# AbrahamSanders/realtime-codec-agent

Measured on AMD Instinct MI355X. Metric: batch-encode audio-hours/hour (+ xRT and p50 frame-step latency of 1 duplex stream in `duplex`), higher is better.
Workload: dtype f32; 1 GPU; batch MagiCodec-style encode, 16 kHz stereo, 0.1 s chunks / 2.0 s context, 256 windows per step (BASELINE configs[1]); codebook=131072x16

## Files before the change

include/rca.h:

```cpp
#ifndef RCA_H
#define RCA_H

#include <stdint.h>

#ifdef __cplusplus
extern "C" {
#endif

#define RCA_OK 0
#define RCA_ERR_ARG -1
#define RCA_ERR_HIP -2
#define RCA_ERR_STATE -3
#define RCA_ERR_MISSING -4

#define RCA_MAX_STAGES 8

typedef struct rca_codec rca_codec_t;
typedef struct rca_lm rca_lm_t;

#define RCA_F32 0
#define RCA_BF16 1
#define RCA_Q8_0 2
#define RCA_F16 3
#define RCA_Q6_K 5
// ... 92 lines not shown
    int32_t n_kv_heads;
    int32_t head_dim;
    int32_t ffn;
    int32_t n_ctx;
    float rms_eps;
    float rope_theta;
    int32_t rope_scaling;
    float rope_factor;
    float rope_low_freq_factor;
    float rope_high_freq_factor;
    int32_t rope_orig_ctx;
    int32_t logits_all;
    int32_t decode_weights;
} rca_lm_config_t;

typedef struct {
    int32_t top_k;
    float top_p;
    float min_p;
    float temp;
    uint32_t seed;
    int32_t n_bias;
    const int32_t* bias_ids;
    const float* bias_vals;
    float repeat_penalty;
    float freq_penalty;
    float presence_penalty;
    int32_t penalty_last_n;
} rca_sampler_params_t;

int rca_lm_create(const rca_lm_config_t* cfg, const rca_tensor_t* tensors, int32_t n_tensors,
                  int32_t device, rca_lm_t** out);
int rca_lm_create_random(const rca_lm_config_t* cfg, uint64_t seed, float init_std, int32_t device,
                         rca_lm_t** out);
int rca_lm_create_shared(rca_lm_t* parent, int32_t n_ctx, int32_t logits_all, rca_lm_t** out);
int rca_lm_destroy(rca_lm_t* h);

int rca_lm_reset(rca_lm_t* h);
int rca_lm_eval(rca_lm_t* h, const int32_t* ids, int32_t n);
int rca_lm_eval_async(rca_lm_t* h, const int32_t* ids, int32_t n);
int rca_lm_copy_kv(rca_lm_t* dst, rca_lm_t* src, int32_t n_pos);
int rca_lm_swap_kv(rca_lm_t* a, rca_lm_t* b);
int rca_lm_kv_remove(rca_lm_t* h, int32_t p0, int32_t p1);
int rca_lm_kv_read(rca_lm_t* h, int32_t layer, int32_t pos0, int32_t n_pos, uint16_t* k_host, uint16_t* v_host);
int rca_lm_set_low_priority(rca_lm_t* h, int32_t enable);
int rca_lm_get_n_tokens(const rca_lm_t* h, int32_t* n);
int rca_lm_set_n_tokens(rca_lm_t* h, int32_t n);
int rca_lm_get_logits(rca_lm_t* h, float* out_host);
int rca_lm_get_logits_row(rca_lm_t* h, int32_t pos, float* out_host);
int rca_lm_logits_dev(rca_lm_t* h, const float** out_dev);

int rca_lm_sampler_init(rca_lm_t* h, const rca_sampler_params_t* p);
int rca_lm_sample(rca_lm_t* h, int32_t* token);
int rca_lm_step(rca_lm_t* h, const int32_t* ids, int32_t n, int32_t* token);
int rca_lm_frame(rca_lm_t* h, const int32_t* first_pair, const int32_t* user_ids, int32_t n_steps, int32_t audio_id_floor,
                 int32_t* out_tokens, int32_t* n_done);
typedef struct rca_duplex_frame_args {
    const float* pcm_window;
    const int64_t* code_ctx;
    int32_t T;
    int32_t F_ctx;
    int32_t n_steps;
    int32_t n_samples;
    int32_t code_token_base;
    int32_t audio_id_floor;
    int32_t probe_id;
    int32_t first_pair[2];
} rca_duplex_frame_args_t;
typedef struct rca_duplex_frame_out {
    int64_t user_codes[8];
    int32_t tokens[8];
    int32_t n_done;
    int32_t flags;
    float probe_prob;
} rca_duplex_frame_out_t;
int rca_duplex_frame(rca_lm_t* lm, rca_codec_t* codec, const rca_duplex_frame_args_t* args, rca_duplex_frame_out_t* out,
                     float* pcm_out_host);
int rca_duplex_prepare(rca_lm_t* lm, int32_t T, int32_t F_ctx, int32_t n_steps, int32_t n_samples);
int rca_duplex_precapture(rca_lm_t* lm, rca_lm_t* twin, rca_codec_t* codec, const rca_duplex_frame_args_t* args, int32_t n_probe);
int rca_codec_workspace_sig(rca_codec_t* h, uint64_t* sig);
int rca_codec_stream_handoff(rca_codec_t* h, void* stream);
int rca_codec_codebook_size(const rca_codec_t* h, int32_t* n);
int rca_lm_step_probe(rca_lm_t* h, const int32_t* ids, int32_t n, const int32_t* probe_ids, int32_t n_probe, int32_t* token, float* probs_out);
int rca_lm_token_probs(rca_lm_t* h, const int32_t* token_ids, int32_t n, float* probs_out);
int rca_lm_mask_head_rows(rca_lm_t* h, int32_t row_begin, int32_t row_end);
int rca_lm_persist_codec_embeddings(rca_lm_t* h, const float* codec_embed, int32_t n_codes, int32_t dim,
                                    const float* w1, const float* b1, const float* w2, const float* b2,
                                    int32_t codec_vocab_start, float* out_f32);
int rca_lm_set_logits_all(rca_lm_t* h, int32_t enable);
int rca_lm_set_graphs(rca_lm_t* h, int32_t enable);
int rca_lm_set_mfma_prefill(rca_lm_t* h, int32_t enable);
int rca_lm_prefill_route(const rca_lm_t* h, int32_t* route);
int rca_lm_weight_format(const rca_lm_t* h, int32_t* fmt, int64_t* bytes_per_step);
int rca_lm_set_attn_fuse(rca_lm_t* h, int32_t enable);
int rca_lm_set_act_format(rca_lm_t* h, int32_t fmt);
int rca_lm_get_act_format(const rca_lm_t* h, int32_t* fmt);
int rca_lm_gemv_tap(rca_lm_t* h, int32_t layer, int32_t kind, const float* x_host, int32_t M, float* y_host, int64_t y_numel,
                    uint16_t* kv_host);
int rca_lm_sync(rca_lm_t* h);
int rca_codec_sync(rca_codec_t* h);

#ifdef __cplusplus
}
#endif
#endif
```

realtime_codec_agent_amd/_native.py:

```python
from __future__ import annotations

import ctypes as C
import os
import subprocess
from typing import Dict, Iterable, List, Optional, Tuple

import numpy as np

_PKG_DIR = os.path.dirname(os.path.abspath(__file__))
CSRC_DIR = os.path.join(_PKG_DIR, "csrc")
LIB_PATH = os.environ.get("RCA_LIB_PATH") or os.path.join(_PKG_DIR, "librca_hip.so")
HIP_SOURCES = ["rca_codec.hip", "rca_lm.hip"]
HIPCC_FLAGS = ["--offload-arch=gfx950", "-O3", "-ffp-contract=off", "-std=c++17", "-fPIC", "-shared",
               "-Wno-unused-result", "-mllvm", "-amdgpu-kernarg-preload-count=14"]

MAX_STAGES = 8
RCA_F32, RCA_BF16, RCA_Q8_0, RCA_F16, RCA_Q4_K, RCA_Q6_K, RCA_Q5_K, RCA_Q4_0, RCA_Q4_1 = 0, 1, 2, 3, 4, 5, 6, 7, 8


class RcaError(RuntimeError):
    pass


class Q8Blocks:
# ... 135 lines not shown


class Tensor(C.Structure):
    _fields_ = [("name", C.c_char_p), ("data", C.c_void_p), ("numel", C.c_int64), ("dtype", C.c_int32)]


class CodecConfigC(C.Structure):
    _fields_ = [
        ("sample_rate", C.c_int32),
        ("n_stages", C.c_int32),
        ("strides", C.c_int32 * MAX_STAGES),
        ("channels", C.c_int32 * (MAX_STAGES + 1)),
        ("k_in", C.c_int32),
        ("k_latent", C.c_int32),
        ("latent_dim", C.c_int32),
        ("codebook_size", C.c_int32),
        ("codebook_raw_dim", C.c_int32),
        ("codebook_dim", C.c_int32),
        ("leaky_slope", C.c_float),
    ]


class LMConfigC(C.Structure):
    _fields_ = [
        ("vocab_size", C.c_int32),
        ("hidden", C.c_int32),
        ("n_layers", C.c_int32),
        ("n_heads", C.c_int32),
        ("n_kv_heads", C.c_int32),
        ("head_dim", C.c_int32),
        ("ffn", C.c_int32),
        ("n_ctx", C.c_int32),
        ("rms_eps", C.c_float),
        ("rope_theta", C.c_float),
        ("rope_scaling", C.c_int32),
        ("rope_factor", C.c_float),
        ("rope_low_freq_factor", C.c_float),
        ("rope_high_freq_factor", C.c_float),
        ("rope_orig_ctx", C.c_int32),
        ("logits_all", C.c_int32),
        ("decode_weights", C.c_int32),
    ]


class SamplerParamsC(C.Structure):
    _fields_ = [
        ("top_k", C.c_int32),
        ("top_p", C.c_float),
        ("min_p", C.c_float),
        ("temp", C.c_float),
        ("seed", C.c_uint32),
        ("n_bias", C.c_int32),
        ("bias_ids", C.POINTER(C.c_int32)),
        ("bias_vals", C.POINTER(C.c_float)),
        ("repeat_penalty", C.c_float),
        ("freq_penalty", C.c_float),
        ("presence_penalty", C.c_float),
        ("penalty_last_n", C.c_int32),
    ]


class DuplexFrameArgsC(C.Structure):
    _fields_ = [
        ("pcm_window", C.c_void_p),
        ("code_ctx", C.c_void_p),
        ("T", C.c_int32),
        ("F_ctx", C.c_int32),
        ("n_steps", C.c_int32),
        ("n_samples", C.c_int32),
        ("code_token_base", C.c_int32),
        ("audio_id_floor", C.c_int32),
        ("probe_id", C.c_int32),
        ("first_pair", C.c_int32 * 2),
    ]


class DuplexFrameOutC(C.Structure):
    _fields_ = [
        ("user_codes", C.c_int64 * 8),
        ("tokens", C.c_int32 * 8),
        ("n_done", C.c_int32),
        ("flags", C.c_int32),
        ("probe_prob", C.c_float),
    ]


def sources() -> List[str]:
    return [os.path.join(CSRC_DIR, s) for s in HIP_SOURCES if os.path.exists(os.path.join(CSRC_DIR, s))]


def _build_key() -> Tuple[str, List[str], List[str]]:
    import hashlib
    extra = os.environ.get("RCA_EXTRA_HIPCC_FLAGS", "").split()
    hipcc = os.environ.get("HIPCC", "/opt/rocm/bin/hipcc")
    if not os.path.exists(hipcc):
        hipcc = "hipcc"
    cflags = [f for f in HIPCC_FLAGS if f != "-shared"] + extra
    return hashlib.sha1(" ".join([hipcc] + cflags).encode()).hexdigest()[:10], hipcc, cflags


def _stamp_path() -> str:
    return LIB_PATH + ".flags"


def needs_build() -> bool:
    if not os.path.exists(LIB_PATH):
        return True
    try:
        with open(_stamp_path()) as f:
            if f.read().strip() != _build_key()[0]:
                return True
    except OSError:
        return True
    deps = sources() + [os.path.join(CSRC_DIR, f) for f in os.listdir(CSRC_DIR) if f.endswith(".h")]
    deps.append(os.path.join(os.path.dirname(_PKG_DIR), "include", "rca.h"))
    t = os.path.getmtime(LIB_PATH)
    return any(os.path.getmtime(d) > t for d in deps if os.path.exists(d))


def build(force: bool = False, verbose: bool = False) -> str:
    key, hipcc, cflags = _build_key()
    extra = os.environ.get("RCA_EXTRA_HIPCC_FLAGS", "").split()
    if extra and not os.environ.get("RCA_LIB_PATH"):
        raise RcaError(f"RCA_EXTRA_HIPCC_FLAGS={' '.join(extra)!r} without RCA_LIB_PATH: a diagnostic build must not replace "
                       f"{LIB_PATH}; set RCA_LIB_PATH=/tmp/<name>.so")
    if not force and not needs_build():
        return LIB_PATH
    import fcntl
    obj_dir = os.path.join(CSRC_DIR, ".obj")
    os.makedirs(obj_dir, exist_ok=True)
    with open(os.path.join(obj_dir, ".lock"), "w") as lock:
        fcntl.flock(lock, fcntl.LOCK_EX)
        if not force and not needs_build():
            return LIB_PATH
        headers = [os.path.join(CSRC_DIR, f) for f in os.listdir(CSRC_DIR) if f.endswith(".h")]
        headers.append(os.path.join(os.path.dirname(_PKG_DIR), "include", "rca.h"))
        hdr_t = max([os.path.getmtime(p) for p in headers if os.path.exists(p)] + [0.0])
        sfx = f".{os.getpid()}.tmp"
        objs, jobs = [], []
        for src in sources():
            obj = os.path.join(obj_dir, f"{os.path.splitext(os.path.basename(src))[0]}.{key}.o")
            objs.append(obj)
            if force or not os.path.exists(obj) or os.path.getmtime(obj) < max(os.path.getmtime(src), hdr_t):
                cmd = [hipcc] + cflags + ["-c", src, "-o", obj + sfx]
                if verbose:
                    print(" ".join(cmd))
                jobs.append((subprocess.Popen(cmd), cmd, obj))
        tmps = [obj + sfx for _, _, obj in jobs] + [LIB_PATH + sfx]
        try:
            failed = [cmd for p, cmd, _ in jobs if p.wait() != 0]
            if failed:
                raise subprocess.CalledProcessError(1, failed[0])
            for _, _, obj in jobs:
                os.replace(obj + sfx, obj)
            cmd = [hipcc, "--offload-arch=gfx950", "-shared", "-fPIC"] + objs + ["-o", LIB_PATH + sfx]
            if verbose:
                print(" ".join(cmd))
            subprocess.check_call(cmd)
            os.replace(LIB_PATH + sfx, LIB_PATH)
            with open(_stamp_path() + sfx, "w") as f:
                f.write(key + "\n")
            os.replace(_stamp_path() + sfx, _stamp_path())
        finally:
            for t in tmps + [_stamp_path() + sfx]:
                if os.path.exists(t):
                    os.remove(t)
    return LIB_PATH


_lib = None

ABI_SYMBOLS = [
    "rca_last_error", "rca_device_count", "rca_device_sync", "rca_version",
    "rca_codec_create", "rca_codec_destroy", "rca_codec_hop", "rca_codec_num_frames",
    "rca_codec_encode", "rca_codec_encode_dev", "rca_codec_encode_windows_dev", "rca_codec_encode_chunk_range_dev", "rca_codec_encode_rows_dev",
    "rca_codec_decode", "rca_codec_decode_dev",
    "rca_codec_encode_tail_dev", "rca_codec_decode_tail_dev", "rca_codec_encode_tail", "rca_codec_decode_tail", "rca_codec_set_stream_graphs", "rca_codec_receptive_field", "rca_codec_set_window_trim",
    "rca_codec_encoder_dev", "rca_codec_quantize_dev", "rca_codec_decoder_dev", "rca_codec_codebook_dev",
    "rca_codec_codebook", "rca_codec_encode_tap", "rca_codec_encode_tap_bf16", "rca_codec_set_variant", "rca_codec_sync",
    "rca_codec_profile", "rca_codec_profile_read",
    "rca_lm_create", "rca_lm_create_random", "rca_lm_destroy", "rca_lm_reset", "rca_lm_eval",
    "rca_lm_get_n_tokens", "rca_lm_set_n_tokens", "rca_lm_get_logits", "rca_lm_get_logits_row",
    "rca_lm_logits_dev", "rca_lm_sampler_init", "rca_lm_sample", "rca_lm_step", "rca_lm_token_probs",
    "rca_lm_sync", "rca_lm_set_graphs", "rca_lm_mask_head_rows", "rca_lm_set_mfma_prefill", "rca_lm_set_logits_all",
    "rca_lm_persist_codec_embeddings", "rca_lm_create_shared", "rca_lm_eval_async", "rca_lm_copy_kv", "rca_lm_swap_kv",
    "rca_lm_set_low_priority", "rca_lm_frame", "rca_lm_weight_format", "rca_lm_set_attn_fuse", "rca_lm_prefill_route",
    "rca_lm_set_act_format", "rca_lm_get_act_format", "rca_lm_gemv_tap", "rca_lm_kv_remove", "rca_lm_kv_read",
    "rca_duplex_frame", "rca_codec_workspace_sig", "rca_codec_stream_handoff", "rca_codec_codebook_size", "rca_codec_set_mfma_mode", "rca_lm_step_probe", "rca_duplex_prepare", "rca_duplex_precapture",
]


def lib():
    global _lib
    if _lib is not None:
        return _lib
    if not os.path.exists(LIB_PATH):
        raise RcaError(
            f"{LIB_PATH} not found: build the HIP extension first (python -c 'import __graft_entry__ as g; g.build()'). "
            "There is no CPU fallback for the product path."
        )
    import torch
    try:
        _lib = C.CDLL(LIB_PATH)
    except OSError as e:
        raise RcaError(f"cannot load {LIB_PATH}: {e}") from e
    _lib.rca_last_error.restype = C.c_char_p
    _lib.rca_version.restype = C.c_char_p
    return _lib


def check(rc: int, what: str = "") -> None:
    if rc != 0:
        msg = lib().rca_last_error()
        raise RcaError(f"{what} failed (rc={rc}): {msg.decode(errors='replace') if msg else ''}")


def make_tensors(weights: Dict[str, np.ndarray]) -> Tuple[C.Array, list]:
    keep = []
    arr = (Tensor * len(weights))()
    for i, (name, a) in enumerate(weights.items()):
        if isinstance(a, (Q8Blocks, Q4KBlocks, Q5KBlocks, Q6KBlocks, Q40Blocks)):
            raw = np.ascontiguousarray(a.raw)
            nb = name.encode()
            keep += [raw, nb]
            arr[i] = Tensor(nb, raw.ctypes.data, int(np.prod(a.shape)), {Q8Blocks: RCA_Q8_0, Q4KBlocks: RCA_Q4_K, Q5KBlocks: RCA_Q5_K, Q6KBlocks: RCA_Q6_K, Q40Blocks: RCA_Q4_0, Q41Blocks: RCA_Q4_1}[type(a)])
            continue
        if a.dtype == np.uint16:
            dt = RCA_BF16
        elif a.dtype == np.float16:
            dt = RCA_F16
        else:
            a = np.ascontiguousarray(a, dtype=np.float32)
            dt = RCA_F32
        a = np.ascontiguousarray(a)
        nb = name.encode()
        keep += [a, nb]
        arr[i] = Tensor(nb, a.ctypes.data, a.size, dt)
    return arr, keep


def codec_config_c(cfg) -> CodecConfigC:
    c = CodecConfigC()
    c.sample_rate = cfg.sample_rate
    c.n_stages = len(cfg.strides)
    for i, s in enumerate(cfg.strides):
        c.strides[i] = s
    for i, ch in enumerate(cfg.channels):
        c.channels[i] = ch
    c.k_in, c.k_latent, c.latent_dim = cfg.k_in, cfg.k_latent, cfg.latent_dim
    c.codebook_size, c.codebook_raw_dim, c.codebook_dim = cfg.codebook_size, cfg.codebook_raw_dim, cfg.codebook_dim
    c.leaky_slope = cfg.leaky_slope
    return c
```

realtime_codec_agent_amd/csrc/rca_lm.hip:

```cpp
#include <algorithm>
#include <type_traits>
#include <cmath>

#include "rca_common.h"

using namespace rca;

typedef unsigned short bf16_t;
typedef _Float16 f16_t;
typedef unsigned u32x4 __attribute__((ext_vector_type(4)));
typedef float f32x4 __attribute__((ext_vector_type(4)));
typedef _Float16 f16x2 __attribute__((ext_vector_type(2)));

#define LM_MAXM 1024
#define LM_STATE_DECODE_BYTES (8 + 4 * 16)
#define LM_TILE32 32
#define LM_GEMV_M 2
#define LM_PREFILL_MIN 8
#define LM_KSLICE 2048
#define LM_MAXSPLIT 4
#define ATT_KEYS 256
#define LM_GRAPH_BUCKETS 8
#define ATT_EPOCH_INTS 64
#define ATT_TAG_MAXSP 128
#define ATT_TAG_SPINS (1 << 22)
#define SAMP_MAXK 256
#define LM_FRAME_MAX 8
#define LM_FRAME_USER0 8

struct LmDevState {
    int n_tokens;
    int m;
    int ids[LM_MAXM];
    unsigned long long rng_counter;
    int out_token;
    int pad;
    int frame_out[LM_FRAME_MAX];
};

struct SamplerDev {
    int top_k;
    float top_p, min_p, temp;
    unsigned long long seed;
    int n_bias;
    int bias_ids[8];
    float bias_vals[8];
    float repeat_penalty, freq_penalty, presence_penalty;
    int last_n;
    int patch;
    int big_k;
    int big_p;
};

typedef float f32x16 __attribute__((ext_vector_type(16)));
__device__ __forceinline__ bf16_t f32_to_bf16_rne(float f) {
    unsigned u = __float_as_uint(f);
    u += 0x7FFFu + ((u >> 16) & 1u);
    return (bf16_t)(u >> 16);
}
__device__ __forceinline__ float bf16_lo(unsigned u) { return __uint_as_float(u << 16); }
__device__ __forceinline__ float bf16_hi(unsigned u) { return __uint_as_float(u & 0xffff0000u); }
template <int CTRL>
__device__ __forceinline__ float dpp_mov(float v) {
    return __builtin_bit_cast(float, __builtin_amdgcn_update_dpp(0, __builtin_bit_cast(int, v), CTRL, 0xF, 0xF, true));
}
#define DPP_XOR1 0xB1
#define DPP_XOR2 0x4E
#define DPP_ROR4 0x124
#define DPP_ROR8 0x128
#define DPP_HALF_MIRROR 0x141
template <typename OP>
__device__ __forceinline__ float wave_butterfly(float v, OP op) {
    float a = v, b = v;
    asm volatile("s_nop 1\n\tv_permlane32_swap_b32 %0, %1\n\ts_nop 1" : "+v"(a), "+v"(b));
    v = op(a, b);
    a = v; b = v;
    asm volatile("s_nop 1\n\tv_permlane16_swap_b32 %0, %1\n\ts_nop 1" : "+v"(a), "+v"(b));
    v = op(a, b);
    v = op(v, dpp_mov<DPP_ROR8>(v));
    v = op(v, dpp_mov<DPP_ROR4>(v));
    v = op(v, dpp_mov<DPP_XOR2>(v));
    v = op(v, dpp_mov<DPP_XOR1>(v));
    return v;
}
__device__ __forceinline__ float wave_sum(float v) {
    return wave_butterfly(v, [](float a, float b) { return a + b; });
}
__device__ __forceinline__ float wave_max(float v) {
    return wave_butterfly(v, [](float a, float b) { return fmaxf(a, b); });
}

__global__ __launch_bounds__(256) void lm_embed_kernel(const LmDevState* __restrict__ stt, const void* __restrict__ table, int f32tab,
                                                       float* __restrict__ x, int H, int V) {
    const int m = blockIdx.x;
    if (m >= stt->m) return;
    int id = stt->ids[m];
    id = id < 0 ? 0 : (id >= V ? V - 1 : id);
    if (f32tab) {
        const float* row = reinterpret_cast<const float*>(table) + (long)id * H;
        for (int h = threadIdx.x; h < H; h += 256) x[(long)m * H + h] = row[h];
// ... 1695 lines not shown
        }
    }
}
__global__ __launch_bounds__(256) void lm_q8_pack_kernel(const signed char* __restrict__ q, const f16_t* __restrict__ d, int N, int K, int qkv_pairs,
                                                         u32x4* __restrict__ qs, unsigned* __restrict__ sc) {
    const long nchunk = K >> 3, npairs = N >> 1;
    for (long i = (long)blockIdx.x * blockDim.x + threadIdx.x; i < npairs * nchunk; i += (long)gridDim.x * blockDim.x) {
        const long pp = i / nchunk;
        const int c = (int)(i - pp * nchunk);
        const long ra = qkv_pairs ? (pp >> 5) * 64 + (pp & 31) : 2 * pp;
        const long rb = qkv_pairs ? ra + 32 : ra + 1;
        const uint2 a = *reinterpret_cast<const uint2*>(q + ra * K + 8 * c);
        const uint2 b = *reinterpret_cast<const uint2*>(q + rb * K + 8 * c);
        qs[i] = u32x4{a.x, a.y, b.x, b.y};
        if ((c & 3) == 0) {
            const unsigned short da = __builtin_bit_cast(unsigned short, d[ra * (K >> 5) + (c >> 2)]);
            const unsigned short db = __builtin_bit_cast(unsigned short, d[rb * (K >> 5) + (c >> 2)]);
            sc[q8_sc_index(pp, c >> 2, K >> 5)] = (unsigned)da | ((unsigned)db << 16);
        }
    }
}

struct WMat {
    int fmt = WF_BF16;
    int N = 0, K = 0;
    bf16_t* w = nullptr;
    u32x4* qs = nullptr;
    unsigned* sc = nullptr;
    unsigned* dd = nullptr;
    unsigned* qh = nullptr;
    void release() {
        for (void* p : {(void*)w, (void*)qs, (void*)sc, (void*)dd, (void*)qh})
            if (p) (void)hipFree(p);
        w = nullptr; qs = nullptr; sc = nullptr; dd = nullptr; qh = nullptr;
    }
    const bf16_t* wptr() const { return fmt == WF_Q5K ? reinterpret_cast<const bf16_t*>(qh) : w; }
    long stream_bytes() const {
        const long n = (long)N * K;
        if (fmt == WF_Q5K) return n / 2 + n / 8 + n / 16 + n / 64;
        if (fmt == WF_Q40 || fmt == WF_Q41) return n / 2 + n / 8;
        return fmt == WF_Q8 ? n + n / 16 : (fmt == WF_Q4K ? n / 2 + n / 16 + n / 64 : (fmt == WF_Q6K ? n + n / 4 : 2 * n));
    }
};
struct LmLayer {
    WMat qkv, o, gu, down;
    WMat vseg;
    bool split_v = false;
    float *attn_norm = nullptr, *ffn_norm = nullptr;
};

struct rca_lm {
    int n_cus = 256;
    rca_lm_config_t cfg;
    int device = 0;
    hipStream_t stream = nullptr;
    void* embed = nullptr;
    int embed_f32 = 0;
    WMat head;
    float* final_norm = nullptr;
    std::vector<LmLayer> layers;
    float *cos_t = nullptr, *sin_t = nullptr;
    f16_t *kc = nullptr, *vc = nullptr;
    f16_t* kv_stage = nullptr;
    long kv_layer_stride = 0;
    int n_ctx_pad = 0, n_splits = 0;
    float *x = nullptr, *xn = nullptr, *qkv = nullptr, *attn = nullptr, *hbuf = nullptr,
          *att_part = nullptr, *logits = nullptr, *probs_dev = nullptr;
    int* probe_ids_dev = nullptr;
    int* att_arrive = nullptr;
    bf16_t *xh = nullptr, *xl = nullptr;
    float* gpart = nullptr;
    long logits_rows_cap = 0;
    int logits_rows = 0;
    LmDevState* stt = nullptr;
    SamplerDev* samp = nullptr;
    SampWork* swork = nullptr;
    LmDevState* h_stt = nullptr;
    int* h_probe = nullptr;
    int n_tokens = 0;
    bool sampler_set = false;
    bool samp_full = false;
    bool samp_patch = false, samp_big_k = false, samp_big_p = false;
    struct GraphSet { const f16_t* kc = nullptr; hipGraphExec_t g[3][LM_GRAPH_BUCKETS] = {}; hipGraphExec_t fg[LM_FRAME_MAX + 1][LM_GRAPH_BUCKETS] = {};
                      hipGraphExec_t gp[3][LM_GRAPH_BUCKETS] = {}; int gp_nprobe[3][LM_GRAPH_BUCKETS] = {};
                      int tile_m[2] = {0, 0}; hipGraphExec_t tile_g[2] = {nullptr, nullptr}; int tile_seen[2] = {0, 0};
                      unsigned long long last_use = 0; };
    GraphSet gset[2];
    unsigned long long gset_clock = 0;
    bool async_pending = false;
    unsigned long long rng_host = 0;
    bool graphs_enabled = true;
    bool mfma_prefill = true;
    bool fuse_attn = true;
    int act_format = 0;
    rca_lm* weights_of = nullptr;
    int borrowers = 0;
    bool zombie = false;
    struct DuplexState* duplex = nullptr;
};
struct DuplexState;
static void duplex_destroy(DuplexState* d);
static void duplex_drop_graphs(DuplexState* d);

static int lm_alloc(void** p, size_t bytes) {
    hipError_t e = hipMalloc(p, bytes);
    if (e != hipSuccess) return fail(RCA_ERR_HIP, "hipMalloc(%zu) -> %s", bytes, hipGetErrorString(e));
    return RCA_OK;
}

static void lm_free_weights(rca_lm* h) {
    for (auto& L : h->layers) {
        for (WMat* m : {&L.qkv, &L.o, &L.gu, &L.down, &L.vseg}) m->release();
        for (void* p : {(void*)L.attn_norm, (void*)L.ffn_norm})
            if (p) (void)hipFree(p);
    }
    h->head.release();
    for (void* p : {(void*)h->embed, (void*)h->final_norm, (void*)h->cos_t, (void*)h->sin_t})
        if (p) (void)hipFree(p);
    h->layers.clear();
    h->embed = nullptr;
    h->final_norm = h->cos_t = h->sin_t = nullptr;
}

static void lm_drop_graph_set(rca_lm::GraphSet& gs) {
    for (int i = 0; i < 3; ++i)
        for (int b = 0; b < LM_GRAPH_BUCKETS; ++b) {
            if (gs.g[i][b]) { (void)hipGraphExecDestroy(gs.g[i][b]); gs.g[i][b] = nullptr; }
            if (gs.gp[i][b]) { (void)hipGraphExecDestroy(gs.gp[i][b]); gs.gp[i][b] = nullptr; }
        }
    for (int i = 0; i <= LM_FRAME_MAX; ++i)
        for (int b = 0; b < LM_GRAPH_BUCKETS; ++b)
            if (gs.fg[i][b]) { (void)hipGraphExecDestroy(gs.fg[i][b]); gs.fg[i][b] = nullptr; }
    for (int i = 0; i < 2; ++i) {
        if (gs.tile_g[i]) { (void)hipGraphExecDestroy(gs.tile_g[i]); gs.tile_g[i] = nullptr; }
        gs.tile_m[i] = gs.tile_seen[i] = 0;
    }
    gs.kc = nullptr;
}
static void lm_drop_graphs(rca_lm* h) {
    for (auto& gs : h->gset) lm_drop_graph_set(gs);
    duplex_drop_graphs(h->duplex);
}
static rca_lm::GraphSet& lm_graph_set(rca_lm* h) {
    rca_lm::GraphSet* hit = nullptr;
    for (auto& gs : h->gset)
        if (gs.kc == h->kc) hit = &gs;
    if (!hit) {
        hit = h->gset[0].last_use <= h->gset[1].last_use ? &h->gset[0] : &h->gset[1];
        lm_drop_graph_set(*hit);
        hit->kc = h->kc;
    }
    hit->last_use = ++h->gset_clock;
    return *hit;
}
template <class F>
static int lm_capture(hipStream_t st, hipGraphExec_t* exec, const char* tag, F&& enqueue) {
    hipGraph_t g = nullptr;
    RCA_HIP(hipStreamSynchronize(st));
    RCA_HIP(hipStreamBeginCapture(st, hipStreamCaptureModeThreadLocal));
    const int rc = enqueue();
    hipError_t e = hipStreamEndCapture(st, &g);
    if (rc != RCA_OK) { if (g) (void)hipGraphDestroy(g); return rc; }
    if (e != hipSuccess) return fail(RCA_ERR_HIP, "%s capture: %s", tag, hipGetErrorString(e));
    e = hipGraphInstantiate(exec, g, nullptr, nullptr, 0);
    (void)hipGraphDestroy(g);
    if (e != hipSuccess) { *exec = nullptr; return fail(RCA_ERR_HIP, "%s graph instantiate: %s", tag, hipGetErrorString(e)); }
    (void)hipGraphUpload(*exec, st);
    return RCA_OK;
}

extern "C" int rca_lm_destroy(rca_lm_t* h) {
    if (!h) return RCA_OK;
    (void)hipSetDevice(h->device);
    if (h->stream) (void)hipStreamSynchronize(h->stream);
    lm_drop_graphs(h);
    duplex_destroy(h->duplex);
    h->duplex = nullptr;
    for (void* p : {(void*)h->kc, (void*)h->vc, (void*)h->kv_stage, (void*)h->x, (void*)h->xn, (void*)h->qkv, (void*)h->attn, (void*)h->hbuf,
                    (void*)h->att_part, (void*)h->logits, (void*)h->probs_dev, (void*)h->probe_ids_dev, (void*)h->att_arrive, (void*)h->xh, (void*)h->xl,
                    (void*)h->gpart, (void*)h->stt, (void*)h->samp, (void*)h->swork})
        if (p) (void)hipFree(p);
    h->kc = h->vc = h->kv_stage = nullptr;
    h->x = h->xn = h->qkv = h->attn = h->hbuf = h->att_part = h->logits = h->probs_dev = h->gpart = nullptr;
    h->probe_ids_dev = nullptr; h->att_arrive = nullptr; h->xh = h->xl = nullptr; h->stt = nullptr; h->samp = nullptr; h->swork = nullptr;
    if (h->h_stt) { (void)hipHostFree(h->h_stt); h->h_stt = nullptr; }
    if (h->h_probe) { (void)hipHostFree(h->h_probe); h->h_probe = nullptr; }
    if (h->stream) { (void)hipStreamDestroy(h->stream); h->stream = nullptr; }
    if (h->weights_of) {
        rca_lm* owner = h->weights_of;
        h->layers.clear();
        if (--owner->borrowers == 0 && owner->zombie) { lm_free_weights(owner); delete owner; }
        delete h;
        return RCA_OK;
    }
    if (h->borrowers > 0) {
        h->zombie = true;
        return RCA_OK;
    }
    lm_free_weights(h);
    delete h;
    return RCA_OK;
}

static int lm_check_cfg(const rca_lm_config_t* c) {
    if (!c) return fail(RCA_ERR_ARG, "null config");
    if (c->head_dim != 64) return fail(RCA_ERR_ARG, "head_dim must be 64 (got %d)", c->head_dim);
    if (c->n_kv_heads < 1 || c->n_heads % c->n_kv_heads) return fail(RCA_ERR_ARG, "n_heads must be a multiple of n_kv_heads");
    const int G = c->n_heads / c->n_kv_heads;
    if (G != 1 && G != 2 && G != 4) return fail(RCA_ERR_ARG, "query group size %d unsupported (1, 2, 4)", G);
    if (c->hidden % 8 || c->ffn % 8 || (c->n_heads * c->head_dim) % 8) return fail(RCA_ERR_ARG, "hidden/ffn must be multiples of 8");
    if (c->hidden > LM_KSLICE || c->n_heads * c->head_dim > LM_KSLICE) return fail(RCA_ERR_ARG, "hidden > %d unsupported", LM_KSLICE);
    if (c->ffn > LM_KSLICE * LM_MAXSPLIT) return fail(RCA_ERR_ARG, "ffn > %d unsupported", LM_KSLICE * LM_MAXSPLIT);
    if (c->ffn > LM_KSLICE && c->ffn % LM_KSLICE) return fail(RCA_ERR_ARG, "ffn above %d must be a multiple of it", LM_KSLICE);
    if (c->vocab_size < 2 || c->n_layers < 1 || c->n_ctx < 2) return fail(RCA_ERR_ARG, "bad sizes");
    if (c->decode_weights < 0 || c->decode_weights > 6) return fail(RCA_ERR_ARG, "decode_weights %d (0 as supplied, 1 q8_0, 2 f16, 3 q4_k, 4 q5_k, 5 q4_0, 6 q4_1)", c->decode_weights);
// ... 365 lines not shown
        const size_t sc_bytes = (size_t)((npairs + 7) / 8) * (K / 16) * 8 * 2 * 4;
        if ((rc = lm_alloc((void**)&out->qs, (size_t)npairs * nchunk * 16)) != RCA_OK || (rc = lm_alloc((void**)&out->sc, sc_bytes)) != RCA_OK) { raw->release(); return rc; }
        (void)hipMemsetAsync(out->sc, 0, sc_bytes, h->stream);
        lm_q6k_pack_kernel<<<4096, 256, 0, h->stream>>>(raw->q, (const signed char*)raw->d, (const f16_t*)raw->dd, N, K, qkv_pairs, out->qs, (float*)out->sc);
        hipError_t e = hipStreamSynchronize(h->stream);
        raw->release();
        if (e != hipSuccess) return fail(RCA_ERR_HIP, "Q6_K pack of %s: %s", what, hipGetErrorString(e));
        return RCA_OK;
    }
    if (raw->fmt != WF_Q8) {
        out->w = raw->w16;
        raw->w16 = nullptr;
        return RCA_OK;
    }
    const int N = out->N, K = out->K;
    if ((K % 32) || (N % 2) || (qkv_pairs && (N % 64))) { raw->release(); return fail(RCA_ERR_ARG, "q8_0 weights: %s is %d x %d (K must be a multiple of 32, N even)", what, N, K); }
    int rc;
    const long npairs = N / 2, nchunk = K / 8;
    if ((rc = lm_alloc((void**)&out->qs, (size_t)npairs * nchunk * 16)) != RCA_OK ||
        (rc = lm_alloc((void**)&out->sc, (size_t)((npairs + 7) / 8) * (K / 32) * 8 * 4)) != RCA_OK) { raw->release(); return rc; }
    (void)hipMemsetAsync(out->sc, 0, (size_t)((npairs + 7) / 8) * (K / 32) * 8 * 4, h->stream);
    lm_q8_pack_kernel<<<4096, 256, 0, h->stream>>>(raw->q, raw->d, N, K, qkv_pairs, out->qs, out->sc);
    hipError_t e = hipStreamSynchronize(h->stream);
    raw->release();
    if (e != hipSuccess) return fail(RCA_ERR_HIP, "q8_0 pack of %s: %s", what, hipGetErrorString(e));
    return RCA_OK;
}

static int g128_splits(int N, int K);
static bool lm_can_gemm128(const rca_lm* h);
static int lm_common_init(rca_lm* h, const rca_tensor_t* ts, int nt, const rca_lm* rope_src = nullptr) {
    const rca_lm_config_t& c = h->cfg;
    int rc;
    const int half = c.head_dim / 2;
    h->n_ctx_pad = (c.n_ctx + ATT_KEYS - 1) / ATT_KEYS * ATT_KEYS;
    h->n_splits = h->n_ctx_pad / ATT_KEYS;
    if (rope_src) {
        h->cos_t = rope_src->cos_t;
        h->sin_t = rope_src->sin_t;
    } else {
    std::vector<float> inv(half);
    const rca_tensor_t* tinv = find_tensor(ts, nt, "rope.inv_freq");
    if (tinv) {
        if (tinv->numel != half || tinv->dtype != RCA_F32) return fail(RCA_ERR_ARG, "rope.inv_freq must hold %d f32", half);
        memcpy(inv.data(), tinv->data, half * sizeof(float));
    } else {
        for (int i = 0; i < half; ++i) {
            double f = 1.0 / pow((double)c.rope_theta, (double)(2 * i) / (double)c.head_dim);
            if (c.rope_scaling == 1) {
                const double low_wl = (double)c.rope_orig_ctx / c.rope_low_freq_factor;
                const double high_wl = (double)c.rope_orig_ctx / c.rope_high_freq_factor;
                const double wl = 2.0 * M_PI / f;
                if (wl > low_wl) f = f / c.rope_factor;
                else if (wl >= high_wl) {
                    const double smooth = ((double)c.rope_orig_ctx / wl - c.rope_low_freq_factor) / (c.rope_high_freq_factor - c.rope_low_freq_factor);
                    f = (1.0 - smooth) * f / c.rope_factor + smooth * f;
                }
            }
            inv[i] = (float)f;
        }
    }
    float* inv_dev = nullptr;
    if ((rc = lm_alloc((void**)&inv_dev, half * 4)) != RCA_OK) return rc;
    RCA_HIP(hipMemcpy(inv_dev, inv.data(), half * 4, hipMemcpyHostToDevice));
    if ((rc = lm_alloc((void**)&h->cos_t, (size_t)h->n_ctx_pad * half * 4)) != RCA_OK) return rc;
    if ((rc = lm_alloc((void**)&h->sin_t, (size_t)h->n_ctx_pad * half * 4)) != RCA_OK) return rc;
    lm_rope_table_kernel<<<cdiv((long)h->n_ctx_pad * half, 256), 256, 0, h->stream>>>(inv_dev, h->cos_t, h->sin_t, h->n_ctx_pad, half);
    RCA_HIP(hipStreamSynchronize(h->stream));
    (void)hipFree(inv_dev);
    }
    h->kv_layer_stride = (long)h->n_ctx_pad * c.n_kv_heads * c.head_dim;
    const size_t kvb = (size_t)c.n_layers * h->kv_layer_stride * 2;
    if ((rc = lm_alloc((void**)&h->kc, kvb)) != RCA_OK) return rc;
    if ((rc = lm_alloc((void**)&h->vc, kvb)) != RCA_OK) return rc;
    RCA_HIP(hipMemsetAsync(h->kc, 0, kvb, h->stream));
    RCA_HIP(hipMemsetAsync(h->vc, 0, kvb, h->stream));
    const int H = c.hidden, QKV = (c.n_heads + 2 * c.n_kv_heads) * c.head_dim, AO = c.n_heads * c.head_dim;
    if ((rc = lm_alloc((void**)&h->x, (size_t)LM_MAXM * H * 4)) != RCA_OK) return rc;
    if ((rc = lm_alloc((void**)&h->xn, (size_t)LM_MAXM * H * 4)) != RCA_OK) return rc;
    if ((rc = lm_alloc((void**)&h->qkv, (size_t)LM_MAXM * QKV * 4)) != RCA_OK) return rc;
    if ((rc = lm_alloc((void**)&h->attn, (size_t)LM_MAXM * AO * 4)) != RCA_OK) return rc;
    if ((rc = lm_alloc((void**)&h->hbuf, (size_t)LM_MAXM * c.ffn * 4)) != RCA_OK) return rc;
    if ((rc = lm_alloc((void**)&h->att_part, (size_t)(LM_MAXM / 2) * c.n_kv_heads * h->n_splits * 8 * 66 * 4)) != RCA_OK) return rc;
    h->logits_rows_cap = c.logits_all ? 64 : 1;
    if ((rc = lm_alloc((void**)&h->logits, (size_t)h->logits_rows_cap * c.vocab_size * 4)) != RCA_OK) return rc;
    if ((rc = lm_alloc((void**)&h->probs_dev, (64 + 2 * PROBS_SLICES) * 4)) != RCA_OK) return rc;
    if ((rc = lm_alloc((void**)&h->probe_ids_dev, 64 * 4)) != RCA_OK) return rc;
    {
        const size_t gb = ATT_EPOCH_INTS * 4 + (size_t)c.n_kv_heads * h->n_splits * 8 * 66 * 8;
        if ((rc = lm_alloc((void**)&h->att_arrive, gb)) != RCA_OK) return rc;
        RCA_HIP(hipMemsetAsync(h->att_arrive, 0, gb, h->stream));
        int ones[ATT_EPOCH_INTS];
        for (int i = 0; i < ATT_EPOCH_INTS; ++i) ones[i] = 1;
        RCA_HIP(hipMemcpyAsync(h->att_arrive, ones, sizeof(ones), hipMemcpyHostToDevice, h->stream));
        RCA_HIP(hipStreamSynchronize(h->stream));
    }
    {
        const size_t kmax = (size_t)std::max(std::max(H, AO), c.ffn);
        if ((rc = lm_alloc((void**)&h->xh, (size_t)LM_MAXM * kmax * 2)) != RCA_OK) return rc;
        if ((rc = lm_alloc((void**)&h->xl, (size_t)LM_MAXM * kmax * 2)) != RCA_OK) return rc;
        RCA_HIP(hipMemsetAsync(h->xh, 0, (size_t)LM_MAXM * kmax * 2, h->stream));
        RCA_HIP(hipMemsetAsync(h->xl, 0, (size_t)LM_MAXM * kmax * 2, h->stream));
        size_t part_rows = 64;
        if (lm_can_gemm128(h)) {
            const int Fq = c.ffn;
            const int nk[4][2] = {{QKV, H}, {H, AO}, {2 * Fq, H}, {H, Fq}};
            for (int i = 0; i < 4; ++i) {
                const int ns = g128_splits(nk[i][0], nk[i][1]);
                if (ns > 1) part_rows = std::max(part_rows, (size_t)ns * nk[i][0]);
            }
        }
        if ((rc = lm_alloc((void**)&h->gpart, part_rows * LM_MAXM * 4)) != RCA_OK) return rc;
    }
    if ((rc = lm_alloc((void**)&h->stt, sizeof(LmDevState))) != RCA_OK) return rc;
    if ((rc = lm_alloc((void**)&h->samp, sizeof(SamplerDev))) != RCA_OK) return rc;
    RCA_HIP(hipMemsetAsync(h->stt, 0, sizeof(LmDevState), h->stream));
    RCA_HIP(hipMemsetAsync(h->samp, 0, sizeof(SamplerDev), h->stream));
    if ((rc = lm_alloc((void**)&h->swork, sizeof(SampWork))) != RCA_OK) return rc;
    RCA_HIP(hipMemsetAsync(h->swork, 0, sizeof(SampWork), h->stream));
    RCA_HIP(hipHostMalloc((void**)&h->h_stt, sizeof(LmDevState), hipHostMallocDefault));
    memset(h->h_stt, 0, sizeof(LmDevState));
    RCA_HIP(hipHostMalloc((void**)&h->h_probe, 128 * 4, hipHostMallocDefault));
    memset(h->h_probe, 0, 128 * 4);
    RCA_HIP(hipStreamSynchronize(h->stream));
    return RCA_OK;
}

static int lm_new(const rca_lm_config_t* cfg, int device, rca_lm** out) {
    int rc;
    if ((rc = lm_check_cfg(cfg)) != RCA_OK) return rc;
    RCA_HIP(hipSetDevice(device));
    rca_lm* h = new rca_lm();
    h->cfg = *cfg;
    h->device = device;
    if (hipDeviceGetAttribute(&h->n_cus, hipDeviceAttributeMultiprocessorCount, device) != hipSuccess || h->n_cus <= 0) h->n_cus = 256;
    h->layers.resize(cfg->n_layers);
    if (hipStreamCreateWithFlags(&h->stream, hipStreamNonBlocking) != hipSuccess) {
        delete h;
        return fail(RCA_ERR_HIP, "stream create");
    }
    *out = h;
    return RCA_OK;
}

static int lm_build_layer(rca_lm* h, LmLayer& L, RawMat& q, RawMat& k, RawMat& v, RawMat& o, RawMat& g, RawMat& u, RawMat& dn) {
    const int want = h->cfg.decode_weights;
    int rc = RCA_OK;
    RawMat qkv, gu;
    auto done = [&](int code) { for (RawMat* m : {&q, &k, &v, &o, &g, &u, &dn, &qkv, &gu}) m->release(); return code; };
    for (RawMat* m : {&q, &k, &v, &o, &g, &u, &dn})
        if ((rc = lm_raw_convert(h, m, want)) != RCA_OK) return done(rc);
    if (q.fmt == k.fmt && k.fmt != v.fmt) {
        if ((rc = lm_raw_concat(h, {&q, &k}, &qkv, "the fused QK projection")) != RCA_OK) return done(rc);
        if ((rc = lm_finish_mat(h, &v, 1, &L.vseg, "v_proj")) != RCA_OK) return done(rc);
        L.split_v = true;
    } else if ((rc = lm_raw_concat(h, {&q, &k, &v}, &qkv, "the fused QKV projection")) != RCA_OK) return done(rc);
    q.release(); k.release(); v.release();
    if ((rc = lm_raw_interleave(h, &g, &u, &gu, "the fused gate/up projection")) != RCA_OK) return done(rc);
    g.release(); u.release();
    if ((rc = lm_finish_mat(h, &qkv, 1, &L.qkv, "the fused QKV projection")) != RCA_OK) return done(rc);
    if ((rc = lm_finish_mat(h, &o, 0, &L.o, "o_proj")) != RCA_OK) return done(rc);
    if ((rc = lm_finish_mat(h, &gu, 0, &L.gu, "the fused gate/up projection")) != RCA_OK) return done(rc);
    if ((rc = lm_finish_mat(h, &dn, 0, &L.down, "down_proj")) != RCA_OK) return done(rc);
    return done(RCA_OK);
}

extern "C" int rca_lm_create(const rca_lm_config_t* cfg, const rca_tensor_t* ts, int32_t nt, int32_t device, rca_lm_t** out) {
// ... 59 lines not shown
        lm_fill_f32_kernel<<<cdiv(n, 256), 256, 0, h->stream>>>(*p, n, 1.0f);
        return RCA_OK;
    };
    h->embed_f32 = 0;
    if ((rc = lm_alloc(&h->embed, (size_t)V * H * 2)) != RCA_OK) return bail(rc);
    lm_random_bf16_kernel<<<4096, 256, 0, h->stream>>>((bf16_t*)h->embed, V * H, seed, tid++, scale);
    if ((rc = rnd(V, H, 0, &h->head, "lm_head")) != RCA_OK || (rc = ones(&h->final_norm, H)) != RCA_OK) return bail(rc);
    for (int l = 0; l < c.n_layers; ++l) {
        LmLayer& L = h->layers[l];
        tid = 10ull * (l + 1) + 3;
        if ((rc = rnd(Q + 2 * KVD, H, 1, &L.qkv, "the fused QKV projection")) != RCA_OK || (rc = rnd(H, Q, 0, &L.o, "o_proj")) != RCA_OK ||
            (rc = rnd(2 * F, H, 0, &L.gu, "the fused gate/up projection")) != RCA_OK || (rc = rnd(H, F, 0, &L.down, "down_proj")) != RCA_OK ||
            (rc = ones(&L.attn_norm, H)) != RCA_OK || (rc = ones(&L.ffn_norm, H)) != RCA_OK)
            return bail(rc);
    }
    RCA_HIP(hipStreamSynchronize(h->stream));
    if ((rc = lm_common_init(h, nullptr, 0)) != RCA_OK) return bail(rc);
    *out = h;
    return RCA_OK;
}

extern "C" int rca_lm_create_shared(rca_lm_t* parent, int32_t n_ctx, int32_t logits_all, rca_lm_t** out) {
    if (!parent || !out) return fail(RCA_ERR_ARG, "null argument");
    rca_lm* owner = parent->weights_of ? parent->weights_of : parent;
    if (owner->zombie) return fail(RCA_ERR_STATE, "create_shared: the parent handle was destroyed");
    rca_lm_config_t cfg = parent->cfg;
    cfg.n_ctx = n_ctx;
    cfg.logits_all = logits_all;
    if (n_ctx < 2 || (n_ctx + ATT_KEYS - 1) / ATT_KEYS * ATT_KEYS > owner->n_ctx_pad)
        return fail(RCA_ERR_ARG, "create_shared: n_ctx %d exceeds the parent's RoPE tables (%d positions)", n_ctx, owner->n_ctx_pad);
    rca_lm* h = nullptr;
    int rc;
    if ((rc = lm_new(&cfg, parent->device, &h)) != RCA_OK) return rc;
    h->embed = owner->embed;
    h->embed_f32 = owner->embed_f32;
    h->head = owner->head;
    h->final_norm = owner->final_norm;
    h->layers = owner->layers;
    h->weights_of = owner;
    h->fuse_attn = parent->fuse_attn;
    h->mfma_prefill = parent->mfma_prefill;
    h->act_format = parent->act_format;
    owner->borrowers++;
    if ((rc = lm_common_init(h, nullptr, 0, owner)) != RCA_OK) { rca_lm_destroy(h); return rc; }
    *out = h;
    return RCA_OK;
}

static constexpr int WF_FORMATS[] = {WF_BF16, WF_Q8, WF_F16, WF_Q4K, WF_Q6K, WF_Q5K, WF_Q40};
template <class F>
static void wf_dispatch(int fmt, F&& f) {
    switch (fmt) {
        case WF_Q6K: return f(std::integral_constant<int, WF_Q6K>{});
        case WF_Q4K: return f(std::integral_constant<int, WF_Q4K>{});
        case WF_Q5K: return f(std::integral_constant<int, WF_Q5K>{});
        case WF_Q40: case WF_Q41: return f(std::integral_constant<int, WF_Q40>{});
        case WF_Q8: return f(std::integral_constant<int, WF_Q8>{});
        case WF_F16: return f(std::integral_constant<int, WF_F16>{});
        default: return f(std::integral_constant<int, WF_BF16>{});
    }
}
struct GemvGeom { int R, bpw; };
enum { GEMV_QKV = 0, GEMV_O, GEMV_GU, GEMV_DOWN, GEMV_HEAD, GEMV_KINDS };
static GemvGeom gemv_geom(int kind, int N, bool q8) {
    static GemvGeom tab[2][GEMV_KINDS];
    static bool init = false;
    if (!init) {
        const GemvGeom def[2][GEMV_KINDS] = {{{4, 1}, {4, 1}, {16, 2}, {4, 1}, {16, 8}}, {{4, 1}, {4, 1}, {16, 2}, {4, 1}, {16, 8}}};
        const char* names[2][GEMV_KINDS] = {{"RCA_GEMV_QKV", "RCA_GEMV_O", "RCA_GEMV_GU", "RCA_GEMV_DOWN", "RCA_GEMV_HEAD"},
                                           {"RCA_GEMVQ_QKV", "RCA_GEMVQ_O", "RCA_GEMVQ_GU", "RCA_GEMVQ_DOWN", "RCA_GEMVQ_HEAD"}};
        for (int f = 0; f < 2; ++f)
            for (int k = 0; k < GEMV_KINDS; ++k) {
                tab[f][k] = def[f][k];
                const char* e = getenv(names[f][k]);
                int r = 0, bw = 0;
                if (e && sscanf(e, "%d,%d", &r, &bw) == 2 && (r == 4 || r == 8 || r == 16) && bw >= 1) tab[f][k] = {r, bw};
            }
        init = true;
    }
    GemvGeom g = tab[q8 ? 1 : 0][kind];
    while (g.bpw > 1 && (N + g.R * g.bpw - 1) / (g.R * g.bpw) < 64) g.bpw >>= 1;
    return g;
}
template <int M, int NIT, int PRO, int EPI, int Q, int ACT>
static void launch_gemv_r(const GemvGeom& g, rca_lm* h, const WMat& w, const float* x, float* y, int N, int K, int ldy, const GemvPro& pro,
                          const GemvRope& rope, hipStream_t st) {
    const int grid = cdiv(cdiv(N, g.R), g.bpw);
    const GemvQ8 qa{w.qs, w.sc, w.dd};
    switch (g.R) {
        case 4: lm_gemv_kernel<M, NIT, 4, PRO, EPI, Q, ACT><<<grid, 256, 0, st>>>(h->stt, w.wptr(), qa, x, N, K, y, g.bpw, ldy, pro, rope); break;
        case 8: lm_gemv_kernel<M, NIT, 8, PRO, EPI, Q, ACT><<<grid, 256, 0, st>>>(h->stt, w.wptr(), qa, x, N, K, y, g.bpw, ldy, pro, rope); break;
        default:
            if constexpr (!((Q == WF_Q5K || Q == WF_Q40) && NIT == 4))
                lm_gemv_kernel<M, NIT, 16, PRO, EPI, Q, ACT><<<grid, 256, 0, st>>>(h->stt, w.wptr(), qa, x, N, K, y, g.bpw, ldy, pro, rope);
            break;
    }
}
template <int PRO, int EPI, int Q, int ACT = 0>
static void launch_gemv_q(GemvGeom g, rca_lm* h, int M, const WMat& w, const float* x, float* y, int N, int K, int ldy, const GemvPro& pro,
                          const GemvRope& rope, hipStream_t st) {
    const int nit = cdiv(cdiv(K >> 3, 4), 64);
    const int lpr = (Q == WF_Q8 || Q == WF_Q6K) ? 2 : ((Q == WF_Q4K || Q == WF_Q5K || Q == WF_Q40) ? 4 : 1);
    const int max_loads = (Q == WF_Q4K || Q == WF_Q5K || Q == WF_Q40) ? 8 : 16;
    while (g.R > 4 && (g.R / lpr) * (nit == 3 ? 4 : nit) > max_loads) g.R >>= 1;
    if ((Q == WF_Q4K || Q == WF_Q6K || Q == WF_Q5K || Q == WF_Q40) && g.R < 8) g.R = 8;
    if (PRO == 0 && EPI == 3 && nit > 1) {
        if (nit == 2) {
            if (M == 1) launch_gemv_r<1, 2, 0, 3, Q, ACT>(g, h, w, x, y, N, K, ldy, pro, rope, st);
            else launch_gemv_r<2, 2, 0, 3, Q, ACT>(g, h, w, x, y, N, K, ldy, pro, rope, st);
        } else {
            if (M == 1) launch_gemv_r<1, 4, 0, 3, Q, ACT>(g, h, w, x, y, N, K, ldy, pro, rope, st);
            else launch_gemv_r<2, 4, 0, 3, Q, ACT>(g, h, w, x, y, N, K, ldy, pro, rope, st);
        }
        return;
    }
    if (M == 1) launch_gemv_r<1, 1, PRO, EPI, Q, ACT>(g, h, w, x, y, N, K, ldy, pro, rope, st);
    else launch_gemv_r<2, 1, PRO, EPI, Q, ACT>(g, h, w, x, y, N, K, ldy, pro, rope, st);
}
template <int PRO, int EPI>
static void launch_gemv(int kind, rca_lm* h, int M, const WMat& w, const float* x, float* y, int N, int K, int ldy, const GemvPro& pro,
                        const GemvRope& rope, hipStream_t st) {
    const GemvGeom g = gemv_geom(kind, N, wf_packed(w.fmt));
    wf_dispatch(w.fmt, [&](auto wf) {
        constexpr int Q = decltype(wf)::value;
        if constexpr (wf_packed(Q))
            if (h->act_format == 1) return launch_gemv_q<PRO, EPI, Q, 1>(g, h, M, w, x, y, N, K, ldy, pro, rope, st);
        launch_gemv_q<PRO, EPI, Q>(g, h, M, w, x, y, N, K, ldy, pro, rope, st);
    });
}

#define CMB_PRE 32
template <bool COHERENT>
__device__ __forceinline__ float attn_part_load(const float* p) {
    if (COHERENT) return __hip_atomic_load(p, __ATOMIC_RELAXED, __HIP_MEMORY_SCOPE_AGENT);
    return *p;
}
template <bool COHERENT>
__device__ __forceinline__ float attn_merge_row(const float* __restrict__ base, int nsp, int d) {
    const long sstride = 32L * 66;
    float pv[CMB_PRE];
#pragma unroll
    for (int j = 0; j < CMB_PRE; ++j) pv[j] = attn_part_load<COHERENT>(base + (long)min(j, nsp - 1) * sstride + 2 + d);
    float mx, ml0, ll0;
    {
        const int sp = min(d, nsp - 1);
        ml0 = attn_part_load<COHERENT>(base + sp * sstride);
        ll0 = attn_part_load<COHERENT>(base + sp * sstride + 1);
        if (d >= nsp) { ml0 = -INFINITY; ll0 = 0.0f; }
        mx = ml0;
    }
    for (int s0 = 64; s0 < nsp; s0 += 64) {
        const int sp = s0 + d;
        mx = fmaxf(mx, sp < nsp ? attn_part_load<COHERENT>(base + sp * sstride) : -INFINITY);
    }
    mx = wave_max(mx);
    float L = 0.0f, O = 0.0f;
    {
        const float fl = (ml0 == -INFINITY) ? 0.0f : __expf(ml0 - mx);
        const int cnt = min(64, nsp);
#pragma unroll
        for (int j = 0; j < CMB_PRE; ++j) {
            if (j < cnt) {
                const float f = __shfl(fl, j), l = __shfl(ll0, j);
                L = __builtin_fmaf(l, f, L);
                O = __builtin_fmaf(f == 0.0f ? 0.0f : pv[j], f, O);
            }
        }
        for (int j = CMB_PRE; j < cnt; ++j) {
            const float f = __shfl(fl, j), l = __shfl(ll0, j);
            const float p = attn_part_load<COHERENT>(base + (long)j * sstride + 2 + d);
            L = __builtin_fmaf(l, f, L);
            O = __builtin_fmaf(f == 0.0f ? 0.0f : p, f, O);
        }
    }
    for (int s0 = 64; s0 < nsp; s0 += 64) {
        const int spl = min(s0 + d, nsp - 1);
        const float ml = attn_part_load<COHERENT>(base + spl * sstride), ll = attn_part_load<COHERENT>(base + spl * sstride + 1);
        const float fl = (ml == -INFINITY) ? 0.0f : __expf(ml - mx);
        const int cnt = min(64, nsp - s0);
        for (int j = 0; j < cnt; ++j) {
            const float f = __shfl(fl, j), l = __shfl(ll, j);
            const float p = attn_part_load<COHERENT>(base + (long)(s0 + j) * sstride + 2 + d);
            L = __builtin_fmaf(l, f, L);
            O = __builtin_fmaf(f == 0.0f ? 0.0f : p, f, O);
        }
    }
    return O / L;
}
// ... 635 lines not shown
        } else {
            *reinterpret_cast<float4*>(attn_out + obase) = make_float4(o[0], o[1], o[2], o[3]);
            *reinterpret_cast<float4*>(attn_out + obase + 4) = make_float4(o[4], o[5], o[6], o[7]);
        }
    }
}
template <int G>
static void launch_attention_flash_g(rca_lm* h, int M, const f16_t* kc, const f16_t* vc, hipStream_t st, bf16_t* hi, bf16_t* lo) {
    const rca_lm_config_t& c = h->cfg;
    const float scale = 1.0f / sqrtf((float)c.head_dim);
    const int ntiles = cdiv(M * G, 32);
    if (c.n_kv_heads * cdiv(ntiles, 4) >= h->n_cus)
        lm_attn_flash_kernel<G, 4><<<dim3(c.n_kv_heads, cdiv(ntiles, 4)), 64 * FLASH_WAVES * 4, 0, st>>>(h->stt, h->qkv, kc, vc, h->attn, hi, lo, c.n_heads, c.n_kv_heads, scale, c.n_ctx);
    else if (c.n_kv_heads * cdiv(ntiles, 2) >= h->n_cus)
        lm_attn_flash_kernel<G, 2><<<dim3(c.n_kv_heads, cdiv(ntiles, 2)), 64 * FLASH_WAVES * 2, 0, st>>>(h->stt, h->qkv, kc, vc, h->attn, hi, lo, c.n_heads, c.n_kv_heads, scale, c.n_ctx);
    else
        lm_attn_flash_kernel<G, 1><<<dim3(c.n_kv_heads, ntiles), 64 * FLASH_WAVES, 0, st>>>(h->stt, h->qkv, kc, vc, h->attn, hi, lo, c.n_heads, c.n_kv_heads, scale, c.n_ctx);
}
static void launch_attention_flash(rca_lm* h, int M, const f16_t* kc, const f16_t* vc, hipStream_t st, bf16_t* hi, bf16_t* lo) {
    const int G = h->cfg.n_heads / h->cfg.n_kv_heads;
    if (G == 4) launch_attention_flash_g<4>(h, M, kc, vc, st, hi, lo);
    else if (G == 2) launch_attention_flash_g<2>(h, M, kc, vc, st, hi, lo);
    else launch_attention_flash_g<1>(h, M, kc, vc, st, hi, lo);
}

static void launch_attention_mfma(rca_lm* h, int M, int nsp_launch, const f16_t* kc, const f16_t* vc, hipStream_t st,
                                  bf16_t* hi = nullptr, bf16_t* lo = nullptr, bool prefill = false) {
    const rca_lm_config_t& c = h->cfg;
    static const bool flash = !(getenv("RCA_LM_FLASH") && atoi(getenv("RCA_LM_FLASH")) == 0);
    if (prefill && flash) {
        launch_attention_flash(h, M, kc, vc, st, hi, lo);
        return;
    }
    const int G = c.n_heads / c.n_kv_heads;
    const float scale = 1.0f / sqrtf((float)c.head_dim);
    dim3 agm(c.n_kv_heads, nsp_launch, cdiv(M * G, 32));
    static bool attr_done = false;
    if (!attr_done) {
        (void)hipFuncSetAttribute((const void*)lm_attn_mfma_kernel<4>, hipFuncAttributeMaxDynamicSharedMemorySize, ATTM_LDS);
        (void)hipFuncSetAttribute((const void*)lm_attn_mfma_kernel<2>, hipFuncAttributeMaxDynamicSharedMemorySize, ATTM_LDS);
        (void)hipFuncSetAttribute((const void*)lm_attn_mfma_kernel<1>, hipFuncAttributeMaxDynamicSharedMemorySize, ATTM_LDS);
        attr_done = true;
    }
    const bool fuse = h->fuse_attn && !hi && agm.z == 1 && c.n_kv_heads * nsp_launch <= 256 && M * G <= 8 && nsp_launch <= ATT_TAG_MAXSP && c.n_kv_heads <= ATT_EPOCH_INTS;
    int* arrive = fuse ? h->att_arrive : nullptr;
#define RCA_ATTN_LAUNCH(GG)                                                                                                                        \
    lm_attn_mfma_kernel<GG><<<agm, 512, ATTM_LDS, st>>>(h->stt, h->qkv, kc, vc, c.n_heads, c.n_kv_heads, h->n_splits, scale, c.n_ctx, h->att_part, \
                                                        arrive, h->attn);                                                                          \
    if (!fuse) lm_attn_mfma_combine_kernel<GG><<<M * c.n_heads, 64, 0, st>>>(h->stt, h->att_part, h->attn, c.n_heads, c.n_kv_heads, h->n_splits, nsp_launch, hi, lo);
    if (G == 4) { RCA_ATTN_LAUNCH(4) }
    else if (G == 2) { RCA_ATTN_LAUNCH(2) }
    else { RCA_ATTN_LAUNCH(1) }
#undef RCA_ATTN_LAUNCH
}

static int lm_splits_needed(const rca_lm* h, int m) { return std::min(h->n_splits, (h->n_tokens + m + ATT_KEYS - 1) / ATT_KEYS); }

static const GemvPro nopro{nullptr, nullptr, 0.0f, 0};
static const GemvRope norope{nullptr, nullptr, nullptr, nullptr, 0, 0, 0, 0};
static void lm_launch_qkv(rca_lm* h, int l, int M, hipStream_t st) {
    const rca_lm_config_t& c = h->cfg;
    const LmLayer& L = h->layers[l];
    const int QKV = (c.n_heads + 2 * c.n_kv_heads) * c.head_dim;
    const GemvPro pro{h->x, L.attn_norm, c.rms_eps, 0};
    GemvRope rope{h->cos_t, h->sin_t, h->kc + (long)l * h->kv_layer_stride, h->vc + (long)l * h->kv_layer_stride, c.n_heads, c.n_kv_heads, c.n_ctx, 0};
    launch_gemv<1, 2>(GEMV_QKV, h, M, L.qkv, nullptr, h->qkv, L.qkv.N, c.hidden, QKV, pro, rope, st);
    if (L.split_v) {
        rope.row_base = L.qkv.N;
        launch_gemv<1, 2>(GEMV_QKV, h, M, L.vseg, nullptr, h->qkv, L.vseg.N, c.hidden, QKV, pro, rope, st);
    }
}
static void lm_launch_o(rca_lm* h, int l, int M, hipStream_t st) {
    const int AO = h->cfg.n_heads * h->cfg.head_dim;
    launch_gemv<0, 3>(GEMV_O, h, M, h->layers[l].o, h->attn, h->x, h->cfg.hidden, AO, h->cfg.hidden, nopro, norope, st);
}
static void lm_launch_gu(rca_lm* h, int l, int M, hipStream_t st) {
    const rca_lm_config_t& c = h->cfg;
    const LmLayer& L = h->layers[l];
    launch_gemv<1, 1>(GEMV_GU, h, M, L.gu, nullptr, h->hbuf, 2 * c.ffn, c.hidden, c.ffn, GemvPro{h->x, L.ffn_norm, c.rms_eps, 0}, norope, st);
}
static void lm_launch_down(rca_lm* h, int l, int M, hipStream_t st) {
    launch_gemv<0, 3>(GEMV_DOWN, h, M, h->layers[l].down, h->hbuf, h->x, h->cfg.hidden, h->cfg.ffn, h->cfg.hidden, nopro, norope, st);
}
static void lm_launch_head(rca_lm* h, int M, hipStream_t st, float* out, bool only_last) {
    const rca_lm_config_t& c = h->cfg;
    launch_gemv<1, 0>(GEMV_HEAD, h, M, h->head, nullptr, out, c.vocab_size, c.hidden, c.vocab_size, GemvPro{h->x, h->final_norm, c.rms_eps, only_last ? 1 : 0}, norope, st);
}

static int lm_enqueue_pass(rca_lm* h, int M, int want_logits, hipStream_t st, int nsp_launch, bool skip_embed = false) {
    const rca_lm_config_t& c = h->cfg;
    if (M < 1 || M > LM_GEMV_M) return fail(RCA_ERR_ARG, "decode pass of %d tokens", M);
    if (!skip_embed) lm_embed_kernel<<<M, 256, 0, st>>>(h->stt, h->embed, h->embed_f32, h->x, c.hidden, c.vocab_size);
    for (int l = 0; l < c.n_layers; ++l) {
        lm_launch_qkv(h, l, M, st);
        launch_attention_mfma(h, M, nsp_launch, h->kc + (long)l * h->kv_layer_stride, h->vc + (long)l * h->kv_layer_stride, st);
        lm_launch_o(h, l, M, st);
        lm_launch_gu(h, l, M, st);
        lm_launch_down(h, l, M, st);
    }
    if (want_logits == 1) lm_launch_head(h, 1, st, h->logits, true);
    else if (want_logits) lm_launch_head(h, M, st, h->logits, false);
    RCA_LAUNCH_CHECK();
    return RCA_OK;
}

#define G128_PITCH 40
#define G128_LDS_T(NT) (2 * (NT) * 128 * G128_PITCH * 2)
#define G128_LDS G128_LDS_T(3)
typedef __bf16 bf16x2_t __attribute__((ext_vector_type(2)));
__device__ __forceinline__ unsigned pack_bf16x2(float a, float b) {
    const bf16x2_t v = {(__bf16)a, (__bf16)b};
    return __builtin_bit_cast(unsigned, v);
}
__device__ __forceinline__ void split_w8(const float (&w)[8], uint4& hi, uint4& lo) {
    unsigned ph[4], pl[4];
#pragma unroll
    for (int j = 0; j < 4; ++j) {
        ph[j] = pack_bf16x2(w[2 * j], w[2 * j + 1]);
        pl[j] = pack_bf16x2(w[2 * j] - bf16_lo(ph[j]), w[2 * j + 1] - bf16_hi(ph[j]));
    }
    hi = make_uint4(ph[0], ph[1], ph[2], ph[3]);
    lo = make_uint4(pl[0], pl[1], pl[2], pl[3]);
}
template <int EPI, int WF>
__global__ __launch_bounds__(256, 2) void lm_gemm128_kernel(const LmDevState* __restrict__ stt, const bf16_t* __restrict__ W, GemvQ8 q8,
                                                            const bf16_t* __restrict__ xh, const bf16_t* __restrict__ xl, int N, int K,
                                                            int kslice, float* __restrict__ y, int ldy, bf16_t* __restrict__ oh,
                                                            bf16_t* __restrict__ ol, float* __restrict__ part, GemvRope rope, int nseq) {
    constexpr int NT = WF == WF_BF16 ? 3 : 4;
    extern __shared__ __attribute__((aligned(16))) bf16_t g128_lds[];
    typedef bf16_t tile_t[NT][128 * G128_PITCH];
    tile_t* sm = reinterpret_cast<tile_t*>(g128_lds);
    const int tid = threadIdx.x;
    const int lane = tid & 63;
    const int half = lane >> 5;
    const int wave = __builtin_amdgcn_readfirstlane(tid >> 6);
    const int wr = wave >> 1, wc = wave & 1;
    const int n0 = blockIdx.x * 128;
    const int ks = blockIdx.y * nseq * kslice;
    const int tb = blockIdx.z * 128;
    const int spf = kslice >> 5;
    const int nstage = nseq * spf;
    const int srow0 = tid >> 2, skc = (tid & 3) * 8;
    const bf16_t* gW = W + (long)(n0 + srow0) * K + ks + skc;
    const bf16_t* gH = xh + (long)(tb + srow0) * K + ks + skc;
    const bf16_t* gL = xl + (long)(tb + srow0) * K + ks + skc;
    const long rstep = 64L * K;
    const int soff0 = srow0 * G128_PITCH + skc, soff1 = soff0 + 64 * G128_PITCH;
    const int qp = tid >> 2;
    const long q_nkb = K >> 5;
    const u32x4* gQ = (WF == WF_Q8 || WF == WF_Q6K) ? q8.qs + ((long)(n0 >> 1) + qp) * (K >> 3) + (ks >> 3) + (tid & 3) : nullptr;
    const unsigned* gS = WF == WF_Q8 ? q8.sc + q8_sc_index((n0 >> 1) + qp, ks >> 5, q_nkb) : nullptr;
    const float* gS6 = WF == WF_Q6K ? reinterpret_cast<const float*>(q8.sc) + 2 * q8_sc_index((n0 >> 1) + qp, (ks >> 4) + ((tid & 3) >> 1), K >> 4) : nullptr;
    const int q4quad = tid >> 3, q4half = tid & 1, q4slot = 4 * ((n0 >> 2) + q4quad) + 2 * q4half;
    constexpr bool W40 = WF == WF_Q40;
    constexpr bool W4 = WF == WF_Q4K || WF == WF_Q5K || W40;
    const unsigned* gH5 = WF == WF_Q5K ? reinterpret_cast<const unsigned*>(W) + ((long)(n0 >> 2) + q4quad) * (K >> 3) + (ks >> 3) + ((tid >> 1) & 3) : nullptr;
    const uint2* gQ4 = W4 ? reinterpret_cast<const uint2*>(q8.qs + ((long)(n0 >> 2) + q4quad) * (K >> 3) + (ks >> 3) + ((tid >> 1) & 3)) + q4half : nullptr;
    const unsigned short* gS4 = (W4 && !W40) ? reinterpret_cast<const unsigned short*>(q8.sc) + q4k_scm_index(q4slot, ks >> 5, q_nkb) : nullptr;
    const unsigned* gF40 = W40 ? q8.sc + q4k_scm_index(q4slot, ks >> 5, q_nkb) : nullptr;
    const unsigned* gD4 = (W4 && !W40) ? q8.dd + q4k_scm_index(q4slot, 0, K >> 8) : nullptr;
    int q4row[2];
#pragma unroll
    for (int i = 0; i < 2; ++i) q4row[i] = (int)packed_slot_row(4 * q4quad + 2 * q4half + i, EPI == GEMM_EPI_ROPE);
    const int q4soff0 = q4row[0] * G128_PITCH + ((tid >> 1) & 3) * 8, q4soff1 = q4row[1] * G128_PITCH + ((tid >> 1) & 3) * 8;
    const int qra = EPI == GEMM_EPI_ROPE ? (qp >> 5) * 64 + (qp & 31) : 2 * qp;
    const int qsoff0 = qra * G128_PITCH + skc, qsoff1 = qsoff0 + (EPI == GEMM_EPI_ROPE ? 32 : 1) * G128_PITCH;
    constexpr int DW = 1, DX = 1;
    uint4 rw[DW][2], rh[DX][2], rl[DX][2];
    unsigned rs[DW];
    uint2 rdd[DW];
    auto gload_w = [&](int slot, int s) {
        const int st = min(s, nstage - 1);
        if (W4) {
            const uint2 t = gQ4[(long)st * 8];
            rw[slot][0] = make_uint4(t.x, t.y, WF == WF_Q5K ? gH5[(long)st * 4] : 0u, 0u);
            if constexpr (W40) {
                rdd[slot] = *reinterpret_cast<const uint2*>(gF40 + (long)st * 16);
            } else {
                rs[slot] = *reinterpret_cast<const unsigned*>(gS4 + (long)st * 16);
                rdd[slot] = *reinterpret_cast<const uint2*>(gD4 + (long)(((ks >> 5) + st) >> 3) * 16);
            }
        } else if (WF == WF_Q6K) {
// ... 438 lines not shown
extern "C" int rca_lm_set_n_tokens(rca_lm_t* h, int32_t n) {
    if (!h) return fail(RCA_ERR_ARG, "null");
    if (n < 0 || n > h->cfg.n_ctx) return fail(RCA_ERR_ARG, "n_tokens %d outside [0, %d]", n, h->cfg.n_ctx);
    h->n_tokens = n;
    return RCA_OK;
}
extern "C" int rca_lm_sync(rca_lm_t* h) {
    if (!h) return fail(RCA_ERR_ARG, "null");
    RCA_HIP(hipSetDevice(h->device));
    RCA_HIP(hipStreamSynchronize(h->stream));
    h->async_pending = false;
    return RCA_OK;
}

static int lm_eval_impl(rca_lm_t* h, const int32_t* ids, int32_t n, bool wait_last, bool as_prefill) {
    if (!h || (!ids && n > 0) || n < 0) return fail(RCA_ERR_ARG, "eval: bad argument");
    if (n == 0) return RCA_OK;
    if (h->n_tokens + n > h->cfg.n_ctx) return fail(RCA_ERR_STATE, "context overflow: %d + %d > n_ctx %d", h->n_tokens, n, h->cfg.n_ctx);
    for (int i = 0; i < n; ++i)
        if (ids[i] < 0 || ids[i] >= h->cfg.vocab_size) return fail(RCA_ERR_ARG, "eval: token id %d at index %d is outside the vocabulary [0, %d)", ids[i], i, h->cfg.vocab_size);
    RCA_HIP(hipSetDevice(h->device));
    hipStream_t st = h->stream;
    int rc;
    if (h->async_pending) { RCA_HIP(hipStreamSynchronize(st)); h->async_pending = false; }
    const bool all = h->cfg.logits_all != 0;
    if (all && n > h->logits_rows_cap) {
        RCA_HIP(hipStreamSynchronize(st));
        lm_drop_graphs(h);
        (void)hipFree(h->logits);
        h->logits = nullptr;
        h->logits_rows_cap = n;
        if ((rc = lm_alloc((void**)&h->logits, (size_t)n * h->cfg.vocab_size * 4)) != RCA_OK) return rc;
    }
    float* logits_base = h->logits;
    const int route = lm_prefill_route(h);
    if ((n > LM_PREFILL_MIN || as_prefill) && route != LM_ROUTE_GEMV) {
        const bool big = route == LM_ROUTE_TILE128;
        const int tile = big ? LM_MAXM : LM_TILE32;
        static const bool tile_graphs = !(getenv("RCA_LM_TILE_GRAPHS") && atoi(getenv("RCA_LM_TILE_GRAPHS")) == 0) &&
                                        !(getenv("RCA_LM_FLASH") && atoi(getenv("RCA_LM_FLASH")) == 0);
        if (!wait_last && big && n <= tile && h->graphs_enabled && tile_graphs) {
            rca_lm::GraphSet& gs = lm_graph_set(h);
            int slot = -1;
            for (int i = 0; i < 2; ++i)
                if (gs.tile_m[i] == n) slot = i;
            if (slot < 0) {
                slot = gs.tile_seen[0] <= gs.tile_seen[1] ? 0 : 1;
                if (gs.tile_g[slot]) { (void)hipGraphExecDestroy(gs.tile_g[slot]); gs.tile_g[slot] = nullptr; }
                gs.tile_m[slot] = n; gs.tile_seen[slot] = 0;
            }
            if (++gs.tile_seen[slot] >= 2) {
                lm_stage_state(h, ids, n);
                if (!gs.tile_g[slot]) {
                    rc = lm_capture(st, &gs.tile_g[slot], "tile", [&]() -> int {
                        hipError_t e = hipMemcpyAsync(h->stt, h->h_stt, lm_state_bytes(n), hipMemcpyHostToDevice, st);
                        if (e != hipSuccess) return fail(RCA_ERR_HIP, "tile capture memcpy: %s", hipGetErrorString(e));
                        const int r = lm_enqueue_prefill_tile128(h, n, st, 1);
                        if (r == RCA_OK) lm_launch_head(h, 1, st, h->logits, true);
                        return r;
                    });
                    if (rc != RCA_OK) return rc;
                }
                RCA_HIP(hipGraphLaunch(gs.tile_g[slot], st));
                h->n_tokens += n;
                h->logits_rows = 1;
                h->async_pending = true;
                return RCA_OK;
            }
        }
        for (int off = 0; off < n; off += tile) {
            const int m = std::min(tile, n - off);
            const bool last = off + m >= n;
            if ((rc = lm_push_state(h, ids + off, m, st)) != RCA_OK) return rc;
            rc = big ? lm_enqueue_prefill_tile128(h, m, st, lm_splits_needed(h, m)) : lm_enqueue_prefill_tile(h, m, st, lm_splits_needed(h, m));
            if (rc != RCA_OK) return rc;
            if (last) {
                lm_launch_head(h, 1, st, h->logits, true);
                RCA_LAUNCH_CHECK();
            }
            h->n_tokens += m;
            if (!last) RCA_HIP(hipStreamSynchronize(st));
        }
    } else {
        for (int off = 0; off < n; off += LM_GEMV_M) {
            const int m = std::min(LM_GEMV_M, n - off);
            const bool last = off + m >= n;
            if ((rc = lm_push_state(h, ids + off, m, st)) != RCA_OK) return rc;
            if (all) h->logits = logits_base + (long)off * h->cfg.vocab_size;
            rc = lm_enqueue_pass(h, m, all ? 2 : (last ? 1 : 0), st, lm_splits_needed(h, m));
            h->logits = logits_base;
            if (rc != RCA_OK) return rc;
            h->n_tokens += m;
            if (!last) RCA_HIP(hipStreamSynchronize(st));
        }
    }
    h->logits_rows = all ? n : 1;
    if (wait_last) RCA_HIP(hipStreamSynchronize(st));
    else h->async_pending = true;
    return RCA_OK;
}
extern "C" int rca_lm_eval(rca_lm_t* h, const int32_t* ids, int32_t n) { return lm_eval_impl(h, ids, n, true, false); }
extern "C" int rca_lm_eval_async(rca_lm_t* h, const int32_t* ids, int32_t n) { return lm_eval_impl(h, ids, n, false, true); }

static int lm_same_cache_shape(const rca_lm* a, const rca_lm* b) {
    return a->device == b->device && a->cfg.n_layers == b->cfg.n_layers && a->cfg.n_kv_heads == b->cfg.n_kv_heads &&
           a->cfg.head_dim == b->cfg.head_dim && a->n_ctx_pad == b->n_ctx_pad && a->cfg.n_ctx == b->cfg.n_ctx;
}
extern "C" int rca_lm_copy_kv(rca_lm_t* dst, rca_lm_t* src, int32_t n_pos) {
    if (!dst || !src || dst == src) return fail(RCA_ERR_ARG, "copy_kv: two different handles needed");
    if (!lm_same_cache_shape(dst, src)) return fail(RCA_ERR_ARG, "copy_kv: the two KV caches differ in shape");
    if (n_pos < 0 || n_pos > src->cfg.n_ctx) return fail(RCA_ERR_ARG, "copy_kv: %d positions outside [0, %d]", n_pos, src->cfg.n_ctx);
    RCA_HIP(hipSetDevice(dst->device));
    RCA_HIP(hipStreamSynchronize(src->stream));
    src->async_pending = false;
    if (dst->async_pending) { RCA_HIP(hipStreamSynchronize(dst->stream)); dst->async_pending = false; }
    const size_t bytes = (size_t)n_pos * src->cfg.n_kv_heads * src->cfg.head_dim * sizeof(f16_t);
    for (int l = 0; l < src->cfg.n_layers && bytes; ++l) {
        RCA_HIP(hipMemcpyAsync(dst->kc + (long)l * dst->kv_layer_stride, src->kc + (long)l * src->kv_layer_stride, bytes, hipMemcpyDeviceToDevice, dst->stream));
        RCA_HIP(hipMemcpyAsync(dst->vc + (long)l * dst->kv_layer_stride, src->vc + (long)l * src->kv_layer_stride, bytes, hipMemcpyDeviceToDevice, dst->stream));
    }
    dst->async_pending = true;
    return RCA_OK;
}
extern "C" int rca_lm_swap_kv(rca_lm_t* a, rca_lm_t* b) {
    if (!a || !b || a == b) return fail(RCA_ERR_ARG, "swap_kv: two different handles needed");
    if (!lm_same_cache_shape(a, b)) return fail(RCA_ERR_ARG, "swap_kv: the two KV caches differ in shape");
    RCA_HIP(hipSetDevice(a->device));
    RCA_HIP(hipStreamSynchronize(a->stream));
    RCA_HIP(hipStreamSynchronize(b->stream));
    a->async_pending = b->async_pending = false;
    std::swap(a->kc, b->kc);
    std::swap(a->vc, b->vc);
    return RCA_OK;
}

__global__ __launch_bounds__(256) void lm_kv_shift_kernel(f16_t* kc, f16_t* vc, f16_t* __restrict__ stage_w, const f16_t* __restrict__ stage_r,
                                                          const float* __restrict__ cos_d, const float* __restrict__ sin_d,
                                                          long layer_stride, int n_layers, int nkv, int src_pos, int n_src, int dst_pos, int n_dst) {
    const long stage_v = (long)n_layers * ATT_KEYS * nkv * 64;
    const long ua = (long)n_layers * n_src * nkv * 4, ub = (long)n_layers * n_dst * nkv * 4;
    for (long u = (long)blockIdx.x * 256 + threadIdx.x; u < ua + ub; u += (long)gridDim.x * 256) {
        const bool rot = u < ua;
        long t = rot ? u : u - ua;
        const int npos = rot ? n_src : n_dst;
        const int q = (int)(t & 3);
        t >>= 2;
        const int kvh = (int)(t % nkv);
        t /= nkv;
        const int r = (int)(t % npos), l = (int)(t / npos);
        const long so = (((long)l * ATT_KEYS + r) * nkv + kvh) * 64 + q * 8;
        const long co = (long)l * layer_stride + ((long)((rot ? src_pos : dst_pos) + r) * nkv + kvh) * 64 + q * 8;
        if (rot) {
            const f16x8 k1 = *reinterpret_cast<const f16x8*>(kc + co), k2 = *reinterpret_cast<const f16x8*>(kc + co + 32);
            const u32x4 v1 = *reinterpret_cast<const u32x4*>(vc + co), v2 = *reinterpret_cast<const u32x4*>(vc + co + 32);
            float c[8], s[8];
            *reinterpret_cast<f32x4*>(c) = *reinterpret_cast<const f32x4*>(cos_d + q * 8);
            *reinterpret_cast<f32x4*>(c + 4) = *reinterpret_cast<const f32x4*>(cos_d + q * 8 + 4);
            *reinterpret_cast<f32x4*>(s) = *reinterpret_cast<const f32x4*>(sin_d + q * 8);
            *reinterpret_cast<f32x4*>(s + 4) = *reinterpret_cast<const f32x4*>(sin_d + q * 8 + 4);
            f16x8 o1, o2;
#pragma unroll
            for (int j = 0; j < 8; ++j) {
                const float x1 = (float)k1[j], x2 = (float)k2[j];
                o1[j] = (f16_t)(x1 * c[j] + x2 * s[j]);
                o2[j] = (f16_t)(x2 * c[j] - x1 * s[j]);
            }
            *reinterpret_cast<f16x8*>(stage_w + so) = o1;
            *reinterpret_cast<f16x8*>(stage_w + so + 32) = o2;
// ... 41 lines not shown
    h->n_tokens = n - delta;
    return RCA_OK;
}
extern "C" int rca_lm_kv_read(rca_lm_t* h, int32_t layer, int32_t pos0, int32_t n_pos, uint16_t* k_host, uint16_t* v_host) {
    if (!h) return fail(RCA_ERR_ARG, "null");
    const rca_lm_config_t& c = h->cfg;
    if (layer < 0 || layer >= c.n_layers) return fail(RCA_ERR_ARG, "kv_read: layer %d outside [0, %d)", layer, c.n_layers);
    if (pos0 < 0 || n_pos < 0 || pos0 > c.n_ctx - n_pos) return fail(RCA_ERR_ARG, "kv_read: positions [%d, %d + %d) outside the context of %d", pos0, pos0, n_pos, c.n_ctx);
    RCA_HIP(hipSetDevice(h->device));
    RCA_HIP(hipStreamSynchronize(h->stream));
    h->async_pending = false;
    const long off = (long)layer * h->kv_layer_stride + (long)pos0 * c.n_kv_heads * 64;
    const size_t bytes = (size_t)n_pos * c.n_kv_heads * 64 * sizeof(f16_t);
    if (k_host && bytes) RCA_HIP(hipMemcpy(k_host, h->kc + off, bytes, hipMemcpyDeviceToHost));
    if (v_host && bytes) RCA_HIP(hipMemcpy(v_host, h->vc + off, bytes, hipMemcpyDeviceToHost));
    return RCA_OK;
}
extern "C" int rca_lm_set_low_priority(rca_lm_t* h, int32_t enable) {
    if (!h) return fail(RCA_ERR_ARG, "null");
    RCA_HIP(hipSetDevice(h->device));
    int lo = 0, hi = 0;
    RCA_HIP(hipDeviceGetStreamPriorityRange(&lo, &hi));
    hipStream_t ns = nullptr;
    RCA_HIP(hipStreamCreateWithPriority(&ns, hipStreamNonBlocking, enable ? lo : hi));
    RCA_HIP(hipStreamSynchronize(h->stream));
    h->async_pending = false;
    (void)hipStreamDestroy(h->stream);
    h->stream = ns;
    return RCA_OK;
}

extern "C" int rca_lm_logits_dev(rca_lm_t* h, const float** out) {
    if (!h || !out) return fail(RCA_ERR_ARG, "null");
    if (h->logits_rows < 1) return fail(RCA_ERR_STATE, "no logits: call eval first");
    *out = h->logits + (long)(h->logits_rows - 1) * h->cfg.vocab_size;
    return RCA_OK;
}
extern "C" int rca_lm_get_logits(rca_lm_t* h, float* out_host) {
    if (!h || !out_host) return fail(RCA_ERR_ARG, "null");
    { const int src = lm_settle(h); if (src != RCA_OK) return src; }
    const float* src;
    int rc;
    if ((rc = rca_lm_logits_dev(h, &src)) != RCA_OK) return rc;
    RCA_HIP(hipSetDevice(h->device));
    RCA_HIP(hipMemcpyAsync(out_host, src, (size_t)h->cfg.vocab_size * 4, hipMemcpyDeviceToHost, h->stream));
    RCA_HIP(hipStreamSynchronize(h->stream));
    return RCA_OK;
}
extern "C" int rca_lm_get_logits_row(rca_lm_t* h, int32_t row, float* out_host) {
    if (!h || !out_host) return fail(RCA_ERR_ARG, "null");
    { const int src = lm_settle(h); if (src != RCA_OK) return src; }
    if (row < 0 || row >= h->logits_rows) return fail(RCA_ERR_ARG, "row %d outside the %d rows of the last eval", row, h->logits_rows);
    RCA_HIP(hipSetDevice(h->device));
    RCA_HIP(hipMemcpyAsync(out_host, h->logits + (long)row * h->cfg.vocab_size, (size_t)h->cfg.vocab_size * 4, hipMemcpyDeviceToHost, h->stream));
    RCA_HIP(hipStreamSynchronize(h->stream));
    return RCA_OK;
}

extern "C" int rca_lm_sampler_init(rca_lm_t* h, const rca_sampler_params_t* p) {
    if (!h || !p) return fail(RCA_ERR_ARG, "null");
    if (p->n_bias < 0 || p->n_bias > 8) return fail(RCA_ERR_ARG, "at most 8 logit-bias entries");
    const int V = h->cfg.vocab_size;
    if (!(p->repeat_penalty > 0.0f) && p->repeat_penalty != 0.0f) return fail(RCA_ERR_ARG, "sampler: repeat_penalty %g must be positive", (double)p->repeat_penalty);
    const float rep = p->repeat_penalty == 0.0f ? 1.0f : p->repeat_penalty;
    const bool stoch = p->temp > 0.0f;
    const bool full = stoch && (p->top_k <= 0 || p->top_k > SAMP_MAXK);
    const bool big_k = full && p->top_k > SAMP_MAXK && p->top_k < V;
    const bool big_p = full && p->top_p < 1.0f;
    const bool pen = rep != 1.0f || p->freq_penalty != 0.0f || p->presence_penalty != 0.0f;
    const bool patch = p->n_bias > 0 || pen;
    RCA_HIP(hipSetDevice(h->device));
    SamplerDev s;
    memset(&s, 0, sizeof(s));
    s.top_k = p->top_k; s.top_p = p->top_p; s.min_p = p->min_p; s.temp = p->temp; s.seed = p->seed; s.n_bias = p->n_bias;
    for (int i = 0; i < p->n_bias; ++i) { s.bias_ids[i] = p->bias_ids[i]; s.bias_vals[i] = p->bias_vals[i]; }
    s.repeat_penalty = rep; s.freq_penalty = p->freq_penalty; s.presence_penalty = p->presence_penalty;
    s.last_n = p->penalty_last_n > 0 ? std::min(p->penalty_last_n, 64) : (p->penalty_last_n == 0 ? 64 : 0);
    s.patch = patch ? 1 : 0; s.big_k = big_k ? p->top_k : 0; s.big_p = big_p ? 1 : 0;
    RCA_HIP(hipStreamSynchronize(h->stream));
    RCA_HIP(hipMemcpy(h->samp, &s, sizeof(s), hipMemcpyHostToDevice));
    const unsigned long long zero = 0;
    RCA_HIP(hipMemcpy(&h->stt->rng_counter, &zero, 8, hipMemcpyHostToDevice));
    h->rng_host = 0;
    h->sampler_set = true;
    if (full != h->samp_full || patch != h->samp_patch || big_k != h->samp_big_k || big_p != h->samp_big_p)
        lm_drop_graphs(h);
    h->samp_full = full; h->samp_patch = patch; h->samp_big_k = big_k; h->samp_big_p = big_p;
    return RCA_OK;
}

static void lm_enqueue_sample(rca_lm* h, float* lg, hipStream_t st, int frame_i = -1) {
    const int V = h->cfg.vocab_size;
    const SampTail tail{frame_i, h->embed, h->embed_f32, h->x, h->cfg.hidden};
    if (h->samp_patch) samp_prepare_kernel<<<1, 128, 0, st>>>(lg, V, h->samp, h->stt, h->swork);
    if (h->samp_full) {
        samp_full_max_kernel<<<SAMPF_SLICES, 1024, 0, st>>>(lg, V, h->samp, h->swork);
        if (h->samp_big_k || h->samp_big_p) {
            for (int m = 0; m < 2; ++m) {
                if (!(m == 0 ? h->samp_big_k : h->samp_big_p)) continue;
                for (int l = 0; l < SAMP_LEVELS; ++l) samp_radix_pass_kernel<<<128, 256, 0, st>>>(lg, V, h->samp, h->swork, m, l);
                samp_radix_finish_kernel<<<1, 256, 0, st>>>(h->samp, h->swork, m);
            }
            samp_big_pick_kernel<<<SAMPF_SLICES, 1024, 0, st>>>(lg, V, h->samp, h->stt, h->swork);
        } else {
            samp_full_pick_kernel<<<SAMPF_SLICES, 1024, 0, st>>>(lg, V, h->samp, h->stt, h->swork);
        }
        samp_full_final_kernel<<<1, 1024, 0, st>>>(lg, V, h->samp, h->stt, h->swork, tail);
        return;
    }
    samp_hist_kernel<<<128, 256, 0, st>>>(lg, V, h->samp, h->swork);
    samp_gather_kernel<<<128, 256, 0, st>>>(lg, V, h->samp, h->swork);
    samp_final_kernel<<<1, 1024, 0, st>>>(lg, V, h->samp, h->stt, h->swork, tail);
}

static int lm_fetch_token(rca_lm* h, int32_t* token, hipStream_t st) {
    RCA_HIP(hipMemcpyAsync(&h->h_stt->out_token, &h->stt->out_token, 4, hipMemcpyDeviceToHost, st));
    RCA_HIP(hipStreamSynchronize(st));
    *token = h->h_stt->out_token;
    return RCA_OK;
}

extern "C" int rca_lm_sample(rca_lm_t* h, int32_t* token) {
    if (!h || !token) return fail(RCA_ERR_ARG, "null");
    { const int src = lm_settle(h); if (src != RCA_OK) return src; }
    if (!h->sampler_set) return fail(RCA_ERR_STATE, "sampler not initialised");
    if (h->logits_rows < 1) return fail(RCA_ERR_STATE, "no logits: call eval first");
    RCA_HIP(hipSetDevice(h->device));
    float* lg = h->logits + (long)(h->logits_rows - 1) * h->cfg.vocab_size;
    lm_enqueue_sample(h, lg, h->stream);
    RCA_LAUNCH_CHECK();
    h->rng_host += 1;
    return lm_fetch_token(h, token, h->stream);
}

static int lm_step_impl(rca_lm_t* h, const int32_t* ids, int32_t n, const int32_t* probe_ids, int32_t n_probe, int32_t* token, float* probs_out,
                        int cap_bucket = -1) {
    if (!h || !ids || !token || n < 1) return fail(RCA_ERR_ARG, "step: bad argument");
    if (n_probe < 0 || n_probe > 8 || (n_probe > 0 && (!probe_ids || !probs_out))) return fail(RCA_ERR_ARG, "step: 0..8 probe ids");
    { const int src = lm_settle(h); if (src != RCA_OK) return src; }
    if (!h->sampler_set) return fail(RCA_ERR_STATE, "sampler not initialised");
    if (h->n_tokens + n > h->cfg.n_ctx) return fail(RCA_ERR_STATE, "context overflow: %d + %d > n_ctx %d", h->n_tokens, n, h->cfg.n_ctx);
    for (int i = 0; i < n; ++i)
        if (ids[i] < 0 || ids[i] >= h->cfg.vocab_size) return fail(RCA_ERR_ARG, "step: token id %d at index %d is outside the vocabulary [0, %d)", ids[i], i, h->cfg.vocab_size);
    for (int i = 0; i < n_probe; ++i)
        if (probe_ids[i] < 0 || probe_ids[i] >= h->cfg.vocab_size) return fail(RCA_ERR_ARG, "step: probe id %d is outside the vocabulary", probe_ids[i]);
    RCA_HIP(hipSetDevice(h->device));
    hipStream_t st = h->stream;
    int rc;
    if (n > 2 || h->cfg.logits_all || !h->graphs_enabled) {
        if ((rc = rca_lm_eval(h, ids, n)) != RCA_OK) return rc;
        if ((rc = rca_lm_sample(h, token)) != RCA_OK) return rc;
        return n_probe ? rca_lm_token_probs(h, probe_ids, n_probe, probs_out) : RCA_OK;
    }
    lm_stage_state(h, ids, n);
    for (int i = 0; i < n_probe; ++i) h->h_probe[i] = probe_ids[i];
    const LmBucket bk = lm_bucket(h, n, cap_bucket);
    rca_lm::GraphSet& gs = lm_graph_set(h);
    hipGraphExec_t& gexec = n_probe ? gs.gp[n][bk.bucket] : gs.g[n][bk.bucket];
    if (n_probe && gexec && gs.gp_nprobe[n][bk.bucket] != n_probe) { (void)hipGraphExecDestroy(gexec); gexec = nullptr; }
    if (!gexec) {
        rc = lm_capture(st, &gexec, "step", [&]() -> int {
            hipError_t e = hipMemcpyAsync(h->stt, h->h_stt, LM_STATE_DECODE_BYTES, hipMemcpyHostToDevice, st);
            if (e == hipSuccess && n_probe) e = hipMemcpyAsync(h->probe_ids_dev, h->h_probe, n_probe * 4, hipMemcpyHostToDevice, st);
            if (e != hipSuccess) return fail(RCA_ERR_HIP, "capture memcpy: %s", hipGetErrorString(e));
            const int r = lm_enqueue_pass(h, n, 1, st, bk.nsp_launch);
            if (r != RCA_OK) return r;
            lm_enqueue_sample(h, h->logits, st);
            if (n_probe) {
                lm_softmax_slices_kernel<<<PROBS_SLICES, 1024, 0, st>>>(h->logits, h->cfg.vocab_size, h->probs_dev + 64);
                lm_token_probs_kernel<<<1, 64, 0, st>>>(h->logits, h->cfg.vocab_size, h->probs_dev + 64, h->probe_ids_dev, n_probe, h->probs_dev);
            }
            e = hipMemcpyAsync(&h->h_stt->out_token, &h->stt->out_token, 4, hipMemcpyDeviceToHost, st);
            if (e == hipSuccess && n_probe) e = hipMemcpyAsync(h->h_probe + 64, h->probs_dev, n_probe * 4, hipMemcpyDeviceToHost, st);
            return e == hipSuccess ? RCA_OK : fail(RCA_ERR_HIP, "capture d2h: %s", hipGetErrorString(e));
        });
        if (rc != RCA_OK) return rc;
        if (n_probe) gs.gp_nprobe[n][bk.bucket] = n_probe;
    }
    if (cap_bucket >= 0) return RCA_OK;
    RCA_HIP(hipGraphLaunch(gexec, st));
    RCA_HIP(hipStreamSynchronize(st));
    h->n_tokens += n;
    h->logits_rows = 1;
    h->rng_host += 1;
    *token = h->h_stt->out_token;
    for (int i = 0; i < n_probe; ++i) probs_out[i] = reinterpret_cast<const float*>(h->h_probe + 64)[i];
    return RCA_OK;
}
static int lm_step_capture_only(rca_lm_t* h, int n, int n_probe, int bucket) {
    if (h->cfg.logits_all || !h->graphs_enabled || n > 2) return RCA_OK;
    const int32_t ids[2] = {0, 0}, probes[8] = {0, 0, 0, 0, 0, 0, 0, 0};
    int32_t tok = 0;
    float pr[8];
    return lm_step_impl(h, ids, n, n_probe ? probes : nullptr, n_probe, &tok, n_probe ? pr : nullptr, bucket);
}
extern "C" int rca_lm_step(rca_lm_t* h, const int32_t* ids, int32_t n, int32_t* token) {
    return lm_step_impl(h, ids, n, nullptr, 0, token, nullptr);
}
extern "C" int rca_lm_step_probe(rca_lm_t* h, const int32_t* ids, int32_t n, const int32_t* probe_ids, int32_t n_probe, int32_t* token, float* probs_out) {
    if (n_probe < 1) return fail(RCA_ERR_ARG, "step_probe: 1..8 probe ids");
    return lm_step_impl(h, ids, n, probe_ids, n_probe, token, probs_out);
}

static int lm_frame_core(rca_lm_t* h, const int32_t* first_pair, const int32_t* user_ids, int32_t n_steps, int32_t audio_id_floor,
                         int32_t* out_tokens, int32_t* n_done, int cap_bucket) {
    if (!h || !first_pair || !user_ids || !out_tokens || !n_done) return fail(RCA_ERR_ARG, "frame: null argument");
    if (n_steps < 1 || n_steps > LM_FRAME_MAX) return fail(RCA_ERR_ARG, "frame: %d steps (1..%d)", n_steps, LM_FRAME_MAX);
    if (!h->sampler_set) return fail(RCA_ERR_STATE, "sampler not initialised");
    if (h->cfg.logits_all) return fail(RCA_ERR_STATE, "frame: not on a logits_all handle");
    if (cap_bucket < 0 && h->n_tokens + 2 * n_steps > h->cfg.n_ctx) return fail(RCA_ERR_STATE, "context overflow: %d + %d > n_ctx %d", h->n_tokens, 2 * n_steps, h->cfg.n_ctx);
    for (int i = 0; i < 2; ++i)
        if (first_pair[i] < 0 || first_pair[i] >= h->cfg.vocab_size) return fail(RCA_ERR_ARG, "frame: token id %d outside the vocabulary", first_pair[i]);
    for (int i = 0; i < n_steps; ++i)
        if (user_ids[i] < 0 || user_ids[i] >= h->cfg.vocab_size) return fail(RCA_ERR_ARG, "frame: token id %d outside the vocabulary", user_ids[i]);
    { const int src = lm_settle(h); if (src != RCA_OK) return src; }
    RCA_HIP(hipSetDevice(h->device));
    hipStream_t st = h->stream;
    int rc = RCA_OK;
    lm_stage_state(h, first_pair, 2);
    for (int i = 0; i < n_steps; ++i) h->h_stt->ids[LM_FRAME_USER0 + i] = user_ids[i];
    const LmBucket bk = lm_bucket(h, 2 * n_steps, cap_bucket);
    hipGraphExec_t& gexec = lm_graph_set(h).fg[n_steps][bk.bucket];
    if (cap_bucket >= 0 && (gexec || !h->graphs_enabled)) return RCA_OK;
    auto enqueue = [&]() -> int {
        hipError_t e = hipMemcpyAsync(h->stt, h->h_stt, LM_STATE_DECODE_BYTES, hipMemcpyHostToDevice, st);
        if (e != hipSuccess) return fail(RCA_ERR_HIP, "frame memcpy: %s", hipGetErrorString(e));
        for (int i = 0; i < n_steps; ++i) {
            const int r = lm_enqueue_pass(h, 2, 1, st, bk.nsp_launch, i > 0);
            if (r != RCA_OK) return r;
            lm_enqueue_sample(h, h->logits, st, i);
        }
        e = hipMemcpyAsync(h->h_stt->frame_out, h->stt->frame_out, sizeof(int) * LM_FRAME_MAX, hipMemcpyDeviceToHost, st);
        return e == hipSuccess ? RCA_OK : fail(RCA_ERR_HIP, "frame d2h: %s", hipGetErrorString(e));
    };
    if (!h->graphs_enabled) {
        RCA_HIP(hipStreamSynchronize(st));
        if ((rc = enqueue()) != RCA_OK) return rc;
    } else if (!gexec && (rc = lm_capture(st, &gexec, "frame", enqueue)) != RCA_OK) {
        return rc;
    }
    if (cap_bucket >= 0) return RCA_OK;
    if (h->graphs_enabled) RCA_HIP(hipGraphLaunch(gexec, st));
    RCA_HIP(hipStreamSynchronize(st));
    int done = n_steps;
    for (int i = 0; i < n_steps; ++i) {
        out_tokens[i] = h->h_stt->frame_out[i];
        if (out_tokens[i] <= audio_id_floor) { done = i + 1; break; }
    }
    *n_done = done;
    h->n_tokens += 2 * done;
    h->logits_rows = done < n_steps ? 0 : 1;
    h->rng_host += (unsigned long long)done;
    if (done < n_steps) {
        RCA_HIP(hipMemcpy(&h->stt->rng_counter, &h->rng_host, 8, hipMemcpyHostToDevice));
    }
    return RCA_OK;
}

extern "C" int rca_lm_frame(rca_lm_t* h, const int32_t* first_pair, const int32_t* user_ids, int32_t n_steps, int32_t audio_id_floor,
                            int32_t* out_tokens, int32_t* n_done) {
    return lm_frame_core(h, first_pair, user_ids, n_steps, audio_id_floor, out_tokens, n_done, -1);
}

struct DuplexDev {
    long long user_codes[LM_FRAME_MAX];
    float probe_prob;
    int flags;
    int probe_id;
    int pad;
};
struct DuplexPin {
    int probe_id;
    int pad0[3];
    long long user_codes[LM_FRAME_MAX];
    float probe_prob;
    int flags;
    int frame_out[LM_FRAME_MAX];
};
__global__ void duplex_codes_to_ids_kernel(const long long* __restrict__ codes, int n, int base, LmDevState* stt, int* flags) {
    if (threadIdx.x == 0) *flags = 0;
    if ((int)threadIdx.x < n) stt->ids[LM_FRAME_USER0 + threadIdx.x] = base + (int)codes[threadIdx.x];
}
__global__ void duplex_tokens_to_codes_kernel(const LmDevState* __restrict__ stt, int n, int base, int n_codes, long long* __restrict__ dst,
                                              int* flags) {
    if ((int)threadIdx.x < n) {
        const int c = stt->frame_out[threadIdx.x] - base;
        const bool ok = c >= 0 && c < n_codes;
        dst[threadIdx.x] = ok ? c : 0;
        if (!ok) atomicOr(flags, 1);
    }
}
struct DuplexGraphKey {
    int T, F_ctx, n_steps, n_samples, probe, bucket, base;
    const void* kc;
    unsigned long long codec_sig;
    const void* codec;
    bool operator==(const DuplexGraphKey& o) const {
        return T == o.T && F_ctx == o.F_ctx && n_steps == o.n_steps && n_samples == o.n_samples && probe == o.probe && bucket == o.bucket &&
               base == o.base && kc == o.kc && codec_sig == o.codec_sig && codec == o.codec;
    }
};
struct DuplexState {
    float* pcm_in = nullptr; size_t pcm_in_cap = 0;
    long long* code_win = nullptr; size_t code_win_cap = 0;
    float* pcm_out = nullptr; size_t pcm_out_cap = 0;
    DuplexDev* dev = nullptr;
    char* pin = nullptr; size_t pin_cap = 0;
    struct Entry { DuplexGraphKey key; hipGraphExec_t exec = nullptr; };
    std::vector<Entry> graphs;
    struct Warm { int T, F_ctx, n_steps, n_samples; const void* codec; unsigned long long codec_sig; };
    std::vector<Warm> warm;
    const void* logits_at_capture = nullptr;
    hipStream_t side = nullptr;
    hipEvent_t ev_fork = nullptr, ev_join = nullptr;
    bool fork = true;
};
static void duplex_drop_graphs(DuplexState* d) {
    if (!d) return;
    for (auto& e : d->graphs)
        if (e.exec) (void)hipGraphExecDestroy(e.exec);
    d->graphs.clear();
}
static void duplex_destroy(DuplexState* d) {
    if (!d) return;
    duplex_drop_graphs(d);
    for (void* p : {(void*)d->pcm_in, (void*)d->code_win, (void*)d->pcm_out, (void*)d->dev})
        if (p) (void)hipFree(p);
    if (d->pin) (void)hipHostFree(d->pin);
    if (d->side) (void)hipStreamDestroy(d->side);
    if (d->ev_fork) (void)hipEventDestroy(d->ev_fork);
    if (d->ev_join) (void)hipEventDestroy(d->ev_join);
    delete d;
}
template <class T>
static int duplex_grow(T** p, size_t* cap, size_t n) {
    if (n <= *cap) return RCA_OK;
    if (*p) { (void)hipFree(*p); *p = nullptr; *cap = 0; }
    int rc = lm_alloc((void**)p, n * sizeof(T));
    if (rc == RCA_OK) *cap = n;
    return rc;
}

struct DuplexPinLayout {
    size_t pcm, codes, out, total;
    DuplexPinLayout(int T, int F_ctx, int n_samples)
        : pcm(sizeof(DuplexPin)), codes(pcm + (((size_t)T * 4 + 255) & ~(size_t)255)), out(codes + (((size_t)F_ctx * 8 + 255) & ~(size_t)255)),
          total(out + (size_t)n_samples * 4) {}
};
static int duplex_reserve(rca_lm* h, int T, int F_ctx, int n, int n_samples) {
    int rc;
    hipStream_t st = h->stream;
    if (!h->duplex) {
        h->duplex = new DuplexState();
        const char* nf = getenv("RCA_DUPLEX_FORK");
        h->duplex->fork = !(nf && nf[0] == '0');
        RCA_HIP(hipStreamCreateWithFlags(&h->duplex->side, hipStreamNonBlocking));
        RCA_HIP(hipEventCreateWithFlags(&h->duplex->ev_fork, hipEventDisableTiming));
        RCA_HIP(hipEventCreateWithFlags(&h->duplex->ev_join, hipEventDisableTiming));
    }
    DuplexState* d = h->duplex;
    const int F = F_ctx + n;
    const size_t pin_total = DuplexPinLayout(T, F_ctx, n_samples).total;
    if ((size_t)T > d->pcm_in_cap || (size_t)F > d->code_win_cap || (size_t)n_samples > d->pcm_out_cap || pin_total > d->pin_cap || !d->dev) {
        RCA_HIP(hipStreamSynchronize(st));
        duplex_drop_graphs(d);
        if ((rc = duplex_grow(&d->pcm_in, &d->pcm_in_cap, (size_t)T)) != RCA_OK) return rc;
        if ((rc = duplex_grow(&d->code_win, &d->code_win_cap, (size_t)F + 8)) != RCA_OK) return rc;
        if ((rc = duplex_grow(&d->pcm_out, &d->pcm_out_cap, (size_t)n_samples)) != RCA_OK) return rc;
        if (!d->dev && (rc = lm_alloc((void**)&d->dev, sizeof(DuplexDev))) != RCA_OK) return rc;
        if (pin_total > d->pin_cap) {
            if (d->pin) (void)hipHostFree(d->pin);
            d->pin = nullptr; d->pin_cap = 0;
            RCA_HIP(hipHostMalloc((void**)&d->pin, pin_total + (pin_total >> 2), hipHostMallocDefault));
            d->pin_cap = pin_total + (pin_total >> 2);
        }
    }
    return RCA_OK;
}
extern "C" int rca_duplex_prepare(rca_lm_t* h, int32_t T, int32_t F_ctx, int32_t n_steps, int32_t n_samples) {
    if (!h || T < 1 || F_ctx < 0 || n_steps < 1 || n_steps > LM_FRAME_MAX || n_samples < 1) return fail(RCA_ERR_ARG, "duplex_prepare: bad shape");
    { const int src = lm_settle(h); if (src != RCA_OK) return src; }
    RCA_HIP(hipSetDevice(h->device));
    return duplex_reserve(h, T, F_ctx, n_steps, n_samples);
}

static int duplex_mark_warm(DuplexState* d, DuplexState::Entry* ent, const rca_duplex_frame_args_t* a, rca_codec_t* codec) {
    uint64_t sig = 0;
    const int rc = rca_codec_workspace_sig(codec, &sig);
    if (rc != RCA_OK) return rc;
    if (d->warm.size() >= 16) d->warm.clear();
    d->warm.push_back(DuplexState::Warm{a->T, a->F_ctx, a->n_steps, a->n_samples, (const void*)codec, sig});
    ent->key.codec_sig = sig;
    return RCA_OK;
}

static int duplex_frame_core(rca_lm_t* h, rca_codec_t* codec, const rca_duplex_frame_args_t* a, rca_duplex_frame_out_t* out,
                             float* pcm_out_host, int cap_bucket) {
    const bool cap_only = cap_bucket >= 0;
    if (!h || !codec || !a || (!cap_only && (!out || !pcm_out_host || !a->pcm_window || (a->F_ctx > 0 && !a->code_ctx)))) return fail(RCA_ERR_ARG, "duplex_frame: null argument");
    const int n = a->n_steps;
    if (n < 1 || n > LM_FRAME_MAX) return fail(RCA_ERR_ARG, "duplex_frame: %d steps (1..%d)", n, LM_FRAME_MAX);
    if (a->T < 1 || a->F_ctx < 0 || a->n_samples < 1) return fail(RCA_ERR_ARG, "duplex_frame: bad shape (T=%d F_ctx=%d n_samples=%d)", a->T, a->F_ctx, a->n_samples);
    if (!h->sampler_set) return fail(RCA_ERR_STATE, "sampler not initialised");
    if (h->cfg.logits_all) return fail(RCA_ERR_STATE, "duplex_frame: not on a logits_all handle");
    if (!cap_only && h->n_tokens + 2 * n > h->cfg.n_ctx) return fail(RCA_ERR_STATE, "context overflow: %d + %d > n_ctx %d", h->n_tokens, 2 * n, h->cfg.n_ctx);
    int32_t n_codes = 0;
    int rc;
    if ((rc = rca_codec_codebook_size(codec, &n_codes)) != RCA_OK) return rc;
    if (a->code_token_base < 0 || (long)a->code_token_base + n_codes > h->cfg.vocab_size) return fail(RCA_ERR_ARG, "duplex_frame: codes [%d, %d + %d) fall outside the vocabulary", a->code_token_base, a->code_token_base, n_codes);
    for (int i = 0; i < 2; ++i)
        if (a->first_pair[i] < 0 || a->first_pair[i] >= h->cfg.vocab_size) return fail(RCA_ERR_ARG, "duplex_frame: token id %d outside the vocabulary", a->first_pair[i]);
    if (a->probe_id >= h->cfg.vocab_size) return fail(RCA_ERR_ARG, "duplex_frame: probe id %d outside the vocabulary", a->probe_id);
    for (int i = 0; !cap_only && i < a->F_ctx; ++i)
        if (a->code_ctx[i] < 0 || a->code_ctx[i] >= n_codes) return fail(RCA_ERR_ARG, "decode: code out of range [0, %d)", n_codes);
    { const int src = lm_settle(h); if (src != RCA_OK) return src; }
    RCA_HIP(hipSetDevice(h->device));
    hipStream_t st = h->stream;
    if ((rc = duplex_reserve(h, a->T, a->F_ctx, n, a->n_samples)) != RCA_OK) return rc;
    DuplexState* d = h->duplex;
    const int F = a->F_ctx + n;
    const DuplexPinLayout lay(a->T, a->F_ctx, a->n_samples);
    if (d->logits_at_capture != (const void*)h->logits) { duplex_drop_graphs(d); d->logits_at_capture = h->logits; }
    DuplexPin* pin = reinterpret_cast<DuplexPin*>(d->pin);
    lm_stage_state(h, a->first_pair, 2);
    for (int i = 0; i < n; ++i) h->h_stt->ids[LM_FRAME_USER0 + i] = 0;
    pin->probe_id = a->probe_id >= 0 ? a->probe_id : 0;
    if (!cap_only) {
        memcpy(d->pin + lay.pcm, a->pcm_window, (size_t)a->T * 4);
        if (a->F_ctx) memcpy(d->pin + lay.codes, a->code_ctx, (size_t)a->F_ctx * 8);
    }
    const LmBucket bk = lm_bucket(h, 2 * n, cap_bucket);
    uint64_t csig = 0;
    if ((rc = rca_codec_workspace_sig(codec, &csig)) != RCA_OK) return rc;
    DuplexGraphKey key{a->T, a->F_ctx, n, a->n_samples, a->probe_id >= 0 ? 1 : 0, bk.bucket, a->code_token_base, (const void*)h->kc, csig, (const void*)codec};
    DuplexState::Entry* ent = nullptr;
    for (auto& e : d->graphs)
        if (e.key == key) ent = &e;
    if (!ent) {
        if (d->graphs.size() >= 32) { RCA_HIP(hipStreamSynchronize(st)); duplex_drop_graphs(d); }
        d->graphs.push_back(DuplexState::Entry{key, nullptr});
        ent = &d->graphs.back();
    }
    bool warmed = false;
    for (auto& w : d->warm)
        warmed = warmed || (w.T == a->T && w.F_ctx == a->F_ctx && w.n_steps == n && w.n_samples == a->n_samples && w.codec == (const void*)codec && w.codec_sig == csig);
    auto enqueue = [&]() -> int {
        hipError_t e = hipMemcpyAsync(h->stt, h->h_stt, LM_STATE_DECODE_BYTES, hipMemcpyHostToDevice, st);
        if (e == hipSuccess) e = hipMemcpyAsync(d->pcm_in, d->pin + lay.pcm, (size_t)a->T * 4, hipMemcpyHostToDevice, st);
        if (e == hipSuccess && a->F_ctx) e = hipMemcpyAsync(d->code_win, d->pin + lay.codes, (size_t)a->F_ctx * 8, hipMemcpyHostToDevice, st);
        if (e == hipSuccess) e = hipMemcpyAsync(&d->dev->probe_id, &pin->probe_id, 4, hipMemcpyHostToDevice, st);
        if (e != hipSuccess) return fail(RCA_ERR_HIP, "duplex h2d: %s", hipGetErrorString(e));
        hipStream_t se = d->fork ? d->side : st;
        if (d->fork) {
            e = hipEventRecord(d->ev_fork, st);
            if (e == hipSuccess) e = hipStreamWaitEvent(se, d->ev_fork, 0);
            if (e != hipSuccess) return fail(RCA_ERR_HIP, "duplex fork: %s", hipGetErrorString(e));
        }
        int r = rca_codec_encode_tail_dev(codec, d->pcm_in, 1, a->T, n, (int64_t*)d->dev->user_codes, se);
        if (r != RCA_OK) return r;
        duplex_codes_to_ids_kernel<<<1, 64, 0, se>>>(d->dev->user_codes, n, a->code_token_base, h->stt, &d->dev->flags);
        if (d->fork) {
            e = hipEventRecord(d->ev_join, se);
            if (e != hipSuccess) return fail(RCA_ERR_HIP, "duplex join: %s", hipGetErrorString(e));
        }
        for (int i = 0; i < n; ++i) {
            if ((r = lm_enqueue_pass(h, 2, 1, st, bk.nsp_launch, i > 0)) != RCA_OK) return r;
            if (i == 0 && d->fork) {
                e = hipStreamWaitEvent(st, d->ev_join, 0);
                if (e != hipSuccess) return fail(RCA_ERR_HIP, "duplex join: %s", hipGetErrorString(e));
            }
            lm_enqueue_sample(h, h->logits, st, i);
        }
        duplex_tokens_to_codes_kernel<<<1, 64, 0, st>>>(h->stt, n, a->code_token_base, n_codes, d->code_win + a->F_ctx, &d->dev->flags);
        if ((r = rca_codec_decode_tail_dev(codec, (const int64_t*)d->code_win, 1, F, a->n_samples, d->pcm_out, st)) != RCA_OK) return r;
        if (a->probe_id >= 0) {
            lm_softmax_slices_kernel<<<PROBS_SLICES, 1024, 0, st>>>(h->logits, h->cfg.vocab_size, h->probs_dev + 64);
            lm_token_probs_kernel<<<1, 64, 0, st>>>(h->logits, h->cfg.vocab_size, h->probs_dev + 64, &d->dev->probe_id, 1, &d->dev->probe_prob);
        }
        RCA_LAUNCH_CHECK();
        e = hipMemcpyAsync(pin->frame_out, h->stt->frame_out, sizeof(int) * LM_FRAME_MAX, hipMemcpyDeviceToHost, st);
        if (e == hipSuccess) e = hipMemcpyAsync(pin->user_codes, d->dev->user_codes, sizeof(long long) * LM_FRAME_MAX + 8, hipMemcpyDeviceToHost, st);
        if (e == hipSuccess) e = hipMemcpyAsync(d->pin + lay.out, d->pcm_out, (size_t)a->n_samples * 4, hipMemcpyDeviceToHost, st);
        if (e != hipSuccess) return fail(RCA_ERR_HIP, "duplex d2h: %s", hipGetErrorString(e));
        return RCA_OK;
    };
    if ((rc = rca_codec_stream_handoff(codec, d->fork ? d->side : st)) != RCA_OK) return rc;
    if (cap_only && !warmed) {
        hipStream_t se = d->fork ? d->side : st;
        RCA_HIP(hipMemsetAsync(d->pcm_in, 0, (size_t)a->T * 4, se));
        RCA_HIP(hipMemsetAsync(d->code_win, 0, (size_t)F * 8, se));
        if ((rc = rca_codec_encode_tail_dev(codec, d->pcm_in, 1, a->T, n, (int64_t*)d->dev->user_codes, se)) != RCA_OK) return rc;
        if ((rc = rca_codec_decode_tail_dev(codec, (const int64_t*)d->code_win, 1, F, a->n_samples, d->pcm_out, se)) != RCA_OK) return rc;
        RCA_HIP(hipStreamSynchronize(se));
        if ((rc = duplex_mark_warm(d, ent, a, codec)) != RCA_OK) return rc;
        warmed = true;
    }
    const bool want_graph = h->graphs_enabled && warmed;
    if (want_graph && !ent->exec && (rc = lm_capture(st, &ent->exec, "duplex", enqueue)) != RCA_OK) return rc;
    if (cap_only) return RCA_OK;
    if (want_graph) {
        RCA_HIP(hipGraphLaunch(ent->exec, st));
    } else if ((rc = enqueue()) != RCA_OK) {
        return rc;
    }
    RCA_HIP(hipStreamSynchronize(st));
    if (!warmed && (rc = duplex_mark_warm(d, ent, a, codec)) != RCA_OK) return rc;
    int done = n;
    for (int i = 0; i < n; ++i) {
        out->tokens[i] = pin->frame_out[i];
        out->user_codes[i] = pin->user_codes[i];
        if (out->tokens[i] <= a->audio_id_floor) { done = i + 1; break; }
    }
    for (int i = done; i < n; ++i) { out->tokens[i] = -1; out->user_codes[i] = pin->user_codes[i]; }
    out->n_done = done;
    out->flags = pin->flags | (done < n ? 2 : 0);
    out->probe_prob = (a->probe_id >= 0 && done == n) ? pin->probe_prob : -1.0f;
    if (out->flags == 0) memcpy(pcm_out_host, d->pin + lay.out, (size_t)a->n_samples * 4);
    h->n_tokens += 2 * done;
    h->logits_rows = done < n ? 0 : 1;
    h->rng_host += (unsigned long long)done;
    if (done < n) RCA_HIP(hipMemcpy(&h->stt->rng_counter, &h->rng_host, 8, hipMemcpyHostToDevice));
    return RCA_OK;
}

extern "C" int rca_duplex_frame(rca_lm_t* h, rca_codec_t* codec, const rca_duplex_frame_args_t* a, rca_duplex_frame_out_t* out,
                                float* pcm_out_host) {
    return duplex_frame_core(h, codec, a, out, pcm_out_host, -1);
}

static int lm_step_capture_only(rca_lm_t* h, int n, int n_probe, int bucket);

extern "C" int rca_duplex_precapture(rca_lm_t* h, rca_lm_t* twin, rca_codec_t* codec, const rca_duplex_frame_args_t* a, int32_t n_probe) {
    if (!h || !codec || !a) return fail(RCA_ERR_ARG, "duplex_precapture: null argument");
    if (!h->sampler_set) return fail(RCA_ERR_STATE, "sampler not initialised");
    if (!h->graphs_enabled) return RCA_OK;
    if (twin && (twin == h || twin->cfg.n_ctx != h->cfg.n_ctx || twin->n_splits != h->n_splits)) return fail(RCA_ERR_ARG, "duplex_precapture: the twin must be another handle of the same n_ctx");
    { const int src = lm_settle(h); if (src != RCA_OK) return src; }
    if (twin) { const int src = lm_settle(twin); if (src != RCA_OK) return src; }
    int rc = RCA_OK;
    for (int pass = 0; pass < (twin ? 2 : 1) && rc == RCA_OK; ++pass) {
        if (pass == 1) { std::swap(h->kc, twin->kc); std::swap(h->vc, twin->vc); }
        for (int b = 0; b < LM_GRAPH_BUCKETS && rc == RCA_OK; ++b) {
            if (!lm_bucket_reachable(h, b)) break;
            rc = duplex_frame_core(h, codec, a, nullptr, nullptr, b);
            if (rc == RCA_OK && n_probe > 0) rc = lm_step_capture_only(h, 1, n_probe, b);
            if (rc == RCA_OK) {
                const int32_t pair[2] = {0, 0}, users[LM_FRAME_MAX] = {0, 0, 0, 0, 0, 0, 0, 0};
                int32_t toks[LM_FRAME_MAX], done = 0;
                rc = lm_frame_core(h, pair, users, a->n_steps, -1, toks, &done, b);
            }
            if (rc == RCA_OK) rc = lm_step_capture_only(h, 2, 0, b);
        }
        if (pass == 1) { std::swap(h->kc, twin->kc); std::swap(h->vc, twin->vc); }
    }
    return rc;
}

extern "C" int rca_lm_token_probs(rca_lm_t* h, const int32_t* token_ids, int32_t n, float* probs_out) {
    if (!h || !token_ids || !probs_out || n < 1 || n > 64) return fail(RCA_ERR_ARG, "token_probs: 1..64 ids");
    { const int src = lm_settle(h); if (src != RCA_OK) return src; }
    if (h->logits_rows < 1) return fail(RCA_ERR_STATE, "no logits: call eval first");
    RCA_HIP(hipSetDevice(h->device));
    hipStream_t st = h->stream;
    RCA_HIP(hipMemcpyAsync(h->probe_ids_dev, token_ids, n * 4, hipMemcpyHostToDevice, st));
    const float* lg = h->logits + (long)(h->logits_rows - 1) * h->cfg.vocab_size;
    lm_softmax_slices_kernel<<<PROBS_SLICES, 1024, 0, st>>>(lg, h->cfg.vocab_size, h->probs_dev + 64);
    lm_token_probs_kernel<<<1, 64, 0, st>>>(lg, h->cfg.vocab_size, h->probs_dev + 64, h->probe_ids_dev, n, h->probs_dev);
    RCA_LAUNCH_CHECK();
    RCA_HIP(hipMemcpyAsync(probs_out, h->probs_dev, n * 4, hipMemcpyDeviceToHost, st));
    RCA_HIP(hipStreamSynchronize(st));
    return RCA_OK;
}

extern "C" int rca_lm_set_logits_all(rca_lm_t* h, int32_t enable) {
    if (!h) return fail(RCA_ERR_ARG, "null");
    if ((h->cfg.logits_all != 0) != (enable != 0)) {
        RCA_HIP(hipSetDevice(h->device));
        RCA_HIP(hipStreamSynchronize(h->stream));
        lm_drop_graphs(h);
    }
    h->cfg.logits_all = enable != 0;
    return RCA_OK;
}

extern "C" int rca_lm_set_graphs(rca_lm_t* h, int32_t enable) {
    if (!h) return fail(RCA_ERR_ARG, "null");
    h->graphs_enabled = enable != 0;
    return RCA_OK;
}

__global__ __launch_bounds__(256) void lm_q8_zero_row_scales_kernel(unsigned* __restrict__ sc, int nblk, int row_begin, int row_end) {
    const long total = (long)(row_end - row_begin) * nblk;
    for (long i = (long)blockIdx.x * blockDim.x + threadIdx.x; i < total; i += (long)gridDim.x * blockDim.x) {
        const int row = row_begin + (int)(i / nblk), j = (int)(i % nblk);
        unsigned short* half = reinterpret_cast<unsigned short*>(sc + q8_sc_index(row >> 1, j, nblk)) + (row & 1);
        *half = 0;
    }
}
__global__ __launch_bounds__(256) void lm_q6k_zero_row_scales_kernel(float* __restrict__ sc, int nk16, int row_begin, int row_end) {
    const long total = (long)(row_end - row_begin) * nk16;
    for (long i = (long)blockIdx.x * blockDim.x + threadIdx.x; i < total; i += (long)gridDim.x * blockDim.x) {
        const int row = row_begin + (int)(i / nk16), j = (int)(i % nk16);
        sc[2 * q8_sc_index(row >> 1, j, nk16) + (row & 1)] = 0.0f;
    }
}
__global__ __launch_bounds__(256) void lm_q4k_zero_row_factors_kernel(unsigned* __restrict__ dd, int nk256, int row_begin, int row_end) {
    const long total = (long)(row_end - row_begin) * nk256;
    for (long i = (long)blockIdx.x * blockDim.x + threadIdx.x; i < total; i += (long)gridDim.x * blockDim.x) {
        const int row = row_begin + (int)(i / nk256), j = (int)(i % nk256);
        dd[q4k_scm_index(row, j, nk256)] = 0u;
    }
}
__global__ __launch_bounds__(256) void lm_zero_rows_kernel(bf16_t* __restrict__ w, long n) {
    for (long i = (long)blockIdx.x * blockDim.x + threadIdx.x; i < n; i += (long)gridDim.x * blockDim.x) w[i] = 0;
}
extern "C" int rca_lm_mask_head_rows(rca_lm_t* h, int32_t row_begin, int32_t row_end) {
    if (!h || row_begin < 0 || row_end > h->cfg.vocab_size || row_begin > row_end) return fail(RCA_ERR_ARG, "mask_head_rows: bad range");
    RCA_HIP(hipSetDevice(h->device));
    const long n = (long)(row_end - row_begin) * h->cfg.hidden;
    if (n > 0 && h->head.fmt == WF_Q6K)
        lm_q6k_zero_row_scales_kernel<<<256, 256, 0, h->stream>>>((float*)h->head.sc, h->cfg.hidden / 16, row_begin, row_end);
    if (n > 0 && (h->head.fmt == WF_Q4K || h->head.fmt == WF_Q5K))
        lm_q4k_zero_row_factors_kernel<<<256, 256, 0, h->stream>>>(h->head.dd, h->cfg.hidden / 256, row_begin, row_end);
    if (n > 0 && (h->head.fmt == WF_Q40 || h->head.fmt == WF_Q41))
        lm_q4k_zero_row_factors_kernel<<<256, 256, 0, h->stream>>>(h->head.sc, h->cfg.hidden / 32, row_begin, row_end);
    if (n > 0 && (h->head.fmt == WF_BF16 || h->head.fmt == WF_F16)) lm_zero_rows_kernel<<<2048, 256, 0, h->stream>>>(h->head.w + (long)row_begin * h->cfg.hidden, n);
    if (n > 0 && h->head.fmt == WF_Q8)
// ... 42 lines not shown
            if (f32tab) reinterpret_cast<float*>(table_rows)[(long)n * H + f] = v;
            else reinterpret_cast<bf16_t*>(table_rows)[(long)n * H + f] = f32_to_bf16_rne(v);
            if (out_f32) out_f32[(long)n * H + f] = v;
        }
    }
}

extern "C" int rca_lm_persist_codec_embeddings(rca_lm_t* h, const float* codec_embed, int32_t n_codes, int32_t dim, const float* w1,
                                               const float* b1, const float* w2, const float* b2, int32_t codec_vocab_start, float* out_f32) {
    if (!h || !codec_embed || !w1 || !b1 || !w2 || !b2) return fail(RCA_ERR_ARG, "persist_codec_embeddings: null argument");
    const int H = h->cfg.hidden;
    if (n_codes <= 0 || dim <= 0 || codec_vocab_start < 0 || (long)codec_vocab_start + n_codes > h->cfg.vocab_size)
        return fail(RCA_ERR_ARG, "persist_codec_embeddings: rows [%d, %ld) are outside the vocabulary of %d", codec_vocab_start,
                    (long)codec_vocab_start + n_codes, h->cfg.vocab_size);
    if (H % 8) return fail(RCA_ERR_ARG, "persist_codec_embeddings: hidden size must be a multiple of 8");
    RCA_HIP(hipSetDevice(h->device));
    const int chunk = std::min<int>(n_codes, 8192);
    float *de = nullptr, *dw1 = nullptr, *db1 = nullptr, *dw2 = nullptr, *db2 = nullptr, *dh1 = nullptr, *dout = nullptr;
    auto free_all = [&]() { for (float* p : {de, dw1, db1, dw2, db2, dh1, dout}) if (p) (void)hipFree(p); };
    auto up = [&](float** d, const float* src, size_t n) {
        if (hipMalloc((void**)d, n * 4) != hipSuccess) return false;
        return hipMemcpy(*d, src, n * 4, hipMemcpyHostToDevice) == hipSuccess;
    };
    if (!up(&de, codec_embed, (size_t)n_codes * dim) || !up(&dw1, w1, (size_t)H * dim) || !up(&db1, b1, H) || !up(&dw2, w2, (size_t)H * H) ||
        !up(&db2, b2, H) || hipMalloc((void**)&dh1, (size_t)chunk * H * 4) != hipSuccess ||
        (out_f32 && hipMalloc((void**)&dout, (size_t)chunk * H * 4) != hipSuccess)) {
        free_all();
        return fail(RCA_ERR_HIP, "persist_codec_embeddings: device allocation / upload failed");
    }
    for (int r0 = 0; r0 < n_codes; r0 += chunk) {
        const int rows = std::min(chunk, n_codes - r0);
        lm_codec_proj1_kernel<<<(unsigned)(((long)rows * H + 255) / 256), 256, 0, h->stream>>>(de + (long)r0 * dim, dw1, db1, dh1, rows, dim, H);
        lm_codec_proj2_kernel<<<dim3((H + 127) / 128, (rows + 31) / 32), 256, 0, h->stream>>>(
            dh1, dw2, db2, (char*)h->embed + ((long)codec_vocab_start + r0) * H * (h->embed_f32 ? 4 : 2), h->embed_f32, dout, rows, H);
        hipError_t e = hipGetLastError();
        if (e == hipSuccess && out_f32) e = hipMemcpyAsync(out_f32 + (long)r0 * H, dout, (size_t)rows * H * 4, hipMemcpyDeviceToHost, h->stream);
        if (e == hipSuccess) e = hipStreamSynchronize(h->stream);
        if (e != hipSuccess) { free_all(); return fail(RCA_ERR_HIP, "persist_codec_embeddings: %s", hipGetErrorString(e)); }
    }
    free_all();
    return RCA_OK;
}

extern "C" int rca_lm_set_attn_fuse(rca_lm_t* h, int32_t enable) {
    if (!h) return fail(RCA_ERR_ARG, "null");
    { const int src = lm_settle(h); if (src != RCA_OK) return src; }
    RCA_HIP(hipSetDevice(h->device));
    RCA_HIP(hipStreamSynchronize(h->stream));
    if (h->fuse_attn != (enable != 0)) lm_drop_graphs(h);
    h->fuse_attn = enable != 0;
    return RCA_OK;
}
static bool lm_has_packed_matrix(const rca_lm* h) {
    auto packed = [](const WMat& m) { return wf_packed(m.fmt); };
    bool any = packed(h->head);
    for (const LmLayer& L : h->layers) any = any || packed(L.qkv) || packed(L.o) || packed(L.gu) || packed(L.down) || (L.split_v && packed(L.vseg));
    return any;
}
extern "C" int rca_lm_set_act_format(rca_lm_t* h, int32_t fmt) {
    if (!h) return fail(RCA_ERR_ARG, "null");
    if (fmt != 0 && fmt != 1) return fail(RCA_ERR_ARG, "set_act_format: %d is neither 0 (f32) nor 1 (q8_1)", fmt);
    if (fmt == 1 && !lm_has_packed_matrix(h))
        return fail(RCA_ERR_ARG, "set_act_format: q8_1 activations need a q8_0 / Q4_K / Q6_K, Q5_K or Q4_0 / Q4_1 projection matrix, and this handle keeps all of its matrices in 16-bit floats");
    { const int src = lm_settle(h); if (src != RCA_OK) return src; }
    if (h->act_format != fmt) {
        RCA_HIP(hipSetDevice(h->device));
        RCA_HIP(hipStreamSynchronize(h->stream));
        lm_drop_graphs(h);
    }
    h->act_format = fmt;
    return RCA_OK;
}
extern "C" int rca_lm_get_act_format(const rca_lm_t* h, int32_t* fmt) {
    if (!h || !fmt) return fail(RCA_ERR_ARG, "null");
    *fmt = h->act_format;
    return RCA_OK;
}
extern "C" int rca_lm_gemv_tap(rca_lm_t* h, int32_t layer, int32_t kind, const float* x_host, int32_t M, float* y_host, int64_t y_numel,
                               uint16_t* kv_host) {
    if (!h || !x_host || !y_host) return fail(RCA_ERR_ARG, "null");
    const rca_lm_config_t& c = h->cfg;
    const int H = c.hidden, QKV = (c.n_heads + 2 * c.n_kv_heads) * c.head_dim, AO = c.n_heads * c.head_dim, F = c.ffn, V = c.vocab_size;
    if (kind < 0 || kind > 4) return fail(RCA_ERR_ARG, "gemv_tap: kind %d outside [0, 4]", kind);
    if (M < 1 || M > LM_GEMV_M) return fail(RCA_ERR_ARG, "gemv_tap: M = %d, a decode pass has 1 or %d tokens", M, LM_GEMV_M);
    if (kind != 4 && (layer < 0 || layer >= c.n_layers)) return fail(RCA_ERR_ARG, "gemv_tap: layer %d outside [0, %d)", layer, c.n_layers);
    if (h->n_tokens + M > c.n_ctx) return fail(RCA_ERR_STATE, "gemv_tap: positions %d .. %d are outside the context of %d", h->n_tokens, h->n_tokens + M - 1, c.n_ctx);
    const int in_w[5] = {H, AO, H, F, H}, out_w[5] = {AO, H, F, H, V};
    if (y_numel != (int64_t)M * out_w[kind]) return fail(RCA_ERR_ARG, "gemv_tap: y_numel %ld, kind %d writes %d x %d values", (long)y_numel, kind, M, out_w[kind]);
    { const int src = lm_settle(h); if (src != RCA_OK) return src; }
    RCA_HIP(hipSetDevice(h->device));
    hipStream_t st = h->stream;
    RCA_HIP(hipStreamSynchronize(st));
    const int32_t ids[LM_GEMV_M] = {};
    int rc;
    if ((rc = lm_push_state(h, ids, M, st)) != RCA_OK) return rc;
    float* xin = kind == 1 ? h->attn : (kind == 3 ? h->hbuf : h->x);
    RCA_HIP(hipMemcpyAsync(xin, x_host, (size_t)M * in_w[kind] * 4, hipMemcpyHostToDevice, st));
    const float* yd = nullptr;
    int ldy = out_w[kind];
    float* head_out = nullptr;
    if (kind == 0) {
        lm_launch_qkv(h, layer, M, st);
        yd = h->qkv; ldy = QKV;
    } else if (kind == 1) {
        RCA_HIP(hipMemsetAsync(h->x, 0, (size_t)M * H * 4, st));
        lm_launch_o(h, layer, M, st);
        yd = h->x;
    } else if (kind == 2) {
        lm_launch_gu(h, layer, M, st);
        yd = h->hbuf;
    } else if (kind == 3) {
        RCA_HIP(hipMemsetAsync(h->x, 0, (size_t)M * H * 4, st));
        lm_launch_down(h, layer, M, st);
        yd = h->x;
    } else {
        if ((rc = lm_alloc((void**)&head_out, (size_t)M * V * 4)) != RCA_OK) return rc;
        lm_launch_head(h, M, st, head_out, false);
        yd = head_out;
    }
    hipError_t e = hipGetLastError();
    if (e == hipSuccess) e = hipMemcpy2DAsync(y_host, (size_t)out_w[kind] * 4, yd, (size_t)ldy * 4, (size_t)out_w[kind] * 4, M, hipMemcpyDeviceToHost, st);
    if (e == hipSuccess && kind == 0 && kv_host) {
        const size_t n = (size_t)M * c.n_kv_heads * 64;
        const long off = (long)layer * h->kv_layer_stride + (long)h->n_tokens * c.n_kv_heads * 64;
        e = hipMemcpyAsync(kv_host, h->kc + off, n * 2, hipMemcpyDeviceToHost, st);
        if (e == hipSuccess) e = hipMemcpyAsync(kv_host + n, h->vc + off, n * 2, hipMemcpyDeviceToHost, st);
    }
    if (e == hipSuccess) e = hipStreamSynchronize(st);
    if (head_out) (void)hipFree(head_out);
    if (e != hipSuccess) return fail(RCA_ERR_HIP, "gemv_tap: %s", hipGetErrorString(e));
    return RCA_OK;
}

extern "C" int rca_lm_weight_format(const rca_lm_t* h, int32_t* fmt, int64_t* bytes_per_step) {
    if (!h || !fmt) return fail(RCA_ERR_ARG, "null");
    *fmt = h->layers.empty() ? h->head.fmt : h->layers[0].gu.fmt;
    if (bytes_per_step) {
        long b = h->head.stream_bytes();
        for (const LmLayer& L : h->layers) b += L.qkv.stream_bytes() + L.o.stream_bytes() + L.gu.stream_bytes() + L.down.stream_bytes() + (L.split_v ? L.vseg.stream_bytes() : 0);
        *bytes_per_step = b;
    }
    return RCA_OK;
}

extern "C" int rca_lm_prefill_route(const rca_lm_t* h, int32_t* route) {
    if (!h || !route) return fail(RCA_ERR_ARG, "null");
    *route = lm_prefill_route(h);
    return RCA_OK;
}

extern "C" int rca_lm_set_mfma_prefill(rca_lm_t* h, int32_t enable) {
    if (!h) return fail(RCA_ERR_ARG, "null");
    h->mfma_prefill = enable != 0;
    return RCA_OK;
}
```

realtime_codec_agent_amd/llm.py:

```python
from __future__ import annotations

import ctypes as C
import json
import math
import os
from dataclasses import asdict, dataclass
from typing import Dict, Generator, List, Optional, Sequence

import numpy as np

from . import _native as N


@dataclass
class LMConfig:
    vocab_size: int = 259344
    hidden: int = 2048
    n_layers: int = 16
    n_heads: int = 32
    n_kv_heads: int = 8
    head_dim: int = 64
    ffn: int = 8192
    rms_eps: float = 1e-5
    rope_theta: float = 500000.0
# ... 357 lines not shown
        top_k: int = 40,
        top_p: float = 0.95,
        min_p: float = 0.05,
        typical_p: float = 1.0,
        temp: float = 0.80,
        repeat_penalty: float = 1.0,
        frequency_penalty: float = 0.0,
        presence_penalty: float = 0.0,
        tfs_z: float = 1.0,
        mirostat_mode: int = 0,
        mirostat_tau: float = 5.0,
        mirostat_eta: float = 0.1,
        penalize_nl: bool = True,
        logits_processor=None,
        grammar=None,
        seed: Optional[int] = None,
        logit_bias: Optional[Dict[int, float]] = None,
    ) -> None:
        if typical_p != 1.0 or mirostat_mode != 0 or grammar is not None:
            raise NotImplementedError("typical_p / mirostat / grammar samplers are not implemented (the duplex agent never sets them)")
        self.set_seed(seed if seed is not None else -1)
        bias = dict(logit_bias or {})
        if logits_processor is not None:
            lb = getattr(logits_processor, "logit_bias_map", None)
            if lb is None:
                raise NotImplementedError("logits_processor must come from get_logits_bias_processor")
            bias.update(lb)
        ids = (C.c_int32 * max(1, len(bias)))(*bias.keys())
        vals = (C.c_float * max(1, len(bias)))(*bias.values())
        p = N.SamplerParamsC(top_k=int(top_k), top_p=float(top_p), min_p=float(min_p), temp=float(temp), seed=self._seed,
                             n_bias=len(bias), bias_ids=ids, bias_vals=vals, repeat_penalty=float(repeat_penalty),
                             freq_penalty=float(frequency_penalty), presence_penalty=float(presence_penalty),
                             penalty_last_n=int(getattr(self, "last_n_tokens_size", 64)))
        N.check(self._lib.rca_lm_sampler_init(self._h, C.byref(p)), "rca_lm_sampler_init")
        self._sampler = True
        self._sampler_params = dict(top_k=top_k, top_p=top_p, min_p=min_p, temp=temp, seed=self._seed, logit_bias=bias,
                                    repeat_penalty=repeat_penalty, frequency_penalty=frequency_penalty, presence_penalty=presence_penalty)

    def sample(self, idx: Optional[int] = None) -> int:
        assert self.n_tokens > 0
        assert self._sampler is not None
        tok = C.c_int32()
        N.check(self._lib.rca_lm_sample(self._h, C.byref(tok)), "rca_lm_sample")
        return tok.value

    def step(self, tokens: Sequence[int]) -> int:
        tokens = list(tokens)
        n0 = self.n_tokens
        arr = (C.c_int32 * len(tokens))(*tokens)
        tok = C.c_int32()
        N.check(self._lib.rca_lm_step(self._h, arr, len(tokens), C.byref(tok)), "rca_lm_step")
        self._input_ids[n0:n0 + len(tokens)] = tokens
        self._logits_valid = False
        return tok.value

    def step_probe(self, tokens: Sequence[int], probe_ids: Sequence[int]):
        tokens, probe_ids = list(tokens), list(probe_ids)
        n0 = self.n_tokens
        arr = (C.c_int32 * len(tokens))(*tokens)
        pid = (C.c_int32 * len(probe_ids))(*probe_ids)
        out = (C.c_float * len(probe_ids))()
        tok = C.c_int32()
        N.check(self._lib.rca_lm_step_probe(self._h, arr, len(tokens), pid, len(probe_ids), C.byref(tok), out), "rca_lm_step_probe")
        self._input_ids[n0:n0 + len(tokens)] = tokens
        self._logits_valid = False
        return tok.value, np.array(out[:], dtype=np.float32)

    def frame(self, first_pair: Sequence[int], user_ids: Sequence[int], audio_id_floor: int) -> List[int]:
        first_pair, user_ids = [int(t) for t in first_pair], [int(t) for t in user_ids]
        if len(first_pair) != 2:
            raise ValueError("frame() starts from the last [agent, user] pair")
        n, n0 = len(user_ids), self.n_tokens
        fp = (C.c_int32 * 2)(*first_pair)
        us = (C.c_int32 * n)(*user_ids)
        out = (C.c_int32 * n)()
        done = C.c_int32()
        N.check(self._lib.rca_lm_frame(self._h, fp, us, n, int(audio_id_floor), out, C.byref(done)), "rca_lm_frame")
        toks = list(out[:done.value])
        evaluated = first_pair + [t for pair in zip(toks[:-1], user_ids) for t in pair]
        self._input_ids[n0:n0 + len(evaluated)] = evaluated
        self._logits_valid = False
        return toks

    def duplex_prepare(self, T: int, F_ctx: int, n_steps: int, n_samples: int) -> None:
        N.check(self._lib.rca_duplex_prepare(self._h, int(T), int(F_ctx), int(n_steps), int(n_samples)), "rca_duplex_prepare")

    def duplex_precapture(self, codec_handle, T: int, F_ctx: int, n_steps: int, n_samples: int, code_token_base: int, with_probe: bool,
                          twin: Optional["LlamaForAlternatingCodeChannels"] = None, n_step_probe: int = 0) -> None:
        a = N.DuplexFrameArgsC(pcm_window=None, code_ctx=None, T=int(T), F_ctx=int(F_ctx), n_steps=int(n_steps), n_samples=int(n_samples),
                               code_token_base=int(code_token_base), audio_id_floor=-1, probe_id=0 if with_probe else -1)
        N.check(self._lib.rca_duplex_precapture(self._h, twin._h if twin is not None else None, codec_handle._h, C.byref(a), int(n_step_probe)),
                "rca_duplex_precapture")

    def duplex_frame(self, codec_handle, pcm_window: np.ndarray, code_ctx: np.ndarray, n_steps: int, n_samples: int,
                     code_token_base: int, audio_id_floor: int, probe_id: int, first_pair: Sequence[int]) -> dict:
        first_pair = [int(t) for t in first_pair]
        if len(first_pair) != 2:
            raise ValueError("duplex_frame() starts from the last [agent, user] pair")
        pcm_window = np.ascontiguousarray(pcm_window, dtype=np.float32).reshape(-1)
        code_ctx = np.ascontiguousarray(code_ctx, dtype=np.int64).reshape(-1)
        n0 = self.n_tokens
        a = N.DuplexFrameArgsC(pcm_window=pcm_window.ctypes.data, code_ctx=code_ctx.ctypes.data if code_ctx.size else None,
                               T=pcm_window.size, F_ctx=code_ctx.size, n_steps=int(n_steps), n_samples=int(n_samples),
                               code_token_base=int(code_token_base), audio_id_floor=int(audio_id_floor), probe_id=int(probe_id))
        a.first_pair[0], a.first_pair[1] = first_pair
        out = N.DuplexFrameOutC()
        pcm = np.empty(int(n_samples), dtype=np.float32)
        N.check(self._lib.rca_duplex_frame(self._h, codec_handle._h, C.byref(a), C.byref(out), C.c_void_p(pcm.ctypes.data)), "rca_duplex_frame")
        codes = [int(c) for c in out.user_codes[:n_steps]]
        toks = [int(t) for t in out.tokens[:out.n_done]]
        user_ids = [int(code_token_base) + c for c in codes]
        evaluated = first_pair + [t for pair in zip(toks[:-1], user_ids) for t in pair]
        self._input_ids[n0:n0 + len(evaluated)] = evaluated
        self._logits_valid = False
        return {"user_codes": codes, "tokens": toks, "pcm": pcm if out.flags == 0 else None,
                "probe_prob": float(out.probe_prob) if out.probe_prob >= 0.0 else None}

    def generate(self, tokens: Sequence[int], reset: bool = True, stopping_criteria=None) -> Generator[int, Optional[Sequence[int]], None]:
        tokens = list(tokens)
        if reset and self.n_tokens > 0:
            longest_prefix = 0
            for a, b in zip(self._input_ids[: self.n_tokens], tokens[:-1]):
                if a == b:
                    longest_prefix += 1
                else:
                    break
            if longest_prefix > 0:
                reset = False
                tokens = tokens[longest_prefix:]
                self.n_tokens = longest_prefix
        if reset:
            self.reset()
        while True:
            token = self.step(tokens)
            if stopping_criteria is not None and stopping_criteria(self._input_ids[: self.n_tokens], self._fetch_logits()):
                return
            tokens_or_none = yield token
            tokens = [token]
            if tokens_or_none is not None:
                tokens.extend(tokens_or_none)

    def token_probs(self, token_ids: Sequence[int]) -> np.ndarray:
        ids = (C.c_int32 * len(token_ids))(*token_ids)
        out = (C.c_float * len(token_ids))()
        N.check(self._lib.rca_lm_token_probs(self._h, ids, len(token_ids), out), "rca_lm_token_probs")
        return np.array(out[:], dtype=np.float32)

    def sync(self) -> None:
        N.check(self._lib.rca_lm_sync(self._h), "rca_lm_sync")

    def make_kv_shadow(self, low_priority: bool = True) -> "LlamaForAlternatingCodeChannels":
        twin = LlamaForAlternatingCodeChannels(model_path=self.model_path, n_ctx=self._n_ctx, share_weights_with=self, device=self._device)
        if low_priority:
            N.check(self._lib.rca_lm_set_low_priority(twin._h, 1), "rca_lm_set_low_priority")
        return twin

    def eval_async(self, tokens: Sequence[int]) -> None:
        tokens = list(tokens)
        if not tokens:
            return
        n0 = self.n_tokens
        arr = (C.c_int32 * len(tokens))(*tokens)
        N.check(self._lib.rca_lm_eval_async(self._h, arr, len(tokens)), "rca_lm_eval_async")
        self._input_ids[n0:n0 + len(tokens)] = tokens
        self._logits_valid = False

    def copy_kv_from(self, other: "LlamaForAlternatingCodeChannels", n_positions: int) -> None:
        N.check(self._lib.rca_lm_copy_kv(self._h, other._h, int(n_positions)), "rca_lm_copy_kv")
        self._input_ids[:n_positions] = other._input_ids[:n_positions]

    def swap_kv(self, other: "LlamaForAlternatingCodeChannels") -> None:
        N.check(self._lib.rca_lm_swap_kv(self._h, other._h), "rca_lm_swap_kv")
        n = max(self._n_ctx, other._n_ctx)
        tmp = self._input_ids[:n].copy()
        self._input_ids[:n] = other._input_ids[:n]
        other._input_ids[:n] = tmp
        self._logits_valid = other._logits_valid = False

    def kv_remove(self, p0: int, p1: int) -> None:
        p0, p1, n = int(p0), int(p1), self.n_tokens
        N.check(self._lib.rca_lm_kv_remove(self._h, p0, p1), "rca_lm_kv_remove")
        self._input_ids[p0:n - (p1 - p0)] = self._input_ids[p1:n].copy()

    def kv_read(self, layer: int, pos0: int, n_pos: int):
        k = np.empty((int(n_pos), self.config.n_kv_heads, 64), np.float16)
        v = np.empty_like(k)
        N.check(self._lib.rca_lm_kv_read(self._h, int(layer), int(pos0), int(n_pos), k.ctypes.data_as(C.POINTER(C.c_uint16)),
                                         v.ctypes.data_as(C.POINTER(C.c_uint16))), "rca_lm_kv_read")
        return k, v

    def mask_head_rows(self, row_begin: int, row_end: int) -> None:
        N.check(self._lib.rca_lm_mask_head_rows(self._h, int(row_begin), int(row_end)), "rca_lm_mask_head_rows")

    def persist_codec_embeddings(self, codec_state: Dict[str, np.ndarray], codec_vocab_start: int, codebook_size: Optional[int] = None,
                                 return_f32: bool = False) -> Optional[np.ndarray]:
        f32 = lambda a: np.ascontiguousarray(bf16_bits_to_f32(a) if a.dtype == np.uint16 else a, dtype=np.float32)
        embed = f32(codec_state["codec_embed.weight"])
        n_books = 1 + max(int(k.split(".")[1]) for k in codec_state if k.startswith("codebook_projectors."))
        size = codebook_size or embed.shape[0] // n_books
# ... 53 lines not shown
```

realtime_codec_agent_amd/realtime_agent_v2.py:

```python
from __future__ import annotations

import re
from typing import Any, Dict, List, Optional, Set, Tuple, Union
from warnings import warn

import numpy as np

from .realtime_agent_config import RealtimeAgentConfig
from .realtime_agent_profiler import RealtimeAgentProfilerCollection
from .realtime_agent_stats import RealtimeAgentStatsCollection
from .utils.audio_utils import create_crossfade_ramps, normalize_audio_rms, pad_or_trim, smooth_join

_TRANSCRIPT_RE = re.compile("([A-Z]):(.*?)(?= [A-Z]:|$)")
_CONSTRAINED_STOP_RE = re.compile(r"\A(?:[^ ]| [^&[]| &[^=]| &=.* | \[.*\] )")
_BACKCHANNELS = frozenset("yeah sure right okay well so and like you know uh huh um oh ah mm mmm hm hmm mhm mhmm".split())


def _softmax(x: np.ndarray) -> np.ndarray:
    e = np.exp(x - np.max(x))
    return e / e.sum()


def _make_fence(resources):
    fns = []
    llm = getattr(resources, "llm", None)
    if hasattr(llm, "sync"):
        fns.append(llm.sync)
    hip = getattr(getattr(getattr(resources, "audio_tokenizer", None), "codec_model", None), "hip", None)
    if hasattr(hip, "sync"):
        fns.append(hip.sync)
    if not fns:
        return None

    def fence():
        for f in fns:
            f()
    return fence


class RealtimeAgent:
    def __init__(self, resources=None, config: RealtimeAgentConfig = None, self_play_mode: bool = False, kv_trim_mode: str = "recompute"):
        if resources is None:
            from .realtime_agent_resources import RealtimeAgentResources
            resources = RealtimeAgentResources()
        self.resources = resources
        self.llm_client = None
        self.tts_client = None
        self.self_play_mode = self_play_mode
        self.transcript_regex = _TRANSCRIPT_RE
        self.constrained_text_gen_stop_regex = _CONSTRAINED_STOP_RE
        self.constrained_text_gen_wordlist = set(_BACKCHANNELS)
        self.use_frame_graph = True
        self.frame_graph_active = False
        self.use_duplex_graph = True
        self.duplex_graph_frames = 0
        self.use_kv_shadow = True
        self.precapture_graphs = True
        self.kv_shadow_tile = 128
        self._kv_shadow = None
        if kv_trim_mode not in ("recompute", "shift"):
            raise ValueError(f"kv_trim_mode {kv_trim_mode!r}: 'recompute' or 'shift'")
        self.kv_trim_mode = kv_trim_mode
        self.set_config(config if config is not None else RealtimeAgentConfig())
        self.reset()

    @property
    def total_frames(self) -> int:
        return len(self.audio_tokens_idx)

    @property
    def total_secs(self) -> float:
        return self.total_frames / (self.resources.audio_tokenizer.framerate * 2)

    @property
    def last_transcription(self) -> Optional[Dict[str, Any]]:
        return next((e for e in reversed(self.transcript) if e["speaker"] != self.config.agent_identity), None)

    @property
    def last_response(self) -> Optional[Dict[str, Any]]:
        return next((e for e in reversed(self.transcript) if e["speaker"] == self.config.agent_identity), None)

    def set_config(self, config: RealtimeAgentConfig):
        if config.use_external_llm or config.use_external_tts:
            raise NotImplementedError("external LLM / TTS services are outside this build's scope (SURVEY.md section 2 rows 10-11)")
        self.config = config
        tok, at = self.resources.tokenizer, self.resources.audio_tokenizer
        self.chunk_size_samples = int(config.chunk_size_secs * at.sampling_rate)
        self.chunk_size_frames_per_channel = int(config.chunk_size_secs * at.framerate)
        self.crossfade_ramps = create_crossfade_ramps(at.sampling_rate, fade_secs=config.chunk_fade_secs)
        self.end_header_token_id = tok.convert_tokens_to_ids(config.end_header_token)
        self.start_audio_token_id = tok.convert_tokens_to_ids(config.start_audio_token)
        self.end_audio_token_id = tok.convert_tokens_to_ids(config.end_audio_token)
        self.external_marker_token_id = tok.encode(config.external_marker_token, add_special_tokens=False)[0]
        self.agent_speaker_token_id = tok.encode(f" {config.agent_identity}", add_special_tokens=False)[0]
        self.user_speaker_token_id = tok.encode(f" {config.user_identity}", add_special_tokens=False)[0]
        self._code_token_base = None
        try:
            from .codec_chars import codes_to_chars
            probe = [0, 1, at.codebook_size // 3, at.codebook_size - 1]
            ids = tok.encode(codes_to_chars(np.asarray(probe), at.codebook_size, unicode_offset=at.unicode_offset), add_special_tokens=False)
            if len(ids) == len(probe) and all(i - c == ids[0] for i, c in zip(ids, probe)) and ids[0] > self.end_header_token_id:
                self._code_token_base = int(ids[0])
        except Exception:
            self._code_token_base = None
        self.stats = RealtimeAgentStatsCollection(config)
        self.profilers = RealtimeAgentProfilerCollection(config, sync=_make_fence(self.resources))

    def set_sampler(self, for_trans: bool = False, suppress_end_audio: bool = False) -> None:
        c = self.config
        processor = None
        if suppress_end_audio:
            from .llm import get_logits_bias_processor
            processor = get_logits_bias_processor({self.end_audio_token_id: -100})
        self.resources.llm.init_sampler_for_generate(
            top_k=c.top_k, top_p=c.top_p, min_p=c.min_p, temp=c.trans_temperature if for_trans else c.temperature,
            repeat_penalty=c.repeat_penalty, presence_penalty=c.presence_penalty, frequency_penalty=c.frequency_penalty,
            logits_processor=processor, seed=c.seed,
        )

    def reset(self):
        c, r = self.config, self.resources
        r.audio_tokenizer.reset_context()
        self.set_sampler()
        r.llm.reset()
        enrollment = np.zeros(r.audio_tokenizer.sampling_rate * 3, dtype=np.float32) if c.agent_voice_enrollment is None else c.agent_voice_enrollment
        enrollment_codes = r.audio_tokenizer.chunked_tokenize_audio(enrollment, c.chunk_size_secs)
        header = "".join([c.header_agent_token, c.header_speaker_token, f" {c.agent_identity}", c.header_speaker_token,
                          f" {c.user_identity}", c.header_agent_voice_token, enrollment_codes, c.end_header_token])
        self.context_start_pos = len(r.tokenizer.encode(header))
        prompt = header
        if c.agent_opening_text:
            prompt += f" {c.agent_identity}: {c.agent_opening_text}"
        prompt += c.start_audio_token
        self.input_ids: List[int] = r.tokenizer.encode(prompt)
        r.llm.eval(self.input_ids[:-1])

        self.trim_to_secs = 0.0
        self.ch1_inactivity_elapsed_secs = 0.0
# ... 286 lines not shown
        ratio = np.exp(aux.get_logprobs(af_ctx, txt_ids)) / np.exp(aux.get_logprobs(to_ctx, txt_ids))
        counter, i = 0, -1
        for i, rt in enumerate(ratio):
            counter = 0 if rt >= 1.0 else counter + 1
            if counter > c.finalize_response_improbable_token_tolerance:
                i -= counter
                break
        final_ids = txt_ids[:i + 1]
        if len(final_ids) == len(txt_ids):
            return
        if not final_ids:
            final_ids = tok.encode(" [silence]", add_special_tokens=False)
        last["text"] = tok.decode(final_ids, skip_special_tokens=False).lstrip()
        a = last["text_start_pos"] + 2
        b = a + len(txt_ids)
        before = len(self.input_ids)
        self.input_ids = self.input_ids[:a] + final_ids + self.input_ids[b:]
        self.recompute_kv_cache(a, b)
        diff = len(self.input_ids) - before
        if diff:
            for j in range(self.total_frames - 1, -1, -1):
                if self.audio_tokens_idx[j] <= b:
                    break
                self.audio_tokens_idx[j] += diff

    def _frame_tokens(self, audio_chunk_input_ids: List[int], forced: bool) -> Optional[List[int]]:
        llm = self.resources.llm
        n = len(audio_chunk_input_ids)
        if not hasattr(llm, "frame") or not self._frame_ready(n, forced):
            return None
        self.frame_graph_active = True
        return llm.frame(self.input_ids[-2:], audio_chunk_input_ids, self.end_header_token_id)

    def _frame_ready(self, n: int, forced: bool) -> bool:
        if not self.use_frame_graph or forced or n < 2 or n > 8:
            return False
        self.trim_sequences()
        if not self._in_audio_mode():
            return False
        per_sec = self.resources.audio_tokenizer.framerate * 2
        return not any((self.total_frames + 2 * i) / per_sec - self.trim_to_secs >= self.config.max_context_secs for i in range(1, n))

    def process_audio_input_ids(self, audio_chunk_input_ids: List[int], force_trans: bool = False, force_response: bool = False,
                                pre: Optional[List[int]] = None) -> List[int]:
        llm = self.resources.llm
        out = [0] * len(audio_chunk_input_ids)
        if pre is None:
            pre = self._frame_tokens(audio_chunk_input_ids, force_trans or force_response)
        for i, user_tok in enumerate(audio_chunk_input_ids):
            self.trim_sequences()
            suppress_end_audio = False
            first = True
            while True:
                audio_mode = self._in_audio_mode()
                if first and pre is not None and i < len(pre):
                    nxt = pre[i]
                elif audio_mode and (force_trans or force_response):
                    self.input_ids.append(self.end_audio_token_id)
                    llm.eval(self.input_ids[-3:])
                    nxt = self.user_speaker_token_id if force_trans else self.agent_speaker_token_id
                    force_trans = force_response = False
                else:
                    if suppress_end_audio:
                        self.set_sampler(suppress_end_audio=True)
                    nxt = self._next_token(self.input_ids[-(2 if audio_mode else 1):])
                    if suppress_end_audio:
                        self.set_sampler()
                        suppress_end_audio = False
                first = False
                self.input_ids.append(nxt)
                if nxt > self.end_header_token_id:
                    self.input_ids.append(user_tok)
                    n = len(self.input_ids)
                    self.audio_tokens_idx.extend([n - 2, n - 1])
                    out[i] = nxt
                    break
                if self.input_ids[-2] == self.end_audio_token_id:
                    if nxt != self.agent_speaker_token_id:
                        suppress_end_audio = not self.generate_for_trans()
                    else:
                        suppress_end_audio = not self.generate_for_response()
        return out

    def measure_event_prob(self, p_end: Optional[float] = None):
        llm = self.resources.llm
        if p_end is not None:
            pass
        elif hasattr(llm, "token_probs"):
            p_end = float(llm.token_probs([self.end_audio_token_id])[0])
        else:
            logits = np.ctypeslib.as_array(llm._ctx.get_logits(), shape=(llm._n_vocab,))
            p_end = float(_softmax(logits)[self.end_audio_token_id])
        self.stats.event_prob.add_value(p_end)
        self.prob_event_speaker_token_id = self.get_probable_event_speaker() if self.stats.event_prob.last_zscore >= 0.0 else None

    def get_probable_event_speaker(self) -> int:
        llm = self.resources.llm
        if hasattr(llm, "step_probe"):
            _, (pa, pu) = llm.step_probe([self.end_audio_token_id], [self.agent_speaker_token_id, self.user_speaker_token_id])
            llm.n_tokens -= 1
            return self.agent_speaker_token_id if pa > pu else self.user_speaker_token_id
        _ = self._next_token([self.end_audio_token_id])
        if hasattr(llm, "token_probs"):
            pa, pu = llm.token_probs([self.agent_speaker_token_id, self.user_speaker_token_id])
        else:
            probs = _softmax(np.ctypeslib.as_array(llm._ctx.get_logits(), shape=(llm._n_vocab,)))
            pa, pu = probs[[self.agent_speaker_token_id, self.user_speaker_token_id]]
        llm.n_tokens -= 1
        return self.agent_speaker_token_id if pa > pu else self.user_speaker_token_id

    def update_inactivity_timers(self) -> None:
        c = self.config
        prev_ch1 = self.ch1_inactivity_elapsed_secs
        prev_z2 = self.stats.ch_abs_max.last_zscore[1]
        self.stats.ch_abs_max.add_value((float(np.abs(self.audio_history_ch1[-1]).max()), float(np.abs(self.audio_history_ch2[-1]).max())))
        z1, z2 = self.stats.ch_abs_max.last_zscore
        if z2 >= 0.0:
            self.ch2_inactivity_elapsed_secs = 0.0
            if prev_z2 < 0.0:
                self.ch2_activity_start_secs = self.total_secs - c.chunk_size_secs
        else:
            self.ch2_inactivity_elapsed_secs += c.chunk_size_secs
        if z1 >= 0.0:
            self.ch1_inactivity_elapsed_secs = 0.0
        else:
            self.ch1_inactivity_elapsed_secs += c.chunk_size_secs
            if prev_ch1 < c.finalize_response_after_inactivity_secs <= self.ch1_inactivity_elapsed_secs:
                self.finalize_last_response()

    def should_force_transcription(self) -> bool:
        c = self.config
        if c.force_trans_after_inactivity_secs == 0.0:
            return False
        return (self.ch2_inactivity_elapsed_secs >= c.force_trans_after_inactivity_secs and self.stats.event_prob.last_zscore >= 1.0
                and self.prob_event_speaker_token_id == self.user_speaker_token_id)

    def should_force_response(self) -> bool:
        c = self.config
        if c.force_response_after_inactivity_secs == 0.0:
            return False
        return min(self.ch1_inactivity_elapsed_secs, self.ch2_inactivity_elapsed_secs) >= c.force_response_after_inactivity_secs

    def process_audio(self, audio_chunk: np.ndarray, audio_chunk_input_ids: Optional[List[int]] = None):
        p, r = self.profilers, self.resources
        with p.total_profiler:
            assert audio_chunk.shape[-1] == self.chunk_size_samples, \
                f"audio_chunk must have length {self.chunk_size_samples}, but got {audio_chunk.shape[-1]}"
            assert audio_chunk_input_ids is None or len(audio_chunk_input_ids) == self.chunk_size_frames_per_channel, \
                f"audio_chunk_input_ids must have length {self.chunk_size_frames_per_channel}, but got {len(audio_chunk_input_ids)}"
            self._settle_shadow()
            fused = self._one_replay_frame(audio_chunk) if audio_chunk_input_ids is None else None
            if fused is not None:
                self._advance_shadow()
                return fused if self.self_play_mode else fused[0]
            with p.audio_tokenize_profiler:
                if audio_chunk_input_ids is None:
                    audio_chunk_str = r.audio_tokenizer.tokenize_audio(audio_chunk)
            with p.tokenize_profiler:
                if audio_chunk_input_ids is None:
                    audio_chunk_input_ids = r.tokenizer.encode(audio_chunk_str, add_special_tokens=False)
            with p.lm_profiler:
                out_ids = self.process_audio_input_ids(audio_chunk_input_ids, self.should_force_transcription(), self.should_force_response())
            out_chunk = self.detokenize_output_chunk(out_ids)
            self.audio_history_ch2.append(audio_chunk)
            self.measure_event_prob()
            self.update_inactivity_timers()
            assert out_chunk.shape[-1] == self.chunk_size_samples, f"out_chunk must have length {self.chunk_size_samples}, but got {out_chunk.shape[-1]}"
            assert len(out_ids) == self.chunk_size_frames_per_channel
            self._advance_shadow()
        return (out_chunk, out_ids) if self.self_play_mode else out_chunk

    step = process_audio

    def _one_replay_frame(self, audio_chunk: np.ndarray):
        p, r = self.profilers, self.resources
        llm, at = r.llm, r.audio_tokenizer
        if not (self.use_duplex_graph and self.use_frame_graph and self._code_token_base is not None
                and hasattr(llm, "duplex_frame") and hasattr(at, "duplex_plan")):
            return None
        L = self.crossfade_ramps[0]
        plan = at.duplex_plan(audio_chunk, preroll_samples=L)
        if plan is None or plan["n_codes"] != self.chunk_size_frames_per_channel:
            return None
        if not self._frame_ready(plan["n_codes"], self.should_force_transcription() or self.should_force_response()):
            return None
        base = self._code_token_base
        for prof in (p.audio_tokenize_profiler, p.tokenize_profiler):
            with prof:
                pass
        with p.lm_profiler:
            res = llm.duplex_frame(at.codec_model.hip, plan["window"], plan["code_ctx"], plan["n_codes"], plan["n_samples"], base,
                                   self.end_header_token_id, self.end_audio_token_id, self.input_ids[-2:])
            at.duplex_commit_pcm(plan)
            self.frame_graph_active = True
            self.duplex_graph_frames += 1
            user_ids = [base + c for c in res["user_codes"]]
            out_ids = self.process_audio_input_ids(user_ids, pre=res["tokens"])
        if res["pcm"] is not None:
            with p.detokenize_profiler:
                out_str = r.tokenizer.decode(out_ids, skip_special_tokens=False)
            with p.audio_detokenize_profiler:
                (_, chunk), _, preroll = at.duplex_commit_codes(plan, out_str, res["pcm"])
            out_chunk = self._splice_output_chunk(chunk, preroll)
        else:
            out_chunk = self.detokenize_output_chunk(out_ids)
        self.audio_history_ch2.append(audio_chunk)
        self.measure_event_prob(res["probe_prob"] if res["pcm"] is not None else None)
        self.update_inactivity_timers()
        assert out_chunk.shape[-1] == self.chunk_size_samples and len(out_ids) == self.chunk_size_frames_per_channel
        return out_chunk, out_ids

    def detokenize_output_chunk(self, out_chunk_input_ids: List[int]) -> np.ndarray:
        p, r = self.profilers, self.resources
        L = self.crossfade_ramps[0]
        with p.detokenize_profiler:
            out_str = r.tokenizer.decode(out_chunk_input_ids, skip_special_tokens=False)
        with p.audio_detokenize_profiler:
            (_, chunk), _, preroll = r.audio_tokenizer.detokenize_audio(out_str, preroll_samples=L)
        return self._splice_output_chunk(chunk, preroll)

    def _splice_output_chunk(self, chunk: np.ndarray, preroll: int) -> np.ndarray:
        L = self.crossfade_ramps[0]
        chunk = pad_or_trim(chunk, self.chunk_size_samples + preroll)
        if self.config.target_volume_rms > 0:
            chunk = normalize_audio_rms(chunk, target_rms=self.config.target_volume_rms)
        if self.audio_history_ch1:
            joined = smooth_join(self.audio_history_ch1[-1], chunk, *self.crossfade_ramps)
            assert joined.shape[-1] == 2 * self.chunk_size_samples, f"joined chunks must have length {2 * self.chunk_size_samples}, but got {joined.shape[-1]}"
            self.audio_history_ch1[-1] = joined[:self.chunk_size_samples]
            self.audio_history_ch1.append(joined[self.chunk_size_samples:])
            return joined[-self.chunk_size_samples - L:-L]
        self.audio_history_ch1.append(chunk)
        return pad_or_trim(chunk[:-L], self.chunk_size_samples, pad_side="left")

    def get_sequence_str(self) -> str:
        return self.resources.tokenizer.decode(self.input_ids, skip_special_tokens=False)

    def get_audio_history(self) -> np.ndarray:
        if not self.audio_history_ch1:
            return np.zeros((2, 0), dtype=np.float32)
        return np.stack([np.concatenate(self.audio_history_ch1), np.concatenate(self.audio_history_ch2)], axis=0)

    @staticmethod
    def _fmt_time(secs: float) -> str:
        h, rem = divmod(secs, 3600)
        m, s = divmod(rem, 60)
        return f"{int(h)}:{int(m):02}:{s:06.3f}"

    def format_transcript(self) -> str:
        lines = []
        for e in self.transcript:
            if "planned_text" in e and e["text"] != e["planned_text"]:
                planned = e["planned_text"] if e["text"] == "[silence]" else e["planned_text"][len(e["text"]):].lstrip()
                body = f"{e['text']}  ⟶  {{{planned}}}"
            else:
                body = e["text_with_external_markers"]
            end = e["end_secs"] if e["end_secs"] is not None else self.total_secs
            lines.append(f"[{self._fmt_time(e['start_secs'])} - {self._fmt_time(end)}] {e['speaker']}: {body}")
        return "\n".join(lines)

    def get_external_llm_messages(self):
        return None


RealtimeAgentV2 = RealtimeAgent


from .realtime_agent_mp import RealtimeAgentMultiprocessing, RealtimeAgentMultiprocessingInfo, RealtimeAgentWorkerError
```

Measured before the change: 3432 audio-hours/hour.

## Fold speculative end-audio speaker probe into the duplex frame's last decode pass

Adds an M=3 GEMV path so the final frame decode pass also evaluates a speculative end_audio token and computes speaker-token probabilities inside the same captured graph. The agent can then commit or discard the speculative KV entry instead of running a separate step_probe when the event z-score fires. This targets the extra LM step and its launch and sync cost in the duplex loop. It adds a new graph family, M=3 GEMV instantiations, RNG-counter settling and extra KV/logit work on every frame. The primary batch-encode throughput path is untouched.

```diff
diff --git a/include/rca.h b/include/rca.h
--- a/include/rca.h
+++ b/include/rca.h
@@ -198,6 +198,21 @@
 int rca_codec_stream_handoff(rca_codec_t* h, void* stream);
 int rca_codec_codebook_size(const rca_codec_t* h, int32_t* n);
 int rca_lm_step_probe(rca_lm_t* h, const int32_t* ids, int32_t n, const int32_t* probe_ids, int32_t n_probe, int32_t* token, float* probs_out);
+typedef struct rca_spec_probe {
+    int32_t token;
+    int32_t n_ids;
+    int32_t ids[8];
+} rca_spec_probe_t;
+typedef struct rca_spec_result {
+    int32_t valid;
+    int32_t token;
+    float probs[8];
+} rca_spec_result_t;
+int rca_lm_frame_spec(rca_lm_t* h, const int32_t* first_pair, const int32_t* user_ids, int32_t n_steps, int32_t audio_id_floor,
+                      const rca_spec_probe_t* spec, int32_t* out_tokens, int32_t* n_done, rca_spec_result_t* spec_out);
+int rca_duplex_frame_spec(rca_lm_t* lm, rca_codec_t* codec, const rca_duplex_frame_args_t* args, const rca_spec_probe_t* spec,
+                          rca_duplex_frame_out_t* out, rca_spec_result_t* spec_out, float* pcm_out_host);
+int rca_lm_spec_commit(rca_lm_t* h, int32_t used);
 int rca_lm_token_probs(rca_lm_t* h, const int32_t* token_ids, int32_t n, float* probs_out);
 int rca_lm_mask_head_rows(rca_lm_t* h, int32_t row_begin, int32_t row_end);
 int rca_lm_persist_codec_embeddings(rca_lm_t* h, const float* codec_embed, int32_t n_codes, int32_t dim,
diff --git a/realtime_codec_agent_amd/_native.py b/realtime_codec_agent_amd/_native.py
--- a/realtime_codec_agent_amd/_native.py
+++ b/realtime_codec_agent_amd/_native.py
@@ -241,6 +241,22 @@
         ("n_done", C.c_int32),
         ("flags", C.c_int32),
         ("probe_prob", C.c_float),
+    ]
+
+
+class SpecProbeC(C.Structure):
+    _fields_ = [
+        ("token", C.c_int32),
+        ("n_ids", C.c_int32),
+        ("ids", C.c_int32 * 8),
+    ]
+
+
+class SpecResultC(C.Structure):
+    _fields_ = [
+        ("valid", C.c_int32),
+        ("token", C.c_int32),
+        ("probs", C.c_float * 8),
     ]
 
 
@@ -346,6 +362,7 @@
     "rca_lm_set_low_priority", "rca_lm_frame", "rca_lm_weight_format", "rca_lm_set_attn_fuse", "rca_lm_prefill_route",
     "rca_lm_set_act_format", "rca_lm_get_act_format", "rca_lm_gemv_tap", "rca_lm_kv_remove", "rca_lm_kv_read",
     "rca_duplex_frame", "rca_codec_workspace_sig", "rca_codec_stream_handoff", "rca_codec_codebook_size", "rca_codec_set_mfma_mode", "rca_lm_step_probe", "rca_duplex_prepare", "rca_duplex_precapture",
+    "rca_lm_frame_spec", "rca_duplex_frame_spec", "rca_lm_spec_commit",
 ]
 
 
diff --git a/realtime_codec_agent_amd/csrc/rca_lm.hip b/realtime_codec_agent_amd/csrc/rca_lm.hip
--- a/realtime_codec_agent_amd/csrc/rca_lm.hip
+++ b/realtime_codec_agent_amd/csrc/rca_lm.hip
@@ -15,7 +15,8 @@
 #define LM_MAXM 1024
 #define LM_STATE_DECODE_BYTES (8 + 4 * 16)
 #define LM_TILE32 32
-#define LM_GEMV_M 2
+#define LM_GEMV_M 3
+#define LM_EVAL_M 2
 #define LM_PREFILL_MIN 8
 #define LM_KSLICE 2048
 #define LM_MAXSPLIT 4
@@ -1877,6 +1878,7 @@
     bool samp_full = false;
     bool samp_patch = false, samp_big_k = false, samp_big_p = false;
     struct GraphSet { const f16_t* kc = nullptr; hipGraphExec_t g[3][LM_GRAPH_BUCKETS] = {}; hipGraphExec_t fg[LM_FRAME_MAX + 1][LM_GRAPH_BUCKETS] = {};
+                      hipGraphExec_t fgs[LM_FRAME_MAX + 1][LM_GRAPH_BUCKETS] = {}; int fgs_nprobe[LM_FRAME_MAX + 1][LM_GRAPH_BUCKETS] = {};
                       hipGraphExec_t gp[3][LM_GRAPH_BUCKETS] = {}; int gp_nprobe[3][LM_GRAPH_BUCKETS] = {};
                       int tile_m[2] = {0, 0}; hipGraphExec_t tile_g[2] = {nullptr, nullptr}; int tile_seen[2] = {0, 0};
                       unsigned long long last_use = 0; };
@@ -1884,6 +1886,7 @@
     unsigned long long gset_clock = 0;
     bool async_pending = false;
     unsigned long long rng_host = 0;
+    bool spec_pending = false;
     bool graphs_enabled = true;
     bool mfma_prefill = true;
     bool fuse_attn = true;
@@ -1924,8 +1927,10 @@
             if (gs.gp[i][b]) { (void)hipGraphExecDestroy(gs.gp[i][b]); gs.gp[i][b] = nullptr; }
         }
     for (int i = 0; i <= LM_FRAME_MAX; ++i)
-        for (int b = 0; b < LM_GRAPH_BUCKETS; ++b)
+        for (int b = 0; b < LM_GRAPH_BUCKETS; ++b) {
             if (gs.fg[i][b]) { (void)hipGraphExecDestroy(gs.fg[i][b]); gs.fg[i][b] = nullptr; }
+            if (gs.fgs[i][b]) { (void)hipGraphExecDestroy(gs.fgs[i][b]); gs.fgs[i][b] = nullptr; }
+        }
     for (int i = 0; i < 2; ++i) {
         if (gs.tile_g[i]) { (void)hipGraphExecDestroy(gs.tile_g[i]); gs.tile_g[i] = nullptr; }
         gs.tile_m[i] = gs.tile_seen[i] = 0;
@@ -2457,7 +2462,7 @@
     if ((rc = lm_alloc((void**)&h->attn, (size_t)LM_MAXM * AO * 4)) != RCA_OK) return rc;
     if ((rc = lm_alloc((void**)&h->hbuf, (size_t)LM_MAXM * c.ffn * 4)) != RCA_OK) return rc;
     if ((rc = lm_alloc((void**)&h->att_part, (size_t)(LM_MAXM / 2) * c.n_kv_heads * h->n_splits * 8 * 66 * 4)) != RCA_OK) return rc;
-    h->logits_rows_cap = c.logits_all ? 64 : 1;
+    h->logits_rows_cap = c.logits_all ? 64 : 2;
     if ((rc = lm_alloc((void**)&h->logits, (size_t)h->logits_rows_cap * c.vocab_size * 4)) != RCA_OK) return rc;
     if ((rc = lm_alloc((void**)&h->probs_dev, (64 + 2 * PROBS_SLICES) * 4)) != RCA_OK) return rc;
     if ((rc = lm_alloc((void**)&h->probe_ids_dev, 64 * 4)) != RCA_OK) return rc;
@@ -2683,6 +2688,7 @@
     while (g.bpw > 1 && (N + g.R * g.bpw - 1) / (g.R * g.bpw) < 64) g.bpw >>= 1;
     return g;
 }
+constexpr bool gemv_has_m3(int Q, int ACT) { return ACT == 0 && (Q == WF_BF16 || Q == WF_F16 || Q == WF_Q8 || Q == WF_Q4K || Q == WF_Q6K); }
 template <int M, int NIT, int PRO, int EPI, int Q, int ACT>
 static void launch_gemv_r(const GemvGeom& g, rca_lm* h, const WMat& w, const float* x, float* y, int N, int K, int ldy, const GemvPro& pro,
                           const GemvRope& rope, hipStream_t st) {
@@ -2705,6 +2711,17 @@
     const int max_loads = (Q == WF_Q4K || Q == WF_Q5K || Q == WF_Q40) ? 8 : 16;
     while (g.R > 4 && (g.R / lpr) * (nit == 3 ? 4 : nit) > max_loads) g.R >>= 1;
     if ((Q == WF_Q4K || Q == WF_Q6K || Q == WF_Q5K || Q == WF_Q40) && g.R < 8) g.R = 8;
+    if (M == 3) {
+        if constexpr (gemv_has_m3(Q, ACT)) {
+            if (PRO == 0 && EPI == 3 && nit > 1) {
+                if (nit == 2) launch_gemv_r<3, 2, 0, 3, Q, ACT>(g, h, w, x, y, N, K, ldy, pro, rope, st);
+                else launch_gemv_r<3, 4, 0, 3, Q, ACT>(g, h, w, x, y, N, K, ldy, pro, rope, st);
+            } else {
+                launch_gemv_r<3, 1, PRO, EPI, Q, ACT>(g, h, w, x, y, N, K, ldy, pro, rope, st);
+            }
+        }
+        return;
+    }
     if (PRO == 0 && EPI == 3 && nit > 1) {
         if (nit == 2) {
             if (M == 1) launch_gemv_r<1, 2, 0, 3, Q, ACT>(g, h, w, x, y, N, K, ldy, pro, rope, st);
@@ -3506,14 +3523,27 @@
 static void lm_launch_down(rca_lm* h, int l, int M, hipStream_t st) {
     launch_gemv<0, 3>(GEMV_DOWN, h, M, h->layers[l].down, h->hbuf, h->x, h->cfg.hidden, h->cfg.ffn, h->cfg.hidden, nopro, norope, st);
 }
-static void lm_launch_head(rca_lm* h, int M, hipStream_t st, float* out, bool only_last) {
+static void lm_launch_head(rca_lm* h, int M, hipStream_t st, float* out, bool only_last, int row0 = 0) {
     const rca_lm_config_t& c = h->cfg;
-    launch_gemv<1, 0>(GEMV_HEAD, h, M, h->head, nullptr, out, c.vocab_size, c.hidden, c.vocab_size, GemvPro{h->x, h->final_norm, c.rms_eps, only_last ? 1 : 0}, norope, st);
+    launch_gemv<1, 0>(GEMV_HEAD, h, M, h->head, nullptr, out, c.vocab_size, c.hidden, c.vocab_size,
+                      GemvPro{h->x + (long)row0 * c.hidden, h->final_norm, c.rms_eps, only_last ? 1 : 0}, norope, st);
+}
+static bool lm_has_m3(const rca_lm* h) {
+    auto ok = [&](const WMat& w) {
+        if (!w.N) return true;
+        bool r = false;
+        wf_dispatch(w.fmt, [&](auto wf) { r = gemv_has_m3(decltype(wf)::value, wf_packed(decltype(wf)::value) && h->act_format == 1 ? 1 : 0); });
+        return r;
+    };
+    for (const LmLayer& L : h->layers)
+        if (!(ok(L.qkv) && ok(L.o) && ok(L.gu) && ok(L.down) && (!L.split_v || ok(L.vseg)))) return false;
+    return ok(h->head);
 }
 
 static int lm_enqueue_pass(rca_lm* h, int M, int want_logits, hipStream_t st, int nsp_launch, bool skip_embed = false) {
     const rca_lm_config_t& c = h->cfg;
     if (M < 1 || M > LM_GEMV_M) return fail(RCA_ERR_ARG, "decode pass of %d tokens", M);
+    if (M == 3 && !lm_has_m3(h)) return fail(RCA_ERR_STATE, "decode pass of 3 tokens: a matrix format of this handle has no M = 3 GEMV");
     if (!skip_embed) lm_embed_kernel<<<M, 256, 0, st>>>(h->stt, h->embed, h->embed_f32, h->x, c.hidden, c.vocab_size);
     for (int l = 0; l < c.n_layers; ++l) {
         lm_launch_qkv(h, l, M, st);
@@ -3523,6 +3553,7 @@
         lm_launch_down(h, l, M, st);
     }
     if (want_logits == 1) lm_launch_head(h, 1, st, h->logits, true);
+    else if (want_logits == 3) lm_launch_head(h, 2, st, h->logits, false, M - 2);
     else if (want_logits) lm_launch_head(h, M, st, h->logits, false);
     RCA_LAUNCH_CHECK();
     return RCA_OK;
@@ -4127,8 +4158,8 @@
             if (!last) RCA_HIP(hipStreamSynchronize(st));
         }
     } else {
-        for (int off = 0; off < n; off += LM_GEMV_M) {
-            const int m = std::min(LM_GEMV_M, n - off);
+        for (int off = 0; off < n; off += LM_EVAL_M) {
+            const int m = std::min(LM_EVAL_M, n - off);
             const bool last = off + m >= n;
             if ((rc = lm_push_state(h, ids + off, m, st)) != RCA_OK) return rc;
             if (all) h->logits = logits_base + (long)off * h->cfg.vocab_size;
@@ -4336,12 +4367,46 @@
     const unsigned long long zero = 0;
     RCA_HIP(hipMemcpy(&h->stt->rng_counter, &zero, 8, hipMemcpyHostToDevice));
     h->rng_host = 0;
+    h->spec_pending = false;
     h->sampler_set = true;
     if (full != h->samp_full || patch != h->samp_patch || big_k != h->samp_big_k || big_p != h->samp_big_p)
         lm_drop_graphs(h);
     h->samp_full = full; h->samp_patch = patch; h->samp_big_k = big_k; h->samp_big_p = big_p;
     return RCA_OK;
 }
+
+#define SPEC_IDS 16
+#define SPEC_PROBS 16
+__global__ __launch_bounds__(256) void lm_spec_arm_kernel(LmDevState* __restrict__ stt, const int* __restrict__ tok, const void* __restrict__ table,
+                                                          int f32tab, float* __restrict__ x, int H, int V) {
+    int id = *tok;
+    if (threadIdx.x == 0) { stt->m = 3; stt->ids[2] = id; }
+    id = id < 0 ? 0 : (id >= V ? V - 1 : id);
+    for (int e = threadIdx.x; e < H; e += 256)
+        x[2L * H + e] = f32tab ? reinterpret_cast<const float*>(table)[(long)id * H + e]
+                               : __uint_as_float((unsigned)reinterpret_cast<const bf16_t*>(table)[(long)id * H + e] << 16);
+}
+static int lm_push_rng(rca_lm* h) {
+    h->h_stt->rng_counter = h->rng_host;
+    RCA_HIP(hipMemcpyAsync(&h->stt->rng_counter, &h->h_stt->rng_counter, 8, hipMemcpyHostToDevice, h->stream));
+    return RCA_OK;
+}
+static int lm_spec_settle(rca_lm* h) {
+    if (!h->spec_pending) return RCA_OK;
+    h->spec_pending = false;
+    return lm_push_rng(h);
+}
+static bool lm_spec_args_ok(const rca_lm* h, const rca_spec_probe_t* sp) {
+    if (sp->n_ids < 1 || sp->n_ids > 8 || sp->token < 0 || sp->token >= h->cfg.vocab_size) return false;
+    for (int i = 0; i < sp->n_ids; ++i)
+        if (sp->ids[i] < 0 || sp->ids[i] >= h->cfg.vocab_size) return false;
+    return true;
+}
+static void lm_spec_stage(rca_lm* h, const rca_spec_probe_t* sp) {
+    for (int i = 0; i < 8; ++i) h->h_probe[SPEC_IDS + i] = i < sp->n_ids ? sp->ids[i] : 0;
+    h->h_probe[SPEC_IDS + 8] = sp->token;
+}
+static int lm_enqueue_spec_tail(rca_lm* h, int n_ids, hipStream_t st);
 
 static void lm_enqueue_sample(rca_lm* h, float* lg, hipStream_t st, int frame_i = -1) {
     const int V = h->cfg.vocab_size;
@@ -4380,6 +4445,7 @@
     if (!h->sampler_set) return fail(RCA_ERR_STATE, "sampler not initialised");
     if (h->logits_rows < 1) return fail(RCA_ERR_STATE, "no logits: call eval first");
     RCA_HIP(hipSetDevice(h->device));
+    { const int src = lm_spec_settle(h); if (src != RCA_OK) return src; }
     float* lg = h->logits + (long)(h->logits_rows - 1) * h->cfg.vocab_size;
     lm_enqueue_sample(h, lg, h->stream);
     RCA_LAUNCH_CHECK();
@@ -4401,6 +4467,7 @@
     RCA_HIP(hipSetDevice(h->device));
     hipStream_t st = h->stream;
     int rc;
+    if ((rc = lm_spec_settle(h)) != RCA_OK) return rc;
     if (n > 2 || h->cfg.logits_all || !h->graphs_enabled) {
         if ((rc = rca_lm_eval(h, ids, n)) != RCA_OK) return rc;
         if ((rc = rca_lm_sample(h, token)) != RCA_OK) return rc;
@@ -4456,8 +4523,22 @@
     return lm_step_impl(h, ids, n, probe_ids, n_probe, token, probs_out);
 }
 
+static int lm_enqueue_spec_tail(rca_lm* h, int n_ids, hipStream_t st) {
+    const int V = h->cfg.vocab_size;
+    lm_enqueue_sample(h, h->logits + V, st);
+    lm_softmax_slices_kernel<<<PROBS_SLICES, 1024, 0, st>>>(h->logits + V, V, h->probs_dev + 64);
+    lm_token_probs_kernel<<<1, 64, 0, st>>>(h->logits + V, V, h->probs_dev + 64, h->probe_ids_dev + SPEC_IDS, n_ids, h->probs_dev + SPEC_PROBS);
+    hipError_t e = hipMemcpyAsync(&h->h_stt->out_token, &h->stt->out_token, 4, hipMemcpyDeviceToHost, st);
+    if (e == hipSuccess) e = hipMemcpyAsync(h->h_probe + 64 + SPEC_PROBS, h->probs_dev + SPEC_PROBS, 8 * 4, hipMemcpyDeviceToHost, st);
+    return e == hipSuccess ? RCA_OK : fail(RCA_ERR_HIP, "spec d2h: %s", hipGetErrorString(e));
+}
+static int lm_enqueue_spec_pass(rca_lm* h, hipStream_t st, int nsp_launch, bool skip_embed) {
+    lm_spec_arm_kernel<<<1, 256, 0, st>>>(h->stt, h->probe_ids_dev + SPEC_IDS + 8, h->embed, h->embed_f32, h->x, h->cfg.hidden, h->cfg.vocab_size);
+    return lm_enqueue_pass(h, 3, 3, st, nsp_launch, skip_embed);
+}
 static int lm_frame_core(rca_lm_t* h, const int32_t* first_pair, const int32_t* user_ids, int32_t n_steps, int32_t audio_id_floor,
-                         int32_t* out_tokens, int32_t* n_done, int cap_bucket) {
+                         int32_t* out_tokens, int32_t* n_done, int cap_bucket, const rca_spec_probe_t* spec = nullptr,
+                         rca_spec_result_t* spec_out = nullptr) {
     if (!h || !first_pair || !user_ids || !out_tokens || !n_done) return fail(RCA_ERR_ARG, "frame: null argument");
     if (n_steps < 1 || n_steps > LM_FRAME_MAX) return fail(RCA_ERR_ARG, "frame: %d steps (1..%d)", n_steps, LM_FRAME_MAX);
     if (!h->sampler_set) return fail(RCA_ERR_STATE, "sampler not initialised");
@@ -4467,22 +4548,34 @@
         if (first_pair[i] < 0 || first_pair[i] >= h->cfg.vocab_size) return fail(RCA_ERR_ARG, "frame: token id %d outside the vocabulary", first_pair[i]);
     for (int i = 0; i < n_steps; ++i)
         if (user_ids[i] < 0 || user_ids[i] >= h->cfg.vocab_size) return fail(RCA_ERR_ARG, "frame: token id %d outside the vocabulary", user_ids[i]);
+    if (spec && (!spec_out || !lm_spec_args_ok(h, spec))) return fail(RCA_ERR_ARG, "frame: speculative probe: a token and 1..8 ids inside the vocabulary, and a result");
+    if (spec_out) spec_out->valid = 0;
     { const int src = lm_settle(h); if (src != RCA_OK) return src; }
     RCA_HIP(hipSetDevice(h->device));
     hipStream_t st = h->stream;
     int rc = RCA_OK;
+    if (cap_bucket < 0 && (rc = lm_spec_settle(h)) != RCA_OK) return rc;
+    const bool with_spec = spec && h->graphs_enabled && lm_has_m3(h) && (cap_bucket >= 0 || h->n_tokens + 2 * n_steps + 1 <= h->cfg.n_ctx);
     lm_stage_state(h, first_pair, 2);
     for (int i = 0; i < n_steps; ++i) h->h_stt->ids[LM_FRAME_USER0 + i] = user_ids[i];
-    const LmBucket bk = lm_bucket(h, 2 * n_steps, cap_bucket);
-    hipGraphExec_t& gexec = lm_graph_set(h).fg[n_steps][bk.bucket];
+    if (with_spec) lm_spec_stage(h, spec);
+    const LmBucket bk = lm_bucket(h, 2 * n_steps + (with_spec ? 1 : 0), cap_bucket);
+    rca_lm::GraphSet& gs = lm_graph_set(h);
+    hipGraphExec_t& gexec = with_spec ? gs.fgs[n_steps][bk.bucket] : gs.fg[n_steps][bk.bucket];
+    if (with_spec && gexec && gs.fgs_nprobe[n_steps][bk.bucket] != spec->n_ids) { (void)hipGraphExecDestroy(gexec); gexec = nullptr; }
     if (cap_bucket >= 0 && (gexec || !h->graphs_enabled)) return RCA_OK;
     auto enqueue = [&]() -> int {
         hipError_t e = hipMemcpyAsync(h->stt, h->h_stt, LM_STATE_DECODE_BYTES, hipMemcpyHostToDevice, st);
+        if (e == hipSuccess && with_spec) e = hipMemcpyAsync(h->probe_ids_dev + SPEC_IDS, h->h_probe + SPEC_IDS, 9 * 4, hipMemcpyHostToDevice, st);
         if (e != hipSuccess) return fail(RCA_ERR_HIP, "frame memcpy: %s", hipGetErrorString(e));
         for (int i = 0; i < n_steps; ++i) {
-            const int r = lm_enqueue_pass(h, 2, 1, st, bk.nsp_launch, i > 0);
+            const int r = (with_spec && i + 1 == n_steps) ? lm_enqueue_spec_pass(h, st, bk.nsp_launch, i > 0) : lm_enqueue_pass(h, 2, 1, st, bk.nsp_launch, i > 0);
             if (r != RCA_OK) return r;
             lm_enqueue_sample(h, h->logits, st, i);
+        }
+        if (with_spec) {
+            const int r = lm_enqueue_spec_tail(h, spec->n_ids, st);
+            if (r != RCA_OK) return r;
         }
         e = hipMemcpyAsync(h->h_stt->frame_out, h->stt->frame_out, sizeof(int) * LM_FRAME_MAX, hipMemcpyDeviceToHost, st);
         return e == hipSuccess ? RCA_OK : fail(RCA_ERR_HIP, "frame d2h: %s", hipGetErrorString(e));
@@ -4490,8 +4583,9 @@
     if (!h->graphs_enabled) {
         RCA_HIP(hipStreamSynchronize(st));
         if ((rc = enqueue()) != RCA_OK) return rc;
-    } else if (!gexec && (rc = lm_capture(st, &gexec, "frame", enqueue)) != RCA_OK) {
-        return rc;
+    } else if (!gexec) {
+        if ((rc = lm_capture(st, &gexec, "frame", enqueue)) != RCA_OK) return rc;
+        if (with_spec) gs.fgs_nprobe[n_steps][bk.bucket] = spec->n_ids;
     }
     if (cap_bucket >= 0) return RCA_OK;
     if (h->graphs_enabled) RCA_HIP(hipGraphLaunch(gexec, st));
@@ -4507,7 +4601,28 @@
     h->rng_host += (unsigned long long)done;
     if (done < n_steps) {
         RCA_HIP(hipMemcpy(&h->stt->rng_counter, &h->rng_host, 8, hipMemcpyHostToDevice));
-    }
+    } else if (with_spec) {
+        spec_out->valid = 1;
+        spec_out->token = h->h_stt->out_token;
+        for (int i = 0; i < 8; ++i) spec_out->probs[i] = i < spec->n_ids ? reinterpret_cast<const float*>(h->h_probe + 64 + SPEC_PROBS)[i] : 0.0f;
+        h->spec_pending = true;
+    }
+    return RCA_OK;
+}
+extern "C" int rca_lm_frame_spec(rca_lm_t* h, const int32_t* first_pair, const int32_t* user_ids, int32_t n_steps, int32_t audio_id_floor,
+                                 const rca_spec_probe_t* spec, int32_t* out_tokens, int32_t* n_done, rca_spec_result_t* spec_out) {
+    return lm_frame_core(h, first_pair, user_ids, n_steps, audio_id_floor, out_tokens, n_done, -1, spec, spec_out);
+}
+extern "C" int rca_lm_spec_commit(rca_lm_t* h, int32_t used) {
+    if (!h) return fail(RCA_ERR_ARG, "null");
+    if (!h->spec_pending) return fail(RCA_ERR_STATE, "spec_commit: the last call on this handle delivered no speculative probe row");
+    if (!used) {
+        RCA_HIP(hipSetDevice(h->device));
+        return lm_spec_settle(h);
+    }
+    h->spec_pending = false;
+    h->rng_host += 1;
+    h->logits_rows = 2;
     return RCA_OK;
 }
 
@@ -4549,9 +4664,10 @@
     const void* kc;
     unsigned long long codec_sig;
     const void* codec;
+    int spec = 0;
     bool operator==(const DuplexGraphKey& o) const {
         return T == o.T && F_ctx == o.F_ctx && n_steps == o.n_steps && n_samples == o.n_samples && probe == o.probe && bucket == o.bucket &&
-               base == o.base && kc == o.kc && codec_sig == o.codec_sig && codec == o.codec;
+               base == o.base && kc == o.kc && codec_sig == o.codec_sig && codec == o.codec && spec == o.spec;
     }
 };
 struct DuplexState {
@@ -4649,8 +4765,10 @@
 }
 
 static int duplex_frame_core(rca_lm_t* h, rca_codec_t* codec, const rca_duplex_frame_args_t* a, rca_duplex_frame_out_t* out,
-                             float* pcm_out_host, int cap_bucket) {
+                             float* pcm_out_host, int cap_bucket, const rca_spec_probe_t* spec = nullptr, rca_spec_result_t* spec_out = nullptr) {
     const bool cap_only = cap_bucket >= 0;
+    if (spec && ((!cap_only && !spec_out) || !h || !lm_spec_args_ok(h, spec))) return fail(RCA_ERR_ARG, "duplex_frame: speculative probe: a token and 1..8 ids inside the vocabulary, and a result");
+    if (spec_out) spec_out->valid = 0;
     if (!h || !codec || !a || (!cap_only && (!out || !pcm_out_host || !a->pcm_window || (a->F_ctx > 0 && !a->code_ctx)))) return fail(RCA_ERR_ARG, "duplex_frame: null argument");
     const int n = a->n_steps;
     if (n < 1 || n > LM_FRAME_MAX) return fail(RCA_ERR_ARG, "duplex_frame: %d steps (1..%d)", n, LM_FRAME_MAX);
@@ -4670,7 +4788,10 @@
     { const int src = lm_settle(h); if (src != RCA_OK) return src; }
     RCA_HIP(hipSetDevice(h->device));
     hipStream_t st = h->stream;
+    if (!cap_only && (rc = lm_spec_settle(h)) != RCA_OK) return rc;
     if ((rc = duplex_reserve(h, a->T, a->F_ctx, n, a->n_samples)) != RCA_OK) return rc;
+    const bool with_spec = spec && h->graphs_enabled && lm_has_m3(h) && (cap_only || h->n_tokens + 2 * n + 1 <= h->cfg.n_ctx);
+    if (with_spec) lm_spec_stage(h, spec);
     DuplexState* d = h->duplex;
     const int F = a->F_ctx + n;
     const DuplexPinLayout lay(a->T, a->F_ctx, a->n_samples);
@@ -4683,10 +4804,11 @@
         memcpy(d->pin + lay.pcm, a->pcm_window, (size_t)a->T * 4);
         if (a->F_ctx) memcpy(d->pin + lay.codes, a->code_ctx, (size_t)a->F_ctx * 8);
     }
-    const LmBucket bk = lm_bucket(h, 2 * n, cap_bucket);
+    const LmBucket bk = lm_bucket(h, 2 * n + (with_spec ? 1 : 0), cap_bucket);
     uint64_t csig = 0;
     if ((rc = rca_codec_workspace_sig(codec, &csig)) != RCA_OK) return rc;
-    DuplexGraphKey key{a->T, a->F_ctx, n, a->n_samples, a->probe_id >= 0 ? 1 : 0, bk.bucket, a->code_token_base, (const void*)h->kc, csig, (const void*)codec};
+    DuplexGraphKey key{a->T, a->F_ctx, n, a->n_samples, a->probe_id >= 0 ? 1 : 0, bk.bucket, a->code_token_base, (const void*)h->kc, csig, (const void*)codec,
+                       with_spec ? spec->n_ids : 0};
     DuplexState::Entry* ent = nullptr;
     for (auto& e : d->graphs)
         if (e.key == key) ent = &e;
@@ -4703,6 +4825,7 @@
         if (e == hipSuccess) e = hipMemcpyAsync(d->pcm_in, d->pin + lay.pcm, (size_t)a->T * 4, hipMemcpyHostToDevice, st);
         if (e == hipSuccess && a->F_ctx) e = hipMemcpyAsync(d->code_win, d->pin + lay.codes, (size_t)a->F_ctx * 8, hipMemcpyHostToDevice, st);
         if (e == hipSuccess) e = hipMemcpyAsync(&d->dev->probe_id, &pin->probe_id, 4, hipMemcpyHostToDevice, st);
+        if (e == hipSuccess && with_spec) e = hipMemcpyAsync(h->probe_ids_dev + SPEC_IDS, h->h_probe + SPEC_IDS, 9 * 4, hipMemcpyHostToDevice, st);
         if (e != hipSuccess) return fail(RCA_ERR_HIP, "duplex h2d: %s", hipGetErrorString(e));
         hipStream_t se = d->fork ? d->side : st;
         if (d->fork) {
@@ -4718,7 +4841,8 @@
             if (e != hipSuccess) return fail(RCA_ERR_HIP, "duplex join: %s", hipGetErrorString(e));
         }
         for (int i = 0; i < n; ++i) {
-            if ((r = lm_enqueue_pass(h, 2, 1, st, bk.nsp_launch, i > 0)) != RCA_OK) return r;
+            r = (with_spec && i + 1 == n) ? lm_enqueue_spec_pass(h, st, bk.nsp_launch, i > 0) : lm_enqueue_pass(h, 2, 1, st, bk.nsp_launch, i > 0);
+            if (r != RCA_OK) return r;
             if (i == 0 && d->fork) {
                 e = hipStreamWaitEvent(st, d->ev_join, 0);
                 if (e != hipSuccess) return fail(RCA_ERR_HIP, "duplex join: %s", hipGetErrorString(e));
@@ -4731,6 +4855,7 @@
             lm_softmax_slices_kernel<<<PROBS_SLICES, 1024, 0, st>>>(h->logits, h->cfg.vocab_size, h->probs_dev + 64);
             lm_token_probs_kernel<<<1, 64, 0, st>>>(h->logits, h->cfg.vocab_size, h->probs_dev + 64, &d->dev->probe_id, 1, &d->dev->probe_prob);
         }
+        if (with_spec && (r = lm_enqueue_spec_tail(h, spec->n_ids, st)) != RCA_OK) return r;
         RCA_LAUNCH_CHECK();
         e = hipMemcpyAsync(pin->frame_out, h->stt->frame_out, sizeof(int) * LM_FRAME_MAX, hipMemcpyDeviceToHost, st);
         if (e == hipSuccess) e = hipMemcpyAsync(pin->user_codes, d->dev->user_codes, sizeof(long long) * LM_FRAME_MAX + 8, hipMemcpyDeviceToHost, st);
@@ -4774,7 +4899,19 @@
     h->logits_rows = done < n ? 0 : 1;
     h->rng_host += (unsigned long long)done;
     if (done < n) RCA_HIP(hipMemcpy(&h->stt->rng_counter, &h->rng_host, 8, hipMemcpyHostToDevice));
-    return RCA_OK;
+    else if (with_spec && out->flags == 0) {
+        spec_out->valid = 1;
+        spec_out->token = h->h_stt->out_token;
+        for (int i = 0; i < 8; ++i) spec_out->probs[i] = i < spec->n_ids ? reinterpret_cast<const float*>(h->h_probe + 64 + SPEC_PROBS)[i] : 0.0f;
+        h->spec_pending = true;
+    } else if (with_spec) {
+        return lm_push_rng(h);
+    }
+    return RCA_OK;
+}
+extern "C" int rca_duplex_frame_spec(rca_lm_t* h, rca_codec_t* codec, const rca_duplex_frame_args_t* a, const rca_spec_probe_t* spec,
+                                     rca_duplex_frame_out_t* out, rca_spec_result_t* spec_out, float* pcm_out_host) {
+    return duplex_frame_core(h, codec, a, out, pcm_out_host, -1, spec, spec_out);
 }
 
 extern "C" int rca_duplex_frame(rca_lm_t* h, rca_codec_t* codec, const rca_duplex_frame_args_t* a, rca_duplex_frame_out_t* out,
@@ -4797,6 +4934,11 @@
         for (int b = 0; b < LM_GRAPH_BUCKETS && rc == RCA_OK; ++b) {
             if (!lm_bucket_reachable(h, b)) break;
             rc = duplex_frame_core(h, codec, a, nullptr, nullptr, b);
+            if (rc == RCA_OK && n_probe > 0 && n_probe <= 8) {
+                rca_spec_probe_t sp{};
+                sp.n_ids = n_probe;
+                rc = duplex_frame_core(h, codec, a, nullptr, nullptr, b, &sp, nullptr);
+            }
             if (rc == RCA_OK && n_probe > 0) rc = lm_step_capture_only(h, 1, n_probe, b);
             if (rc == RCA_OK) {
                 const int32_t pair[2] = {0, 0}, users[LM_FRAME_MAX] = {0, 0, 0, 0, 0, 0, 0, 0};
@@ -5005,7 +5147,8 @@
     const rca_lm_config_t& c = h->cfg;
     const int H = c.hidden, QKV = (c.n_heads + 2 * c.n_kv_heads) * c.head_dim, AO = c.n_heads * c.head_dim, F = c.ffn, V = c.vocab_size;
     if (kind < 0 || kind > 4) return fail(RCA_ERR_ARG, "gemv_tap: kind %d outside [0, 4]", kind);
-    if (M < 1 || M > LM_GEMV_M) return fail(RCA_ERR_ARG, "gemv_tap: M = %d, a decode pass has 1 or %d tokens", M, LM_GEMV_M);
+    if (M < 1 || M > LM_GEMV_M) return fail(RCA_ERR_ARG, "gemv_tap: M = %d, a decode pass has 1 to %d tokens", M, LM_GEMV_M);
+    if (M == 3 && !lm_has_m3(h)) return fail(RCA_ERR_STATE, "gemv_tap: a matrix format of this handle has no M = 3 GEMV");
     if (kind != 4 && (layer < 0 || layer >= c.n_layers)) return fail(RCA_ERR_ARG, "gemv_tap: layer %d outside [0, %d)", layer, c.n_layers);
     if (h->n_tokens + M > c.n_ctx) return fail(RCA_ERR_STATE, "gemv_tap: positions %d .. %d are outside the context of %d", h->n_tokens, h->n_tokens + M - 1, c.n_ctx);
     const int in_w[5] = {H, AO, H, F, H}, out_w[5] = {AO, H, F, H, V};
diff --git a/realtime_codec_agent_amd/llm.py b/realtime_codec_agent_amd/llm.py
--- a/realtime_codec_agent_amd/llm.py
+++ b/realtime_codec_agent_amd/llm.py
@@ -463,6 +463,49 @@
         self._logits_valid = False
         return toks
 
+    @staticmethod
+    def _spec_probe_c(spec_token: int, spec_ids: Sequence[int]) -> "N.SpecProbeC":
+        ids = [int(t) for t in spec_ids]
+        if not 1 <= len(ids) <= 8:
+            raise ValueError("the speculative probe row takes 1..8 ids")
+        sp = N.SpecProbeC(token=int(spec_token), n_ids=len(ids))
+        for i, t in enumerate(ids):
+            sp.ids[i] = t
+        return sp
+
+    def _spec_result(self, sp: "N.SpecProbeC", so: "N.SpecResultC"):
+        self._spec_token = int(sp.token) if so.valid else None
+        if not so.valid:
+            return None, None
+        return int(so.token), np.array(so.probs[:sp.n_ids], dtype=np.float32)
+
+    def frame_spec(self, first_pair: Sequence[int], user_ids: Sequence[int], audio_id_floor: int, spec_token: int, spec_ids: Sequence[int]):
+        first_pair, user_ids = [int(t) for t in first_pair], [int(t) for t in user_ids]
+        if len(first_pair) != 2:
+            raise ValueError("frame_spec() starts from the last [agent, user] pair")
+        n, n0 = len(user_ids), self.n_tokens
+        fp = (C.c_int32 * 2)(*first_pair)
+        us = (C.c_int32 * n)(*user_ids)
+        out = (C.c_int32 * n)()
+        done = C.c_int32()
+        sp, so = self._spec_probe_c(spec_token, spec_ids), N.SpecResultC()
+        N.check(self._lib.rca_lm_frame_spec(self._h, fp, us, n, int(audio_id_floor), C.byref(sp), out, C.byref(done), C.byref(so)), "rca_lm_frame_spec")
+        toks = list(out[:done.value])
+        evaluated = first_pair + [t for pair in zip(toks[:-1], user_ids) for t in pair]
+        self._input_ids[n0:n0 + len(evaluated)] = evaluated
+        self._logits_valid = False
+        tok, probs = self._spec_result(sp, so)
+        return toks, tok, probs
+
+    def spec_commit(self, used: bool) -> None:
+        N.check(self._lib.rca_lm_spec_commit(self._h, 1 if used else 0), "rca_lm_spec_commit")
+        if used:
+            n0 = self.n_tokens
+            if n0 < len(self._input_ids) and getattr(self, "_spec_token", None) is not None:
+                self._input_ids[n0] = self._spec_token
+            self._logits_valid = False
+        self._spec_token = None
+
     def duplex_prepare(self, T: int, F_ctx: int, n_steps: int, n_samples: int) -> None:
         N.check(self._lib.rca_duplex_prepare(self._h, int(T), int(F_ctx), int(n_steps), int(n_samples)), "rca_duplex_prepare")
 
@@ -474,7 +517,8 @@
                 "rca_duplex_precapture")
 
     def duplex_frame(self, codec_handle, pcm_window: np.ndarray, code_ctx: np.ndarray, n_steps: int, n_samples: int,
-                     code_token_base: int, audio_id_floor: int, probe_id: int, first_pair: Sequence[int]) -> dict:
+                     code_token_base: int, audio_id_floor: int, probe_id: int, first_pair: Sequence[int],
+                     spec_token: Optional[int] = None, spec_ids: Optional[Sequence[int]] = None) -> dict:
         first_pair = [int(t) for t in first_pair]
         if len(first_pair) != 2:
             raise ValueError("duplex_frame() starts from the last [agent, user] pair")
@@ -487,7 +531,14 @@
         a.first_pair[0], a.first_pair[1] = first_pair
         out = N.DuplexFrameOutC()
         pcm = np.empty(int(n_samples), dtype=np.float32)
-        N.check(self._lib.rca_duplex_frame(self._h, codec_handle._h, C.byref(a), C.byref(out), C.c_void_p(pcm.ctypes.data)), "rca_duplex_frame")
+        spec_tok = spec_probs = None
+        if spec_token is not None and spec_ids:
+            sp, so = self._spec_probe_c(spec_token, spec_ids), N.SpecResultC()
+            N.check(self._lib.rca_duplex_frame_spec(self._h, codec_handle._h, C.byref(a), C.byref(sp), C.byref(out), C.byref(so),
+                                                    C.c_void_p(pcm.ctypes.data)), "rca_duplex_frame_spec")
+            spec_tok, spec_probs = self._spec_result(sp, so)
+        else:
+            N.check(self._lib.rca_duplex_frame(self._h, codec_handle._h, C.byref(a), C.byref(out), C.c_void_p(pcm.ctypes.data)), "rca_duplex_frame")
         codes = [int(c) for c in out.user_codes[:n_steps]]
         toks = [int(t) for t in out.tokens[:out.n_done]]
         user_ids = [int(code_token_base) + c for c in codes]
@@ -495,7 +546,8 @@
         self._input_ids[n0:n0 + len(evaluated)] = evaluated
         self._logits_valid = False
         return {"user_codes": codes, "tokens": toks, "pcm": pcm if out.flags == 0 else None,
-                "probe_prob": float(out.probe_prob) if out.probe_prob >= 0.0 else None}
+                "probe_prob": float(out.probe_prob) if out.probe_prob >= 0.0 else None,
+                "spec_token": spec_tok, "spec_probs": spec_probs}
 
     def generate(self, tokens: Sequence[int], reset: bool = True, stopping_criteria=None) -> Generator[int, Optional[Sequence[int]], None]:
         tokens = list(tokens)
diff --git a/realtime_codec_agent_amd/realtime_agent_v2.py b/realtime_codec_agent_amd/realtime_agent_v2.py
--- a/realtime_codec_agent_amd/realtime_agent_v2.py
+++ b/realtime_codec_agent_amd/realtime_agent_v2.py
@@ -54,6 +54,9 @@
         self.frame_graph_active = False
         self.use_duplex_graph = True
         self.duplex_graph_frames = 0
+        self.use_spec_probe = True
+        self.spec_probe_frames = 0
+        self.separate_probe_steps = 0
         self.use_kv_shadow = True
         self.precapture_graphs = True
         self.kv_shadow_tile = 128
@@ -506,7 +509,7 @@
                         suppress_end_audio = not self.generate_for_response()
         return out
 
-    def measure_event_prob(self, p_end: Optional[float] = None):
+    def measure_event_prob(self, p_end: Optional[float] = None, spec_probs=None):
         llm = self.resources.llm
         if p_end is not None:
             pass
@@ -516,10 +519,21 @@
             logits = np.ctypeslib.as_array(llm._ctx.get_logits(), shape=(llm._n_vocab,))
             p_end = float(_softmax(logits)[self.end_audio_token_id])
         self.stats.event_prob.add_value(p_end)
-        self.prob_event_speaker_token_id = self.get_probable_event_speaker() if self.stats.event_prob.last_zscore >= 0.0 else None
+        want = self.stats.event_prob.last_zscore >= 0.0
+        if spec_probs is not None:
+            llm.spec_commit(want)
+            if want:
+                self.spec_probe_frames += 1
+                pa, pu = spec_probs
+                self.prob_event_speaker_token_id = self.agent_speaker_token_id if pa > pu else self.user_speaker_token_id
+            else:
+                self.prob_event_speaker_token_id = None
+            return
+        self.prob_event_speaker_token_id = self.get_probable_event_speaker() if want else None
 
     def get_probable_event_speaker(self) -> int:
         llm = self.resources.llm
+        self.separate_probe_steps += 1
         if hasattr(llm, "step_probe"):
             _, (pa, pu) = llm.step_probe([self.end_audio_token_id], [self.agent_speaker_token_id, self.user_speaker_token_id])
             llm.n_tokens -= 1
@@ -613,8 +627,11 @@
             with prof:
                 pass
         with p.lm_profiler:
+            spec = {}
+            if self.use_spec_probe and hasattr(llm, "spec_commit"):
+                spec = dict(spec_token=self.end_audio_token_id, spec_ids=[self.agent_speaker_token_id, self.user_speaker_token_id])
             res = llm.duplex_frame(at.codec_model.hip, plan["window"], plan["code_ctx"], plan["n_codes"], plan["n_samples"], base,
-                                   self.end_header_token_id, self.end_audio_token_id, self.input_ids[-2:])
+                                   self.end_header_token_id, self.end_audio_token_id, self.input_ids[-2:], **spec)
             at.duplex_commit_pcm(plan)
             self.frame_graph_active = True
             self.duplex_graph_frames += 1
@@ -629,7 +646,7 @@
         else:
             out_chunk = self.detokenize_output_chunk(out_ids)
         self.audio_history_ch2.append(audio_chunk)
-        self.measure_event_prob(res["probe_prob"] if res["pcm"] is not None else None)
+        self.measure_event_prob(res["probe_prob"] if res["pcm"] is not None else None, res.get("spec_probs"))
         self.update_inactivity_timers()
         assert out_chunk.shape[-1] == self.chunk_size_samples and len(out_ids) == self.chunk_size_frames_per_channel
         return out_chunk, out_ids
```

Result: no change. 3431 audio-hours/hour (median of 2 runs) (-0.0%).
